# Luonic/semi-supervised_semantic_segmentation

Hardware: AMD Instinct MI355X
Metric: images/sec (UNet-R50 512x512 bs=16/GPU, mean-teacher + CowMix semi-supervised training step) (higher is better)
Workload: dtype bf16; 1 GPU; C2: UNet(ResNet-50 encoder, max_width=128, ConvT up) 512x512, semi-supervised mean-teacher + CowMix step (BCE sup loss w=0.5, consistency w=10, SGD m=0.9); global_batch=16, per_gpu_batch=16, image_size=512, parallelism=dp1

## Files before the change

### include/ssseg.h

```cpp
#ifndef SSSEG_H
#define SSSEG_H
#include <stdint.h>
#include <stddef.h>

#ifdef __cplusplus
extern "C" {
#endif

typedef struct ihipStream_t* ssseg_stream_t;

enum { SSSEG_F32 = 0, SSSEG_BF16 = 1, SSSEG_F16 = 2, SSSEG_F64 = 3  };
enum { SSSEG_OK = 0, SSSEG_EINVAL = -1, SSSEG_EUNSUPPORTED = -2, SSSEG_EWORKSPACE = -3, SSSEG_ECOMM = -4 };

const char* ssseg_version(void);


size_t ssseg_cowmix_workspace_bytes(int64_t B, int64_t H, int64_t W);

int ssseg_cowmix_mask(const float* noise, const float* sigma, const float* p, int64_t B, int64_t H,
                      int64_t W, float* mask_out, float* field_out, float* thr_out, void* workspace,
                      size_t workspace_bytes, ssseg_stream_t stream);

int ssseg_normal_f32(float* out, int64_t n, uint64_t seed, uint64_t offset, ssseg_stream_t stream);

// ... 184 lines not shown
                        const float* gout, float* gx, const void* ws, size_t ws_bytes, ssseg_stream_t stream);

int ssseg_ohem_labels_fwd(const float* x, const void* labels, int label_kind, int64_t B, int64_t C, int64_t HW,
                          int64_t ignore_label, float thresh, int64_t min_kept, float* out, void* ws, size_t ws_bytes,
                          ssseg_stream_t stream);
int ssseg_ohem_labels_bwd(const float* x, const void* labels, int label_kind, int64_t B, int64_t C, int64_t HW,
                          const float* gout, float* gx, const void* ws, size_t ws_bytes, ssseg_stream_t stream);

int ssseg_focal_fwd(const float* x, const float* t, int64_t n, double alpha, double gamma, float* out, void* ws,
                    size_t ws_bytes, ssseg_stream_t stream);
int ssseg_focal_bwd(const float* x, const float* t, int64_t n, double alpha, double gamma, const float* gout,
                    float* gx, ssseg_stream_t stream);

typedef struct ssseg_nfl_params {
  double alpha, gamma, eps, scale, weight, ignore_label;
  int32_t from_logits, size_average;
} ssseg_nfl_params;
int ssseg_nfl_fwd(const float* x, const float* label, int64_t B, int64_t C, int64_t HW,
                  const ssseg_nfl_params* params_host, float* out, float* k_sum, void* ws, size_t ws_bytes,
                  ssseg_stream_t stream);
int ssseg_nfl_bwd(const float* x, const float* label, int64_t B, int64_t C, int64_t HW,
                  const ssseg_nfl_params* params_host, const float* gout, float* gx, const void* ws, size_t ws_bytes,
                  ssseg_stream_t stream);

int ssseg_dice_logits_fwd(const float* x, const float* t, int64_t B, int64_t C, int64_t HW, float* out, void* ws,
                          size_t ws_bytes, ssseg_stream_t stream);
int ssseg_dice_logits_bwd(const float* x, const float* t, int64_t B, int64_t C, int64_t HW, const float* gout,
                          float* gx, const void* ws, size_t ws_bytes, ssseg_stream_t stream);

int ssseg_dice_prob_fwd(const float* p, const float* t, int64_t B, int64_t n, int log_mode, float gamma, float* out,
                        void* ws, size_t ws_bytes, ssseg_stream_t stream);
int ssseg_dice_prob_bwd(const float* t, int64_t B, int64_t n, int log_mode, float gamma, const float* gout,
                        float* gx, const void* ws, size_t ws_bytes, ssseg_stream_t stream);

int ssseg_binary_entropy_fwd(const float* x, int64_t n, float* out, void* ws, size_t ws_bytes,
                             ssseg_stream_t stream);
int ssseg_binary_entropy_bwd(const float* x, int64_t n, const float* gout, float* gx, ssseg_stream_t stream);
int ssseg_entropy_fwd(const float* x, int64_t B, int64_t C, int64_t HW, float* out, void* ws, size_t ws_bytes,
                      ssseg_stream_t stream);
int ssseg_entropy_bwd(const float* x, int64_t B, int64_t C, int64_t HW, const float* gout, float* gx,
                      ssseg_stream_t stream);

int ssseg_bce_logits_red_fwd(const float* x, const float* t, int64_t n, int reduction, float* out, void* ws,
                             size_t ws_bytes, ssseg_stream_t stream);
int ssseg_bce_logits_red_bwd(const float* x, const float* t, int64_t n, int reduction, const float* gout, float* gx,
                             ssseg_stream_t stream);

int ssseg_smooth_labels(const float* t, float* out, int64_t n, float a, float b, ssseg_stream_t stream);


int ssseg_ema_update(float* ema, const float* param, int64_t n, double alpha, ssseg_stream_t stream);

int ssseg_sigmoid_fwd(const float* x, float* y, int64_t n, ssseg_stream_t stream);
int ssseg_sigmoid_bwd(const float* y, const float* gy, float* gx, int64_t n, ssseg_stream_t stream);

int ssseg_axpby(const float* x, float a, const float* y, float b, float* out, int64_t n, ssseg_stream_t stream);
int ssseg_scale_f32(float* x, int64_t n, float a, ssseg_stream_t stream);

int ssseg_sqnorm_accum(const float* x, int64_t n, float* out, void* ws, size_t ws_bytes, ssseg_stream_t stream);

int ssseg_sgd_step(float* param, float* grad, float* momentum_buf, uint16_t* bf16_shadow, int64_t n,
                   float lr, float momentum, float weight_decay, float max_norm, const float* sqnorm,
                   int first_step, const float* amp_state, ssseg_stream_t stream);
int ssseg_amp_update(float* state, const float* sqnorm, float growth, float backoff, int interval,
                     ssseg_stream_t stream);
enum { SSSEG_OPT_ADAM = 0, SSSEG_OPT_ADAMOD = 1, SSSEG_OPT_DIFFGRAD = 2, SSSEG_OPT_DIFFMOD = 3, SSSEG_OPT_RANGER = 4 };
#define SSSEG_OPT_STATE_DOUBLES 8
int ssseg_optim_prepare(double* state, int mode, double lr, double beta1, double beta2, double weight_decay,
                        double max_norm, int64_t k, double nsma_threshold, const float* sqnorm,
                        const float* amp_state, ssseg_stream_t stream);
int ssseg_optim_step(float* param, const float* grad, float* exp_avg, float* exp_avg_sq, float* exp_avg_lr,
                     float* previous_grad, float* slow_buffer, int64_t n, int mode, int version, double beta1,
                     double beta2, double beta3, double eps, double weight_decay, double alpha, const double* state,
                     ssseg_stream_t stream);
int ssseg_scale_by(const float* x, const float* s, float* y, int64_t n, ssseg_stream_t stream);

typedef struct {
  int64_t N, H, W, C, ldx;
  int64_t OH, OW;
  int64_t K;
  int64_t R, S;
  int64_t sy, sx, dy, dx, py, px;
  int64_t outH, outW;
  int64_t osy, osx, ooy, oox;
  int64_t ldy;
  int64_t ldw;
} ssseg_conv_desc;

int ssseg_conv_igemm(const void* x, const void* w, void* y, const ssseg_conv_desc* desc_host, int dt, int dt_out,
                     const float* bias, int relu, void* ws, size_t ws_bytes, ssseg_stream_t stream);
#define SSSEG_ACT_NONE 0
#define SSSEG_ACT_RELU 1
#define SSSEG_ACT_RELU6 2
#define SSSEG_ACT_LEAKY 3

typedef struct ssseg_conv_epilogue {
  const float* scale;
  const float* shift;
  const void* residual;
  int64_t ldr;
  void* aux;
  int32_t relu;
  float slope;
  double* stats;
  int64_t stats_ld;
  int64_t* stats_rows_host;
} ssseg_conv_epilogue;
int ssseg_conv_igemm_epi(const void* x, const void* w, void* y, const ssseg_conv_desc* desc_host, int dt, int dt_out,
                         const ssseg_conv_epilogue* epi, void* ws, size_t ws_bytes, ssseg_stream_t stream);
int ssseg_conv_igemm_epi_actmask(const void* x, const void* w, void* y, const ssseg_conv_desc* desc_host, int dt,
                                 int dt_out, const ssseg_conv_epilogue* epi, int act, float slope, void* ws,
                                 size_t ws_bytes, ssseg_stream_t stream);
int ssseg_conv_igemm_epi_join(const void* x, const void* w, void* y, const ssseg_conv_desc* desc_host, int dt,
                              int dt_out, const ssseg_conv_epilogue* epi, const void* mask, int64_t ldm, void* ws,
                              size_t ws_bytes, ssseg_stream_t stream);
typedef struct {
  const void* x2;
  int64_t c1;
  int64_t ldx2;
} ssseg_vcat;

int ssseg_conv_igemm_epi_vcat(const void* x, const ssseg_vcat* vc, const void* w, void* y,
                              const ssseg_conv_desc* desc_host, int dt, int dt_out, const ssseg_conv_epilogue* epi,
                              void* ws, size_t ws_bytes, ssseg_stream_t stream);
int ssseg_conv_igemm_epi_vsplit(const void* x, const void* w, void* y, const ssseg_vcat* ysplit,
                                const ssseg_conv_desc* desc_host, int dt, int dt_out, const ssseg_conv_epilogue* epi,
                                void* ws, size_t ws_bytes, ssseg_stream_t stream);
int ssseg_conv_igemm_phases(const void* x, void* y, const ssseg_conv_desc* desc_host, int dt, int dt_out,
                            const ssseg_conv_epilogue* epi, int64_t nphase, const int64_t* phase_geom,
                            const void* const* w, ssseg_stream_t stream);
size_t ssseg_conv_igemm_phases_workspace_bytes(const ssseg_conv_desc* desc_host, int64_t nphase, int dt);
int ssseg_conv_igemm_phases_ws(const void* x, void* y, const ssseg_conv_desc* desc_host, int dt, int dt_out,
                               const ssseg_conv_epilogue* epi, int64_t nphase, const int64_t* phase_geom,
                               const void* const* w, void* ws, size_t ws_bytes, ssseg_stream_t stream);

int ssseg_conv_stem_epi(const void* x, const void* w4, void* y, const ssseg_conv_desc* desc_host, int dt,
                        const ssseg_conv_epilogue* epi, ssseg_stream_t stream);
size_t ssseg_conv_igemm_workspace_bytes(const ssseg_conv_desc* desc_host, int dt);

int ssseg_set_knob(int id, int value);

int64_t ssseg_tune_table_export(unsigned long long* keys_host, int32_t* variants_host, int64_t cap);
int ssseg_tune_table_import(const unsigned long long* keys_host, const int32_t* variants_host, int64_t n,
                            int overwrite);

size_t ssseg_conv_wgrad_workspace_bytes(const ssseg_conv_desc* desc_host, int dt);
int ssseg_conv_wgrad(const void* x, const void* dy, float* dw, const ssseg_conv_desc* desc_host, int dt, int64_t c_real,
                     int64_t k_real, int layout, int accumulate, void* ws, size_t ws_bytes, ssseg_stream_t stream);

size_t ssseg_conv_wgrad2_workspace_bytes(const ssseg_conv_desc* desc_host, int64_t n2, int dt);
int ssseg_conv_wgrad2(const void* x, const void* dy, const void* x2, const void* dy2, int64_t n2, float* dw,
                      const ssseg_conv_desc* desc_host, int dt, int64_t c_real, int64_t k_real, int layout,
                      int accumulate, void* ws, size_t ws_bytes, ssseg_stream_t stream);

int ssseg_conv_wgrad_vcat(const void* x, const ssseg_vcat* vc, const void* dy, float* dw,
                          const ssseg_conv_desc* desc_host, int dt, int64_t c_real, int64_t k_real, int layout,
                          int accumulate, void* ws, size_t ws_bytes, ssseg_stream_t stream);
int ssseg_conv_wgrad2_vcat(const void* x, const ssseg_vcat* vc, const void* dy, const void* x2, const ssseg_vcat* vc2,
                           const void* dy2, int64_t n2, float* dw, const ssseg_conv_desc* desc_host, int dt,
                           int64_t c_real, int64_t k_real, int layout, int accumulate, void* ws, size_t ws_bytes,
                           ssseg_stream_t stream);

int ssseg_weight_pack(const float* src, void* dst, int64_t Kd, int64_t Kr, int64_t Cd, int64_t Rs, int64_t Ss,
                      int64_t Cp, int layout, int64_t r0, int64_t rstep, int64_t Rn, int64_t s0, int64_t sstep,
                      int64_t Sn, int dt, ssseg_stream_t stream);

typedef struct ssseg_pack_desc {
  const float* src;
  void* dst;
  int64_t Kd, Kr, Cd, Rs, Ss, Cp;
  int64_t layout, r0, rstep, Rn, s0, sstep, Sn;
} ssseg_pack_desc;
int ssseg_weight_pack_batch(const ssseg_pack_desc* descs, int64_t n, int dt, ssseg_stream_t stream);

#define SSSEG_PSTEP_SGD 1
#define SSSEG_PSTEP_EMA 2
#define SSSEG_PSTEP_CLEAR 4
typedef struct ssseg_pstep_desc {
  int64_t off, n;
  int64_t A, B, Rs, Ss, Ap, Bp;
  int64_t pack0, npacks;
} ssseg_pstep_desc;
typedef struct ssseg_pstep_pack {
  void* dst;
  int64_t teacher, layout;
  int64_t Kd, Cp, r0, rstep, Rn, s0, sstep, Sn;
} ssseg_pstep_pack;
int ssseg_param_step(float* param, float* grad, float* momentum_buf, float* ema, const ssseg_pstep_desc* descs,
                     int64_t n_descs, const ssseg_pstep_pack* packs, float lr, float momentum, float weight_decay,
                     float max_norm, const float* sqnorm, int first_step, const float* amp_state, double alpha,
                     int flags, ssseg_stream_t stream);

int ssseg_dwconv_fwd(const void* x, const void* w, void* y, const ssseg_conv_desc* desc_host, int dt,
                     const ssseg_conv_epilogue* epi, ssseg_stream_t stream);
int ssseg_dwconv_dgrad(const void* dy, const void* w, void* dx, const ssseg_conv_desc* desc_host, int dt,
                       ssseg_stream_t stream);
size_t ssseg_dwconv_wgrad_workspace_bytes(const ssseg_conv_desc* desc_host, int dt);
int ssseg_dwconv_wgrad(const void* x, const void* dy, float* dw, const ssseg_conv_desc* desc_host, int dt,
                       int64_t c_real, int accumulate, void* ws, size_t ws_bytes, ssseg_stream_t stream);

size_t ssseg_bn_workspace_bytes(int64_t C);
int ssseg_bn_stats(const void* x, int64_t P, int64_t C, int64_t ldx, int dt, double* sums, void* ws, size_t ws_bytes,
                   ssseg_stream_t stream);
int ssseg_bn_finalize(const double* sums, int64_t C, double count, float eps, float momentum, float* mean_out,
                      float* invstd_out, float* running_mean, float* running_var, int64_t* num_batches_tracked,
                      ssseg_stream_t stream);
int ssseg_bn_stats_finalize(const void* x, int64_t P, int64_t C, int64_t ldx, int dt, double* sums, void* ws,
                            size_t ws_bytes, double count, float eps, float momentum, float* mean_out, float* invstd_out,
                            float* running_mean, float* running_var, int64_t* num_batches_tracked,
                            ssseg_stream_t stream);
int ssseg_bn_partials_finalize(double* part, int64_t nparts, int64_t C, double* sums, double count, float eps,
                               float momentum, float* mean_out, float* invstd_out, float* running_mean,
                               float* running_var, int64_t* num_batches_tracked, ssseg_stream_t stream);
int ssseg_channel_sum_grad(const void* x, int64_t P, int64_t C, int64_t ldx, int dt, float* dsum, double* sums,
                           void* ws, size_t ws_bytes, ssseg_stream_t stream);
int ssseg_bn_gstat_finalize(double* part, int64_t nparts, int64_t C, double* sums, const float* gamma,
                            const float* beta, const float* mean_eff, const float* invstd, float* dgamma, float* dbeta,
                            float* dconv_bias, ssseg_stream_t stream);
int ssseg_bn_gstat_finalize_x(double* part, int64_t nparts, int64_t C, double* sums, const float* gamma,
                              const float* beta, const void* dy, const void* x, int64_t P, int64_t ld, int dt,
                              const float* mean, const float* invstd, float* dgamma, float* dbeta,
                              ssseg_stream_t stream);
int ssseg_bn_eval_params(const float* running_mean, const float* running_var, float eps, int64_t C, float* mean_out,
                         float* invstd_out, ssseg_stream_t stream);
int ssseg_bn_fold(const float* running_mean, const float* running_var, const float* gamma, const float* beta,
                  const float* conv_bias, float eps, int64_t C, int64_t Cp, float* scale, float* shift,
                  float* mean_eff, float* invstd_out, ssseg_stream_t stream);
typedef struct ssseg_fold_desc {
  const float* running_mean;
  const float* running_var;
  const float* gamma;
  const float* beta;
  const float* conv_bias;
  float* out;
  int64_t C, Cp;
  double eps;
} ssseg_fold_desc;
int ssseg_bn_fold_batch(const ssseg_fold_desc* descs, int64_t n, ssseg_stream_t stream);
int ssseg_bn_eval_bwd(const void* dy, const void* y, const void* aux, void* dconv, void* dres, int64_t P, int64_t C,
                      int64_t ld, const float* scale, const float* mean_eff, const float* invstd, int relu, int dt,
                      double* sums, void* ws, size_t ws_bytes, ssseg_stream_t stream);
int ssseg_bn_eval_param_grad(const double* sums, int64_t C, const float* scale, float* dgamma, float* dbeta,
                             float* dconv_bias, ssseg_stream_t stream);
int ssseg_bn_eval_bwd_grad(const void* dy, const void* y, const void* aux, void* dconv, void* dres, int64_t P, int64_t C,
                           int64_t ld, const float* scale, const float* mean_eff, const float* invstd, int relu, int dt,
                           double* sums, void* ws, size_t ws_bytes, float* dgamma, float* dbeta, float* dconv_bias,
                           ssseg_stream_t stream);
int ssseg_bn_eval_bwd_grad_y(const void* dy, const void* y, void* dconv, void* dres, int64_t P, int64_t C, int64_t ld,
                             const float* scale, const float* shift, const float* mean_eff, const float* invstd,
                             int relu, int dt, double* sums, void* ws, size_t ws_bytes, float* dgamma, float* dbeta,
                             float* dconv_bias, ssseg_stream_t stream);
int ssseg_bn_eval_bwd_part(const void* dy, const void* y, const void* aux, void* dconv, void* dres, int64_t P, int64_t C,
                           int64_t ld, const float* scale, const float* shift, const float* mean_eff,
                           const float* invstd, int relu, int dt, double* part, size_t part_bytes, int64_t* nparts_host,
                           ssseg_stream_t stream);
typedef struct ssseg_pgrad_desc {
  const double* part;
  int64_t nparts, C;
  const float* scale;
  float* dgamma;
  float* dbeta;
  float* dconv_bias;
  const float* shift;
  const float* mean_eff;
  const float* invstd;
} ssseg_pgrad_desc;
int ssseg_bn_param_grad_batch(const ssseg_pgrad_desc* descs, int64_t n, int64_t max_c, ssseg_stream_t stream);
int ssseg_bn_apply(const void* x, const void* residual, void* y, int64_t P, int64_t C, int64_t ldx, int64_t ldr,
                   int64_t ldy, const float* mean, const float* invstd, const float* gamma, const float* beta, int relu,
                   int dt, ssseg_stream_t stream);
int ssseg_bn_bwd_reduce(const void* dy, const void* x, const void* residual, int64_t P, int64_t C, int64_t ldx,
                        int64_t ldr, int64_t lddy, const float* mean, const float* invstd, const float* gamma,
                        const float* beta, int relu, int dt, double* sums, void* ws, size_t ws_bytes,
                        ssseg_stream_t stream);
int ssseg_bn_param_grad(const double* sums, int64_t C, float* dgamma, float* dbeta, ssseg_stream_t stream);
int ssseg_bn_bwd_reduce_grad(const void* dy, const void* x, const void* residual, int64_t P, int64_t C, int64_t ldx,
                             int64_t ldr, int64_t lddy, const float* mean, const float* invstd, const float* gamma,
                             const float* beta, int relu, int dt, double* sums, void* ws, size_t ws_bytes,
                             float* dgamma, float* dbeta, ssseg_stream_t stream);
int ssseg_bn_bwd_apply(const void* dy, const void* x, const void* residual, void* dx, void* dres, int64_t P, int64_t C,
                       int64_t ldx, int64_t ldr, int64_t lddy, int64_t lddx, const float* mean, const float* invstd,
                       const float* gamma, const float* beta, int relu, int train, const double* sums, double count,
                       int dt, ssseg_stream_t stream);

int ssseg_maxpool_fwd(const void* x, void* y, uint8_t* idx, int64_t N, int64_t H, int64_t W, int64_t C, int64_t OH,
                      int64_t OW, int64_t k, int64_t s, int64_t p, int dt, ssseg_stream_t stream);
int ssseg_maxpool_bwd(const void* gy, const uint8_t* idx, void* gx, int64_t N, int64_t H, int64_t W, int64_t C,
                      int64_t OH, int64_t OW, int64_t k, int64_t s, int64_t p, int dt, ssseg_stream_t stream);
int ssseg_maxpool_bwd_res(const void* gy, const uint8_t* idx, const void* res, void* gx, int64_t N, int64_t H,
                          int64_t W, int64_t C, int64_t OH, int64_t OW, int64_t k, int64_t s, int64_t p, int dt,
                          ssseg_stream_t stream);
int ssseg_nhwc_copy(const void* src, void* dst, int64_t N, int64_t H, int64_t W, int64_t C, int64_t sH, int64_t sW,
                    int64_t sld, int64_t soy, int64_t sox, int64_t dH, int64_t dW, int64_t dld, int64_t doy, int64_t dox,
                    int dt, ssseg_stream_t stream);
int ssseg_zero(void* p, size_t bytes, ssseg_stream_t stream);

typedef struct {
  const void* src;
  void* dst;
  const void* add;
  int64_t ld;
  int64_t c;
} ssseg_cat_part;
int ssseg_nhwc_cat_n(const ssseg_cat_part* parts_host, int64_t nparts, void* y, int64_t npix, int64_t ldy, int dt,
                     ssseg_stream_t stream);
int ssseg_nhwc_split_n(const void* gy, int64_t ldg, const ssseg_cat_part* parts_host, int64_t nparts, int64_t npix,
// ... 100 lines not shown
```

### semi-supervised_semantic_segmentation_amd/csrc/conv_kernels.h

```cpp
#pragma once
#include <algorithm>
#include <type_traits>

#include "common.h"

typedef __bf16 bf16x8 __attribute__((ext_vector_type(8)));
typedef _Float16 f16x8 __attribute__((ext_vector_type(8)));

typedef short s16x4 __attribute__((ext_vector_type(4)));
typedef float f32x4 __attribute__((ext_vector_type(4)));

template <typename T16> struct M16;
template <> struct M16<bf16_t> {
  __device__ __forceinline__ static f32x4 mma(const bf16x8& a, const bf16x8& b, const f32x4& c) {
    return __builtin_amdgcn_mfma_f32_16x16x32_bf16(a, b, c, 0, 0, 0);
  }
};
template <> struct M16<f16_t> {
  __device__ __forceinline__ static f32x4 mma(const bf16x8& a, const bf16x8& b, const f32x4& c) {
    return __builtin_amdgcn_mfma_f32_16x16x32_f16(__builtin_bit_cast(f16x8, a), __builtin_bit_cast(f16x8, b), c, 0, 0,
                                                  0);
  }
};
typedef __attribute__((address_space(3))) s16x4 lds_s16x4;
// ... 1222 lines not shown
      const float z[8] = {0.f, 0.f, 0.f, 0.f, 0.f, 0.f, 0.f, 0.f};
      Out8<TO>::st(ep.aux + op * g.ldy + n, z);
    }
    Out8<TO>::st(out_at(ep, y, g.ldy, op, n), v);
  }
}

template <typename TO>
__global__ void phase_zero_kernel(TO* y, ConvGeom g, Epi<TO> ep) {
  const long long total = g.M * g.K;
  for (long long i = (long long)blockIdx.x * blockDim.x + threadIdx.x; i < total; i += (long long)gridDim.x * blockDim.x) {
    const int n = (int)(i % g.K);
    const long long m = i / g.K;
    const long long op = out_pixel(g, (int)m);
    float v = ep.shift ? ep.shift[n] : 0.f;
    if (ep.aux) io<TO>::st(ep.aux, op * g.ldy + n, 0.f);
    if (ep.res && !ep.rmask) v += io<TO>::ld(ep.res, op * ep.ldr + n);
    v = act_fwd(v, ep.relu, ep.slope);
    io<TO>::st(out_at(ep, y, g.ldy, op, n), 0, v);
  }
}

template <typename T, int BM, int BN>
inline int plan_splits(const ConvGeom& g);

template <typename TO>
__global__ void splitk_finalize_kernel(const float* __restrict__ ws, TO* __restrict__ y, ConvGeom g, Epi<TO> ep);

extern thread_local int t_dsplit;

unsigned* ticket_slots(long long n);

template <typename TO, int BM, int BN, int WM, int WN, int NW, int NS, int VC>
int launch_glds_vc(const void* x, const void* w, void* y, const ConvGeom& g, const Epi<TO>& ep, unsigned xb,
                   unsigned wb, hipStream_t s, float* ws, const PhaseTab* ph, const void* x2, unsigned x2b) {
  static_assert(sizeof(TO) == 2, "LDS-DMA configs: 16-bit activations in and out (fp32-output heads have K <= 16)");
  constexpr int FRAGS = (BM / WM / 16) * (BN / WN / 16);
  const long long tiles = ((g.M + BM - 1) / BM) * ((g.K + BN - 1) / BN);
  const int epi = (int)(g_knobs[7] == 0);
  const TO* xa = (const TO*)x2;
  const PhaseTab one{1, {0}, {0}, {0}, {0}, {nullptr}};
  const bool phased = ph && ph->n > 1;
  const PhaseTab& pt = phased ? *ph : one;
  const unsigned nph = phased ? (unsigned)ph->n : 1u;
  const int sp = ws ? t_dsplit : 1;
  if (sp > 1 && (FRAGS > DSPLIT_MAX_FRAGS || tiles * sp > 0x7fffffffLL)) return -1;
  unsigned* tix = sp > 1 ? ticket_slots(tiles * nph) : nullptr;
  if (sp > 1 && !tix) return -1;
  const dim3 grid((unsigned)(tiles * sp), nph);
  if (ep.zmask) {
    if constexpr (VC != 1 && BM * BN < 256 * 256) {
      if (ep.stats) return -1;
      hipLaunchKernelGGL((igemm_glds_kernel<TO, BM, BN, WM, WN, NW, NS, false, VC, true>), grid, dim3(NW * 64), 0, s,
                         (const TO*)x, (const TO*)w, (TO*)y, g, ep, xb, wb, epi, sp, ws, tix, pt, xa, x2b);
      return BM;
    }
    return -1;
  }
  if (ep.stats)
    hipLaunchKernelGGL((igemm_glds_kernel<TO, BM, BN, WM, WN, NW, NS, true, VC>), grid, dim3(NW * 64), 0, s,
                       (const TO*)x, (const TO*)w, (TO*)y, g, ep, xb, wb, epi, sp, ws, tix, pt, xa, x2b);
  else
    hipLaunchKernelGGL((igemm_glds_kernel<TO, BM, BN, WM, WN, NW, NS, false, VC>), grid, dim3(NW * 64), 0, s,
                       (const TO*)x, (const TO*)w, (TO*)y, g, ep, xb, wb, epi, sp, ws, tix, pt, xa, x2b);
  return BM;
}

static inline size_t dsplit_ws_bytes(const ConvGeom& g, int nph, int S) {
  if (S <= 1) return 0;
  const long long t64 = (long long)nph * ((g.M + 63) / 64) * ((g.K + 63) / 64);
  return (size_t)(dsplit_ticket_bytes(t64) + (long long)S * nph * (g.M + 255) * (g.K + 127) * 4);
}

template <typename TO, int BM, int BN, int WM, int WN, int NW, int NS>
int launch_glds(const void* x, const void* w, void* y, const ConvGeom& g, const Epi<TO>& ep, unsigned xb, unsigned wb,
                hipStream_t s, float* ws, const PhaseTab* ph, const void* x2 = nullptr, unsigned x2b = 0) {
  if (x2) return launch_glds_vc<TO, BM, BN, WM, WN, NW, NS, 1>(x, w, y, g, ep, xb, wb, s, ws, ph, x2, x2b);
  if (g.C & 63) {
    if constexpr (BN == 64) return launch_glds_vc<TO, BM, BN, WM, WN, NW, NS, 2>(x, w, y, g, ep, xb, wb, s, ws, ph, nullptr, 0);
    return -1;
  }
  return launch_glds_vc<TO, BM, BN, WM, WN, NW, NS, 0>(x, w, y, g, ep, xb, wb, s, ws, ph, nullptr, 0);
}


template <typename TO>
int launch_glds_grp_a(int cfg, const void* x, const void* w, void* y, const ConvGeom& g, const Epi<TO>& ep, unsigned xb,
                      unsigned wb, hipStream_t s, float* ws, const PhaseTab* ph, const void* x2 = nullptr,
                      unsigned x2b = 0);
template <typename TO>
int launch_glds_grp_b(int cfg, const void* x, const void* w, void* y, const ConvGeom& g, const Epi<TO>& ep, unsigned xb,
                      unsigned wb, hipStream_t s, float* ws, const PhaseTab* ph, const void* x2 = nullptr,
                      unsigned x2b = 0);
template <typename TO>
int launch_glds_grp_d(int cfg, const void* x, const void* w, void* y, const ConvGeom& g, const Epi<TO>& ep, unsigned xb,
                      unsigned wb, hipStream_t s, float* ws, const PhaseTab* ph, const void* x2 = nullptr,
                      unsigned x2b = 0);
template <typename TO>
int launch_glds_grp_e(int cfg, const void* x, const void* w, void* y, const ConvGeom& g, const Epi<TO>& ep, unsigned xb,
                      unsigned wb, hipStream_t s, float* ws, const PhaseTab* ph, const void* x2 = nullptr,
                      unsigned x2b = 0);
template <typename TO>
int launch_glds_grp_c(int cfg, const void* x, const void* w, void* y, const ConvGeom& g, const Epi<TO>& ep, unsigned xb,
                      unsigned wb, hipStream_t s, float* ws, const PhaseTab* ph, const void* x2 = nullptr,
                      unsigned x2b = 0);


template <typename T, int BM, int BN>
inline int plan_splits(const ConvGeom& g) {
  const long long tiles = ((g.M + BM - 1) / BM) * ((g.K + BN - 1) / BN);
  const int nk = (g.KK + 64 / (int)sizeof(T) - 1) / (64 / (int)sizeof(T));
  if (g_knobs[1] < 0 || tiles >= 512 || nk < 32) return 1;
  long long sp = (1024 + tiles - 1) / tiles;
  sp = std::min<long long>(sp, nk / 16);
  if (g_knobs[1] > 0) sp = std::min<long long>(sp, g_knobs[1]);
  return (int)std::max<long long>(1, std::min<long long>(sp, 64));
}


template <typename TO>
int launch_hconv3(const void* x, const void* w, void* y, const ConvGeom& g, const Epi<TO>& ep, unsigned xb,
                  unsigned wb, hipStream_t s, float* ws, const PhaseTab* ph, const void* x2, unsigned x2b,
                  int mode = 0);

template <typename TO>
int launch_hconv3s(const void* x, const void* w, void* y, const ConvGeom& g, const Epi<TO>& ep, unsigned xb,
                   hipStream_t s, float* ws, const PhaseTab* ph, const void* x2);

template <typename TO>
int launch_pw(int fj, const void* x, const void* w, void* y, const ConvGeom& g, const Epi<TO>& ep, hipStream_t s,
              float* ws, const PhaseTab* ph, const void* x2);
extern thread_local long long t_pw_rows;

struct HaloSeg {
  const void* x;
  const void* x2;
  const void* dy;
  unsigned xbytes, x2bytes, dbytes;
};
struct HaloArgs {
  HaloSeg seg[2];
  int H, W, C, K, ldx, ldx2, ldy, c1;
  int ncb, nkb, nstrips;
  long long steps[2], sps[2];
  int splits, s1;
  float* slab;
  float* dw;
  int c_real, k_real, layout, accumulate;
};
struct HaloPlan {
  int ncb, nkb, nstrips, splits, s1;
  long long steps[2], sps[2];
};
bool halo3_eligible(const ConvGeom& g, int dt);
HaloPlan halo3_plan(const ConvGeom& g, long long n1, long long n2);
size_t halo3_ws_bytes(const ConvGeom& g, long long n1, long long n2);
void launch_wgrad_halo3(int dt, const HaloArgs& a, hipStream_t s);

template <typename T, typename TO>
int dispatch_regstaged(const void* x, const void* w, void* y, const ConvGeom& g, const Epi<TO>& ep, float* ws,
                       hipStream_t s);
```

### semi-supervised_semantic_segmentation_amd/csrc/conv_wgrad.hip

```cpp
#include <algorithm>

#include "conv_kernels.h"

template <typename T> struct WG;
template <> struct WG<bf16_t> {
  static constexpr int BKP = 64;
  static constexpr int PADB = 32;
};
template <> struct WG<f16_t> : WG<bf16_t> {};
template <> struct WG<float> {
  static constexpr int BKP = 16;
  static constexpr int PADB = 64;
};

__device__ __forceinline__ int kperm(int g, int j) { return 16 * (g >> 1) + 8 * (j >> 2) + 4 * (g & 1) + (j & 3); }

struct WDirect {
  float* dw;
  int c_real, k_real, layout, accumulate;
};

template <typename T, int BMW, int BNW>
__global__ void __launch_bounds__(256) wgrad_kernel(const T* __restrict__ x, const T* __restrict__ dy,
                                                    float* __restrict__ slab, ConvGeom g, long long pix_per_split,
// ... 90 lines not shown
    const int buf = kt & 1;
    if (kt + 1 < nk) load();
    const char* Xs = smem + buf * BKP * (ROWX + ROWD);
    const char* Ds = Xs + BKP * ROWX;
    if constexpr (sizeof(T) == 2) {
#pragma unroll
      for (int ks = 0; ks < BKP / 32; ++ks) {
      bf16x8 af[FM], bfr[FN];
      const int r0 = ks * 32 + kperm(gq, q4), r1 = ks * 32 + kperm(gq, 4 + q4);
#pragma unroll
      for (int i = 0; i < FM; ++i) {
        const int col = wm * WTM + i * 16 + 4 * p4;
        s16x4 lo = __builtin_amdgcn_ds_read_tr16_b64_v4i16((lds_s16x4*)(Xs + r0 * ROWX + col * 2));
        s16x4 hi = __builtin_amdgcn_ds_read_tr16_b64_v4i16((lds_s16x4*)(Xs + r1 * ROWX + col * 2));
        af[i] = __builtin_bit_cast(bf16x8, __builtin_shufflevector(lo, hi, 0, 1, 2, 3, 4, 5, 6, 7));
      }
#pragma unroll
      for (int j = 0; j < FN; ++j) {
        const int col = wn * WTN + j * 16 + 4 * p4;
        s16x4 lo = __builtin_amdgcn_ds_read_tr16_b64_v4i16((lds_s16x4*)(Ds + r0 * ROWD + col * 2));
        s16x4 hi = __builtin_amdgcn_ds_read_tr16_b64_v4i16((lds_s16x4*)(Ds + r1 * ROWD + col * 2));
        bfr[j] = __builtin_bit_cast(bf16x8, __builtin_shufflevector(lo, hi, 0, 1, 2, 3, 4, 5, 6, 7));
      }
#pragma unroll
      for (int i = 0; i < FM; ++i)
#pragma unroll
        for (int j = 0; j < FN; ++j) acc[i][j] = M16<T>::mma(af[i], bfr[j], acc[i][j]);
      }
    } else {
#pragma unroll
      for (int ks = 0; ks < BKP / 4; ++ks) {
        const int row = ks * 4 + gq;
        float af[FM], bfr[FN];
#pragma unroll
        for (int i = 0; i < FM; ++i) af[i] = *(const float*)(Xs + row * ROWX + (wm * WTM + i * 16 + li) * 4);
#pragma unroll
        for (int j = 0; j < FN; ++j) bfr[j] = *(const float*)(Ds + row * ROWD + (wn * WTN + j * 16 + li) * 4);
#pragma unroll
        for (int i = 0; i < FM; ++i)
#pragma unroll
          for (int j = 0; j < FN; ++j) acc[i][j] = __builtin_amdgcn_mfma_f32_16x16x4f32(af[i], bfr[j], acc[i][j], 0, 0, 0);
      }
    }
    if (kt + 1 < nk) store(buf ^ 1);
    __syncthreads();
  }

  if (dd.dw) {
#pragma unroll
    for (int i = 0; i < FM; ++i) {
      const int kkb = kk0 + wm * WTM + i * 16 + 4 * gq;
#pragma unroll
      for (int j = 0; j < FN; ++j) {
        const int co = co0 + wn * WTN + j * 16 + li;
        if (co >= dd.k_real) continue;
#pragma unroll
        for (int e = 0; e < 4; ++e) {
          const int kk = kkb + e;
          if (kk >= g.KK) continue;
          const int c = kk % g.C, tap = kk / g.C;
          if (c >= dd.c_real) continue;
          long long o;
          if (dd.layout == 0) o = ((long long)co * g.R * g.S + tap) * g.C + c;
          else o = (((long long)co * dd.c_real + c) * g.R + tap / g.S) * g.S + tap % g.S;
          dd.dw[o] = dd.accumulate ? dd.dw[o] + acc[i][j][e] : acc[i][j][e];
        }
      }
    }
    return;
  }
  float* sl = slab + (long long)blockIdx.z * g.K * g.KK;
#pragma unroll
  for (int i = 0; i < FM; ++i) {
    const int kk = kk0 + wm * WTM + i * 16 + 4 * gq;
#pragma unroll
    for (int j = 0; j < FN; ++j) {
      const int co = co0 + wn * WTN + j * 16 + li;
      if (co >= g.K || kk >= g.KK) continue;
      float* p = sl + (long long)co * g.KK + kk;
      if (kk + 3 < g.KK) {
        *(float4*)p = make_float4(acc[i][j][0], acc[i][j][1], acc[i][j][2], acc[i][j][3]);
      } else {
        for (int e = 0; e < 4 && kk + e < g.KK; ++e) p[e] = acc[i][j][e];
      }
    }
  }
}

template <int FM, int FN>
__device__ __forceinline__ void wgrad_store(const f32x4 (&acc)[FM][FN], int kkb0, int cob0, int lane,
                                            const ConvGeom& g, float* __restrict__ slab, const WDirect& dd,
                                            int split) {
  const int gq = lane >> 4, li = lane & 15;
  if (dd.dw) {
#pragma unroll
    for (int i = 0; i < FM; ++i) {
      const int kkb = kkb0 + i * 16 + 4 * gq;
#pragma unroll
      for (int j = 0; j < FN; ++j) {
        const int co = cob0 + j * 16 + li;
        if (co >= dd.k_real) continue;
#pragma unroll
        for (int e = 0; e < 4; ++e) {
          const int kk = kkb + e;
          if (kk >= g.KK) continue;
          const int c = kk % g.C, tap = kk / g.C;
          if (c >= dd.c_real) continue;
          long long o;
          if (dd.layout == 0) o = ((long long)co * g.R * g.S + tap) * g.C + c;
          else o = (((long long)co * dd.c_real + c) * g.R + tap / g.S) * g.S + tap % g.S;
          dd.dw[o] = dd.accumulate ? dd.dw[o] + acc[i][j][e] : acc[i][j][e];
        }
      }
    }
    return;
  }
  float* sl = slab + (long long)split * g.K * g.KK;
#pragma unroll
  for (int i = 0; i < FM; ++i) {
    const int kk = kkb0 + i * 16 + 4 * gq;
#pragma unroll
    for (int j = 0; j < FN; ++j) {
      const int co = cob0 + j * 16 + li;
      if (co >= g.K || kk >= g.KK) continue;
      float* p = sl + (long long)co * g.KK + kk;
      if (kk + 3 < g.KK) {
        *(float4*)p = make_float4(acc[i][j][0], acc[i][j][1], acc[i][j][2], acc[i][j][3]);
      } else {
        for (int e = 0; e < 4 && kk + e < g.KK; ++e) p[e] = acc[i][j][e];
      }
    }
  }
}

template <int ROWB>
__device__ __forceinline__ int wswz(int r) {
  if constexpr (ROWB == 256) return ((r & 3) << 2) | ((r >> 2) & 3);
  else return (((r >> 1) & 1) << 2) | (((r >> 3) & 1) << 1);
}
__device__ __forceinline__ int wkp(int g, int j) { return 16 * (g >> 1) + 8 * (g & 1) + 4 * (j >> 2) + (j & 3); }

struct WSeg2 {
  const void* x;
  const void* dy;
  long long M;
  unsigned xbytes, dbytes;
  int s1;
  int c1, ldx2;
  const void* xa;
  const void* xb;
  unsigned xabytes, xbbytes;
};

template <typename T16, int BMW, int BNW, int NS, int WM = 2, int WN = 2, int BKP = 64, bool ST = false, bool GK = false>
__global__ void __launch_bounds__(WM * WN * 64) wgrad_glds_kernel(const T16* __restrict__ x, const T16* __restrict__ dy,
                                                                   float* __restrict__ slab, ConvGeom g,
                                                                   long long pix_per_split, WDirect dd, unsigned xbytes,
                                                                   unsigned dbytes, WSeg2 sg) {
  constexpr int NW = WM * WN, NT = NW * 64;
  constexpr int ROWX = BMW * 2, ROWD = BNW * 2;
  constexpr int XCPR = ROWX / 16, DCPR = ROWD / 16;
  constexpr int XI = BKP * XCPR / NT, DI = BKP * DCPR / NT;
  constexpr int NL = (ST ? 2 : 1) * XI + DI;
  constexpr int STAGE = BKP * (ROWX + ROWD);
  constexpr int WTM = BMW / WM, WTN = BNW / WN, FM = WTM / 16, FN = WTN / 16;
  static_assert(XI >= 1 && DI >= 1 && NS >= 2 && NS <= 4 && FM >= 1 && FN >= 1 && BKP % 32 == 0, "wgrad glds tile");
  __shared__ __attribute__((aligned(1024))) char smem[NS * STAGE];

  const int t = threadIdx.x, lane = t & 63, wave = __builtin_amdgcn_readfirstlane(t >> 6);
  const int wm = wave / WN, wn = wave % WN;
  const int mt = (g.KK + BMW - 1) / BMW, nt = (g.K + BNW - 1) / BNW;
  const int tile = xcd_tile(blockIdx.x, gridDim.x);
  const int split = tile / (mt * nt), rem = tile - split * (mt * nt);
  const int kk0 = (rem % mt) * BMW, co0 = (rem / mt) * BNW;
  const bool seg2 = sg.s1 > 0 && split >= sg.s1;
  const long long p_begin = (long long)(seg2 ? split - sg.s1 : split) * pix_per_split;
  const long long p_end = min(p_begin + pix_per_split, seg2 ? sg.M : g.M);
  const int tap = kk0 / g.C, c0 = kk0 - tap * g.C;
  const int tr = tap / g.S, ts = tap - tr * g.S;
  const int offy = tr * g.dy + g.py, offx = ts * g.dx + g.px;
  const bool src2 = sg.c1 > 0 && c0 >= sg.c1;
  const void* xbase = src2 ? (seg2 ? sg.xb : sg.xa) : (seg2 ? sg.x : (const void*)x);
  const unsigned xbyt = src2 ? (seg2 ? sg.xbbytes : sg.xabytes) : (seg2 ? sg.xbytes : xbytes);
  const int ldx = src2 ? sg.ldx2 : g.ldx, cb0 = src2 ? c0 - sg.c1 : c0;
  const __amdgpu_buffer_rsrc_t xr = __builtin_amdgcn_make_buffer_rsrc((void*)xbase, (short)0, (int)xbyt, 0x00020000);
  const bool strad = ST && sg.c1 > c0 && sg.c1 < c0 + BMW;
  __amdgpu_buffer_rsrc_t xr2 = xr;
  if constexpr (ST)
    xr2 = __builtin_amdgcn_make_buffer_rsrc(seg2 ? (void*)sg.xb : (void*)sg.xa, (short)0,
                                            (int)(seg2 ? sg.xbbytes : sg.xabytes), 0x00020000);
  const __amdgpu_buffer_rsrc_t dr = __builtin_amdgcn_make_buffer_rsrc(seg2 ? (void*)sg.dy : (void*)dy, (short)0,
                                                                      (int)(seg2 ? sg.dbytes : dbytes), 0x00020000);

  long long xp[XI];
  int xoy[XI], xox[XI], ximg[XI], xcb[XI];
  int gofy[GK ? XI : 1], gofx[GK ? XI : 1];
  bool xin2[ST ? XI : 1];
#pragma unroll
  for (int ii = 0; ii < XI; ++ii) {
    const int row = (wave * XI + ii) * (64 / XCPR) + lane / XCPR;
    xcb[ii] = (cb0 + ((lane % XCPR) ^ wswz<ROWX>(row)) * 8) * 2;
    if constexpr (GK) {
      const int kk = kk0 + ((lane % XCPR) ^ wswz<ROWX>(row)) * 8;
      const int tp = fdiv(kk, g.mC, g.sC), c = kk - tp * g.C;
      const int r = fdiv(tp, g.mS, g.sS), s_ = tp - r * g.S;
      xcb[ii] = c * 2;
      gofy[ii] = tp < g.R * g.S ? r * g.dy + g.py : -0x40000000;
      gofx[ii] = s_ * g.dx + g.px;
    }
    if constexpr (ST) {
      xin2[ii] = strad && c0 + ((lane % XCPR) ^ wswz<ROWX>(row)) * 8 >= sg.c1;
      if (xin2[ii]) xcb[ii] -= sg.c1 * 2;
    }
    xp[ii] = p_begin + row;
    const long long pp = xp[ii] < p_end ? xp[ii] : 0;
    decode_m(g, (int)pp, ximg[ii], xoy[ii], xox[ii]);
  }
  long long dp[DI];
  int dcb[DI];
#pragma unroll
  for (int jj = 0; jj < DI; ++jj) {
    const int row = (wave * DI + jj) * (64 / DCPR) + lane / DCPR;
    const int co = co0 + ((lane % DCPR) ^ wswz<ROWD>(row)) * 8;
    dcb[jj] = co < g.K ? co * 2 : -1;
    dp[jj] = p_begin + row;
  }
  auto issue = [&](int buf) {
    char* Xs = smem + buf * STAGE;
    char* Ds = Xs + BKP * ROWX;
#pragma unroll
    for (int ii = 0; ii < XI; ++ii) {
      unsigned off = OOB;
      if constexpr (ST) {
        if (strad) {
          unsigned o1 = OOB, o2 = OOB;
          if (xp[ii] < p_end) {
            const int iy = xoy[ii] * g.sy + offy, ix = xox[ii] * g.sx + offx;
            if ((unsigned)iy < (unsigned)g.H && (unsigned)ix < (unsigned)g.W) {
              const unsigned pix = (unsigned)((ximg[ii] * g.H + iy) * g.W + ix);
              o1 = pix * (unsigned)g.ldx * 2u + (unsigned)xcb[ii];
              o2 = pix * (unsigned)sg.ldx2 * 2u + (unsigned)xcb[ii];
            }
          }
          if (!xin2[ii]) bldslds16_nt(xr, Xs + (wave * XI + ii) * 1024, o1, 0);
          if (xin2[ii]) bldslds16_nt(xr2, Xs + (wave * XI + ii) * 1024, o2, 0);
        }
      }
      if (xp[ii] < p_end) {
        const int iy = xoy[ii] * g.sy + (GK ? gofy[ii] : offy), ix = xox[ii] * g.sx + (GK ? gofx[ii] : offx);
        if ((unsigned)iy < (unsigned)g.H && (unsigned)ix < (unsigned)g.W)
          off = (unsigned)(((ximg[ii] * g.H + iy) * g.W + ix) * ldx) * 2u + (unsigned)xcb[ii];
      }
      if (!strad) bldslds16_nt(xr, Xs + (wave * XI + ii) * 1024, off, 0);
      xp[ii] += BKP;
      if (BKP < g.OW) {
        xox[ii] += BKP;
        if (xox[ii] >= g.OW) {
          xox[ii] -= g.OW;
          if (++xoy[ii] == g.OH) {
            xoy[ii] = 0;
            ++ximg[ii];
          }
        }
      } else if (xp[ii] < p_end) {
        decode_m(g, (int)xp[ii], ximg[ii], xoy[ii], xox[ii]);
      }
    }
#pragma unroll
    for (int jj = 0; jj < DI; ++jj) {
      const unsigned off = (dp[jj] < p_end && dcb[jj] >= 0) ? (unsigned)(dp[jj] * g.ldy * 2 + dcb[jj]) : OOB;
      bldslds16_nt(dr, Ds + (wave * DI + jj) * 1024, off, 0);
      dp[jj] += BKP;
    }
  };

  f32x4 acc[FM][FN];
#pragma unroll
  for (int i = 0; i < FM; ++i)
#pragma unroll
    for (int j = 0; j < FN; ++j) acc[i][j] = f32x4{0.f, 0.f, 0.f, 0.f};

  const int gq = lane >> 4, li = lane & 15, q4 = li >> 2, p4 = li & 3;
  auto compute = [&](int buf) {
    const char* Xs = smem + buf * STAGE;
    const char* Ds = Xs + BKP * ROWX;
#pragma unroll
    for (int ks = 0; ks < BKP / 32; ++ks) {
      const int r0 = ks * 32 + wkp(gq, q4), r1 = ks * 32 + wkp(gq, 4 + q4);
      const int sx0 = 16 * wswz<ROWX>(r0), sx1 = 16 * wswz<ROWX>(r1);
      const int sd0 = 16 * wswz<ROWD>(r0), sd1 = 16 * wswz<ROWD>(r1);
      bf16x8 af[FM], bfr[FN];
#pragma unroll
      for (int i = 0; i < FM; ++i) {
        const int col = wm * WTM + i * 16 + 4 * p4;
        const int cb = 16 * (col >> 3), e8 = 2 * (col & 7);
        s16x4 lo = __builtin_amdgcn_ds_read_tr16_b64_v4i16((lds_s16x4*)(Xs + r0 * ROWX + (cb ^ sx0) + e8));
        s16x4 hi = __builtin_amdgcn_ds_read_tr16_b64_v4i16((lds_s16x4*)(Xs + r1 * ROWX + (cb ^ sx1) + e8));
        af[i] = __builtin_bit_cast(bf16x8, __builtin_shufflevector(lo, hi, 0, 1, 2, 3, 4, 5, 6, 7));
      }
#pragma unroll
      for (int j = 0; j < FN; ++j) {
        const int col = wn * WTN + j * 16 + 4 * p4;
        const int cb = 16 * (col >> 3), e8 = 2 * (col & 7);
        s16x4 lo = __builtin_amdgcn_ds_read_tr16_b64_v4i16((lds_s16x4*)(Ds + r0 * ROWD + (cb ^ sd0) + e8));
        s16x4 hi = __builtin_amdgcn_ds_read_tr16_b64_v4i16((lds_s16x4*)(Ds + r1 * ROWD + (cb ^ sd1) + e8));
        bfr[j] = __builtin_bit_cast(bf16x8, __builtin_shufflevector(lo, hi, 0, 1, 2, 3, 4, 5, 6, 7));
      }
#pragma unroll
      for (int i = 0; i < FM; ++i)
#pragma unroll
        for (int j = 0; j < FN; ++j) acc[i][j] = M16<T16>::mma(af[i], bfr[j], acc[i][j]);
    }
  };

  const long long npix = p_end > p_begin ? p_end - p_begin : 0;
  const int nk = (int)((npix + BKP - 1) / BKP);
  constexpr int D = NS - 1;
#pragma unroll
  for (int p = 0; p < D; ++p)
    if (p < nk) issue(p);
  for (int kt = 0; kt < nk; ++kt) {
    const int ahead = min(nk - 1, kt + D - 1) - kt;
    if (ST && !strad) ring_wait<XI + DI, D>(ahead);
    else ring_wait<NL, D>(ahead);
    __builtin_amdgcn_s_barrier();
    if (kt + D < nk) issue((kt + D) % NS);
    compute(kt % NS);
  }
  wgrad_store<FM, FN>(acc, kk0 + wm * WTM, co0 + wn * WTN, lane, g, slab, dd, split);
}

template <int V>
__global__ void __launch_bounds__(1024) wgrad_reduce_wide_kernel(const float* __restrict__ slab, int splits, int K, int R,
                                                            int S, int C, int c_real, int k_real,
                                                            float* __restrict__ dst, int layout, int accumulate) {
  typedef float vec_t __attribute__((ext_vector_type(V)));
  __shared__ vec_t red[16][64];
  const long long KK = (long long)R * S * C;
  const long long total = (long long)K * KK;
  const int lane = threadIdx.x & 63, w = threadIdx.x >> 6;
  const long long i = ((long long)blockIdx.x * 64 + lane) * V;
  vec_t a0 = 0.f, a1 = 0.f;
  if (i < total) {
    int z = w;
#pragma unroll 8
    for (; z + 16 < splits; z += 32) {
      a0 += *(const vec_t*)(slab + (long long)z * total + i);
      a1 += *(const vec_t*)(slab + (long long)(z + 16) * total + i);
    }
    if (z < splits) a0 += *(const vec_t*)(slab + (long long)z * total + i);
  }
  red[w][lane] = a0 + a1;
  __syncthreads();
  if (w != 0 || i >= total) return;
  vec_t sum = 0.f;
#pragma unroll
  for (int k = 0; k < 16; ++k) sum += red[k][lane];
  const int kk = (int)(i % KK), k = (int)(i / KK);
  const int c = kk % C, tap = kk / C, r = tap / S, s = tap % S;
  if (k >= k_real) return;
#pragma unroll
  for (int e = 0; e < V; ++e) {
    if (c + e >= c_real) break;
    long long o;
    if (layout == 0) o = ((long long)k * R * S + tap) * C + c + e;
    else o = (((long long)k * c_real + c + e) * R + r) * S + s;
    const float v = sum[e];
    dst[o] = accumulate ? dst[o] + v : v;
  }
}

__global__ void wgrad_reduce_kernel(const float* __restrict__ slab, int splits, int K, int R, int S, int C, int c_real,
                                    int k_real, float* __restrict__ dst, int layout, int accumulate) {
  const long long KK = (long long)R * S * C;
  const long long total = (long long)K * KK;
  for (long long i = (long long)blockIdx.x * blockDim.x + threadIdx.x; i < total; i += (long long)gridDim.x * blockDim.x) {
    const int kk = (int)(i % KK), k = (int)(i / KK);
    const int c = kk % C, tap = kk / C, r = tap / S, s = tap % S;
    if (c >= c_real || k >= k_real) continue;
    float s0 = 0.f, s1 = 0.f, s2 = 0.f, s3 = 0.f;
    int z = 0;
    for (; z + 4 <= splits; z += 4) {
      s0 += slab[(long long)z * total + i];
      s1 += slab[(long long)(z + 1) * total + i];
      s2 += slab[(long long)(z + 2) * total + i];
      s3 += slab[(long long)(z + 3) * total + i];
    }
    for (; z < splits; ++z) s0 += slab[(long long)z * total + i];
    const float sum = (s0 + s1) + (s2 + s3);
    long long o;
    if (layout == 0) o = ((long long)k * R * S + tap) * C + c;
    else o = (((long long)k * c_real + c) * R + r) * S + s;
    dst[o] = accumulate ? dst[o] + sum : sum;
  }
}

namespace {

struct WgradPlan {
  int bmw, bnw, mt, nt, splits;
  long long pps;
  bool glds;
  int cfg;
  bool st = false;
};

struct WgradCfg {
  int bmw, bnw, ns, wm, wn, bkp;
  int pct = 100;
};
constexpr WgradCfg WGRAD_CFGS[] = {
    {0, 0, 0, 0, 0, 0},
    {64, 64, 3, 2, 2, 64},
    {128, 64, 3, 2, 2, 64},
    {64, 128, 3, 2, 2, 64},
    {128, 128, 2, 2, 2, 64},
    {128, 64, 3, 4, 2, 64},
    {128, 128, 2, 2, 4, 64},
    {128, 64, 2, 2, 2, 128},
    {64, 64, 3, 2, 2, 128},
    {256, 64, 2, 4, 2, 64},
    {128, 128, 3, 2, 4, 64},
    {64, 64, 4, 2, 2, 64},
    {128, 64, 4, 2, 2, 64},
    {64, 128, 4, 2, 2, 64},
    {64, 64, 3, 2, 4, 64},
    {64, 128, 3, 2, 4, 64},
    {64, 128, 3, 4, 2, 64},
    {128, 128, 2, 4, 2, 64},
    {128, 64, 2, 4, 2, 64},
    {128, 128, 2, 2, 4, 64, 50},
    {64, 128, 3, 4, 2, 64, 50},
};
constexpr int N_WGRAD_CFGS = (int)(sizeof(WGRAD_CFGS) / sizeof(WGRAD_CFGS[0]));

template <typename T>
WgradPlan plan_wgrad(const ConvGeom& g, int bmw = 0, long long slots = 0, int bnw = 0, int bkp_ = 0, int pct = 100) {
  WgradPlan p;
  p.glds = false;
  p.cfg = 0;
  p.bnw = bnw ? bnw : (g.K <= 64 ? 64 : 128);
  p.bmw = bmw ? bmw : (g.KK <= 64 ? 64 : 128);
  p.mt = (g.KK + p.bmw - 1) / p.bmw;
  p.nt = (g.K + p.bnw - 1) / p.bnw;
  const long long tiles = (long long)p.mt * p.nt;
  const int bkp = bkp_ ? bkp_ : WG<T>::BKP;
  const long long max_splits_by_work = std::max<long long>(1, g.M / (bkp * 8));
  long long want = std::max<long long>(1, (1024 + tiles - 1) / tiles);
  if (slots > 0 && tiles < 1024) {
    const long long rounds = std::max<long long>(1, (1024 + slots / 2) / slots);
    want = std::max<long long>(1, rounds * slots / tiles);
  }
  if (pct != 100) want = std::max<long long>(1, want * pct / 100);
  if (g_knobs[10] != 100 && g_knobs[10] > 0) want = std::max<long long>(1, want * g_knobs[10] / 100);
  const long long slab_cap = std::max<long long>(1, (64ll << 20) / (4ll * g.K * g.KK + 1));
  long long sp = std::min(std::min(want, max_splits_by_work), slab_cap);
  sp = std::max<long long>(1, std::min<long long>(sp, 65535));
  p.pps = (g.M + sp - 1) / sp;
  p.pps = (p.pps + bkp - 1) / bkp * bkp;
  p.splits = (int)((g.M + p.pps - 1) / p.pps);
  if (p.splits < 1) p.splits = 1;
  return p;
}

template <typename T>
void launch_wgrad(const void* x, const void* dy, float* slab, const ConvGeom& g, const WgradPlan& p, WDirect dd,
                  hipStream_t s) {
  const dim3 grid(p.mt, p.nt, p.splits);
  if (p.bmw == 64 && p.bnw == 64)
    hipLaunchKernelGGL((wgrad_kernel<T, 64, 64>), grid, dim3(256), 0, s, (const T*)x, (const T*)dy, slab, g, p.pps, dd);
  else if (p.bmw == 64)
    hipLaunchKernelGGL((wgrad_kernel<T, 64, 128>), grid, dim3(256), 0, s, (const T*)x, (const T*)dy, slab, g, p.pps, dd);
  else if (p.bnw == 64)
    hipLaunchKernelGGL((wgrad_kernel<T, 128, 64>), grid, dim3(256), 0, s, (const T*)x, (const T*)dy, slab, g, p.pps, dd);
  else
    hipLaunchKernelGGL((wgrad_kernel<T, 128, 128>), grid, dim3(256), 0, s, (const T*)x, (const T*)dy, slab, g, p.pps, dd);
}

static bool wgrad_glds_ok(const ConvGeom& g, int dt) {
  if ((dt != SSSEG_BF16 && dt != SSSEG_F16) || g_knobs[8] != 0) return false;
  if (g.C % 8 || g.ldx % 8 || g.ldy % 8 || g.K % 8) return false;
  const long long xb = (long long)g.N * g.H * g.W * g.ldx * 2, db = g.M * g.ldy * 2;
  return xb < 0x7fffffffLL && db < 0x7fffffffLL;
}

long long wgrad_slots(int cfg);

static int static_wgrad_cfg(const ConvGeom& g) {
  const int bmw = (g.C % 128 == 0 && g.KK > 64) ? 128 : 64;
  const int bnw = g.K <= 64 ? 64 : 128;
  return bmw == 64 ? (bnw == 64 ? 1 : 20) : (bnw == 64 ? 18 : 19);
}

static int wgrad_cfg_for(const ConvGeom& g, int c1 = 0, bool* st = nullptr) {
  int c = g_knobs[9];
  if (!(c > 0 && c < N_WGRAD_CFGS && (g.C % 64 ? WGRAD_CFGS[c].bmw == 64 : g.C % WGRAD_CFGS[c].bmw == 0)))
    c = static_wgrad_cfg(g);
  if (st) *st = false;
  if (c1 > 0 && c1 % WGRAD_CFGS[c].bmw) {
    if (WGRAD_CFGS[c].bmw == 128 && c1 % 64 == 0 && st) *st = true;
    else c = WGRAD_CFGS[c].bnw == 64 ? 1 : 20;
  }
  return c;
}

static WgradPlan plan_for_cfg(const ConvGeom& g, int c) {
  const WgradCfg& wc = WGRAD_CFGS[c];
  WgradPlan p = plan_wgrad<bf16_t>(g, wc.bmw, wgrad_slots(c), wc.bnw, wc.bkp, wc.pct);
  p.glds = true;
  p.cfg = c;
  return p;
}

static WgradPlan choose_wgrad(const ConvGeom& g, int dt) {
  if (wgrad_glds_ok(g, dt)) return plan_for_cfg(g, wgrad_cfg_for(g));
  return dt != SSSEG_F32 ? plan_wgrad<bf16_t>(g) : plan_wgrad<float>(g);
}

template <typename T16, int C, bool ST = false, bool GK = false>
constexpr auto wgrad_kernel_of() {
  return &wgrad_glds_kernel<T16, WGRAD_CFGS[C].bmw, WGRAD_CFGS[C].bnw, WGRAD_CFGS[C].ns, WGRAD_CFGS[C].wm,
                            WGRAD_CFGS[C].wn, WGRAD_CFGS[C].bkp, ST, GK>;
}

template <int C>
long long wgrad_slots_t() {
  static long long slots = -1;
  if (slots < 0) {
    int per_cu = 0, dev = 0, cus = 0;
    if (hipGetDevice(&dev) != hipSuccess ||
        hipDeviceGetAttribute(&cus, hipDeviceAttributeMultiprocessorCount, dev) != hipSuccess ||
        hipOccupancyMaxActiveBlocksPerMultiprocessor(&per_cu, wgrad_kernel_of<bf16_t, C>(),
                                                     WGRAD_CFGS[C].wm * WGRAD_CFGS[C].wn * 64, 0) != hipSuccess)
      return 0;
    slots = (long long)per_cu * cus;
  }
  return slots;
}

template <int C = 1>
long long wgrad_slots_dispatch(int c) {
  if constexpr (C < N_WGRAD_CFGS) {
    if (c == C) return wgrad_slots_t<C>();
    return wgrad_slots_dispatch<C + 1>(c);
  } else {
    return 0;
  }
}

long long wgrad_slots(int cfg) { return wgrad_slots_dispatch<1>(cfg); }

template <typename T16, int C>
void launch_wgrad_glds_t(const void* x, const void* dy, float* slab, const ConvGeom& g, const WgradPlan& p, WDirect dd,
                         hipStream_t s, const WSeg2& sg) {
  const unsigned xb = (unsigned)((long long)g.N * g.H * g.W * g.ldx * 2), db = (unsigned)(g.M * g.ldy * 2);
  if constexpr (WGRAD_CFGS[C].bmw == 64) {
    if (g.C % 64) {
      hipLaunchKernelGGL((wgrad_kernel_of<T16, C, false, true>()), dim3(p.mt * p.nt * p.splits),
                         dim3(WGRAD_CFGS[C].wm * WGRAD_CFGS[C].wn * 64), 0, s, (const T16*)x, (const T16*)dy, slab, g,
                         p.pps, dd, xb, db, sg);
      return;
    }
  }
  if constexpr (WGRAD_CFGS[C].bmw == 128) {
    if (p.st) {
      hipLaunchKernelGGL((wgrad_kernel_of<T16, C, true>()), dim3(p.mt * p.nt * p.splits),
                         dim3(WGRAD_CFGS[C].wm * WGRAD_CFGS[C].wn * 64), 0, s, (const T16*)x, (const T16*)dy, slab, g,
                         p.pps, dd, xb, db, sg);
      return;
    }
  }
  hipLaunchKernelGGL((wgrad_kernel_of<T16, C>()), dim3(p.mt * p.nt * p.splits),
                     dim3(WGRAD_CFGS[C].wm * WGRAD_CFGS[C].wn * 64), 0, s, (const T16*)x, (const T16*)dy, slab, g,
                     p.pps, dd, xb, db, sg);
}

template <typename T16, int C = 1>
void launch_wgrad_glds_dispatch(const void* x, const void* dy, float* slab, const ConvGeom& g, const WgradPlan& p,
                                WDirect dd, hipStream_t s, const WSeg2& sg) {
  if constexpr (C < N_WGRAD_CFGS) {
    if (p.cfg == C) return launch_wgrad_glds_t<T16, C>(x, dy, slab, g, p, dd, s, sg);
    return launch_wgrad_glds_dispatch<T16, C + 1>(x, dy, slab, g, p, dd, s, sg);
  }
}

template <typename T16>
void launch_wgrad_glds(const void* x, const void* dy, float* slab, const ConvGeom& g, const WgradPlan& p, WDirect dd,
                       hipStream_t s, const WSeg2& sg = WSeg2{nullptr, nullptr, 0, 0, 0, 0, 0, 0, nullptr, nullptr, 0,
                                                               0}) {
  launch_wgrad_glds_dispatch<T16, 1>(x, dy, slab, g, p, dd, s, sg);
}


bool wg_geom_ok(const ConvGeom& g, int dt) {
  const int vec = dt == SSSEG_F32 ? 4 : 8;
  if (g.C % vec || g.ldx % vec || g.ldw % vec) return false;
  if (g.N < 1 || g.OH < 1 || g.OW < 1 || g.K < 1 || g.C < 1) return false;
  if (g.M >= 0x7fffffffLL) return false;
  if (g.R < 0 || g.S < 0) return false;
  return true;
}

}

static size_t wgrad_ws_bytes(const ConvGeom& g, int dt) {
  const WgradPlan p = choose_wgrad(g, dt);
  size_t b = (size_t)p.splits * g.K * g.KK * sizeof(float);
  if (halo3_eligible(g, dt)) b = std::max(b, halo3_ws_bytes(g, g.N, 0));
  if (p.glds) {
    const WgradPlan q = plan_for_cfg(g, wgrad_cfg_for(g, 64));
    b = std::max(b, (size_t)q.splits * g.K * g.KK * sizeof(float));
  }
  return b + 256;
}

extern "C" size_t ssseg_conv_wgrad_workspace_bytes(const ssseg_conv_desc* d, int dt) {
  ConvGeom g;
  if (!make_geom(d, g)) return 0;
  return wgrad_ws_bytes(g, dt);
}

namespace {

void launch_reduce(const float* slab, const ConvGeom& g, int splits, int64_t c_real, int64_t k_real, float* dw,
                   int layout, int accumulate, hipStream_t s) {
  const long long total = (long long)g.K * g.KK;
  if (splits >= 64 && total >= 32768 && g.C % 4 == 0 && ((uintptr_t)slab & 15) == 0)
    hipLaunchKernelGGL(wgrad_reduce_wide_kernel<4>, dim3((unsigned)((total + 255) / 256)), dim3(1024), 0, s, slab,
                       splits, g.K, g.R, g.S, g.C, (int)c_real, (int)k_real, dw, layout, accumulate);
  else if (splits >= 64)
    hipLaunchKernelGGL(wgrad_reduce_wide_kernel<1>, dim3((unsigned)((total + 63) / 64)), dim3(1024), 0, s, slab, splits,
                       g.K, g.R, g.S, g.C, (int)c_real, (int)k_real, dw, layout, accumulate);
  else
    hipLaunchKernelGGL(wgrad_reduce_kernel, dim3(ssseg_grid(total, 256)), dim3(256), 0, s, slab, splits, g.K, g.R, g.S,
                       g.C, (int)c_real, (int)k_real, dw, layout, accumulate);
}

bool vcat_ok(const ssseg_vcat* vc, const ConvGeom& g, int dt) {
  if (!vc) return true;
  return vc->x2 && vc->c1 > 0 && vc->c1 < g.C && vc->c1 % 64 == 0 && (g.C - vc->c1) % 64 == 0 && g.ldx >= vc->c1 &&
         vc->ldx2 >= g.C - vc->c1 && vc->ldx2 % 8 == 0 && vc->ldx2 <= 0x7fffffff && (dt == SSSEG_BF16 || dt == SSSEG_F16) &&
         (long long)g.N * g.H * g.W * vc->ldx2 * 2 < 0x7fffffffLL;
}

void run_halo3(const ConvGeom& g, int dt, const void* x, const ssseg_vcat* vc, const void* dy, const void* x2,
               const ssseg_vcat* vc2, const void* dy2, long long n2, float* dw, int64_t c_real, int64_t k_real,
               int layout, int accumulate, float* slab, hipStream_t s) {
  const HaloPlan p = halo3_plan(g, g.N, n2);
  HaloArgs a{};
  const long long pix1 = (long long)g.N * g.H * g.W, pix2 = n2 * g.H * g.W;
  a.seg[0] = HaloSeg{x, vc ? vc->x2 : nullptr, dy, (unsigned)(pix1 * g.ldx * 2),
                     vc ? (unsigned)(pix1 * vc->ldx2 * 2) : 0u, (unsigned)(pix1 * g.ldy * 2)};
  if (n2 > 0)
    a.seg[1] = HaloSeg{x2, vc2 ? vc2->x2 : nullptr, dy2, (unsigned)(pix2 * g.ldx * 2),
                       vc2 ? (unsigned)(pix2 * vc2->ldx2 * 2) : 0u, (unsigned)(pix2 * g.ldy * 2)};
  a.H = g.H;
  a.W = g.W;
  a.C = g.C;
  a.K = g.K;
  a.ldx = g.ldx;
  a.ldx2 = vc ? (int)vc->ldx2 : 0;
  a.ldy = g.ldy;
  a.c1 = vc ? (int)vc->c1 : 0;
  a.ncb = p.ncb;
  a.nkb = p.nkb;
  a.nstrips = p.nstrips;
  a.steps[0] = p.steps[0];
  a.steps[1] = p.steps[1];
  a.sps[0] = p.sps[0];
  a.sps[1] = p.sps[1];
  a.splits = p.splits;
  a.s1 = p.s1;
  a.slab = slab;
  a.dw = p.splits == 1 ? dw : nullptr;
  a.c_real = (int)c_real;
  a.k_real = (int)k_real;
  a.layout = layout;
  a.accumulate = accumulate;
  launch_wgrad_halo3(dt, a, s);
  if (p.splits > 1) launch_reduce(slab, g, p.splits, c_real, k_real, dw, layout, accumulate, s);
}

bool halo3_fits(const ConvGeom& g, long long n, const ssseg_vcat* vc) {
  if (!vc && g.ldx < g.C) return false;
  const long long pix = n * g.H * g.W;
  return pix * g.ldx * 2 < 0x7fffffffLL && pix * g.ldy * 2 < 0x7fffffffLL && (!vc || pix * vc->ldx2 * 2 < 0x7fffffffLL);
}

int wgrad_one(const void* x, const ssseg_vcat* vc, const void* dy, float* dw, const ssseg_conv_desc* d, int dt,
              int64_t c_real, int64_t k_real, int layout, int accumulate, void* ws, size_t ws_bytes,
              ssseg_stream_t stream) {
  ConvGeom g;
  if (!make_geom(d, g) || !x || !dy || !dw) return SSSEG_EINVAL;
  const int vec = dt == SSSEG_F32 ? 4 : 8;
  if (!wg_geom_ok(g, dt) || g.ldy % vec || g.K % vec) return SSSEG_EINVAL;
  if (c_real < 1 || c_real > g.C || k_real < 1 || k_real > g.K || (layout != 0 && layout != 1)) return SSSEG_EINVAL;
  if (!vcat_ok(vc, g, dt)) return SSSEG_EINVAL;
  if (!ws || ws_bytes < wgrad_ws_bytes(g, dt)) return SSSEG_EWORKSPACE;
  if (dt != SSSEG_BF16 && dt != SSSEG_F16 && dt != SSSEG_F32) return SSSEG_EUNSUPPORTED;
  hipStream_t s = (hipStream_t)stream;
  float* slab = (float*)ws;
  if (halo3_eligible(g, dt) && halo3_fits(g, g.N, vc)) {
    run_halo3(g, dt, x, vc, dy, nullptr, nullptr, nullptr, 0, dw, c_real, k_real, layout, accumulate, slab, s);
    SSSEG_LAUNCH_CHECK();
    return 0;
  }
  WgradPlan p = choose_wgrad(g, dt);
  if (!p.glds && g.C > g.ldx) return SSSEG_EUNSUPPORTED;
  if (vc) {
    if (!p.glds) return SSSEG_EUNSUPPORTED;
    bool st = false;
    p = plan_for_cfg(g, wgrad_cfg_for(g, (int)vc->c1, &st));
    p.st = st;
  }
  const WDirect dd{p.splits == 1 ? dw : nullptr, (int)c_real, (int)k_real, layout, accumulate};
  WSeg2 sg{nullptr, nullptr, 0, 0, 0, 0, 0, 0, nullptr, nullptr, 0, 0};
  if (vc) {
    sg.c1 = (int)vc->c1;
    sg.ldx2 = (int)vc->ldx2;
    sg.xa = vc->x2;
    sg.xabytes = (unsigned)((long long)g.N * g.H * g.W * vc->ldx2 * 2);
  }
  if (p.glds && dt == SSSEG_F16)
    launch_wgrad_glds<f16_t>(x, dy, slab, g, p, dd, s, sg);
  else if (p.glds)
    launch_wgrad_glds<bf16_t>(x, dy, slab, g, p, dd, s, sg);
  else if (dt == SSSEG_BF16)
    launch_wgrad<bf16_t>(x, dy, slab, g, p, dd, s);
  else if (dt == SSSEG_F16)
    launch_wgrad<f16_t>(x, dy, slab, g, p, dd, s);
  else
    launch_wgrad<float>(x, dy, slab, g, p, dd, s);
  if (p.splits > 1) launch_reduce(slab, g, p.splits, c_real, k_real, dw, layout, accumulate, s);
  SSSEG_LAUNCH_CHECK();
  return 0;
}

bool merged_plan(const ConvGeom& g1, int64_t n2, int dt, WgradPlan& p, int& s1, ConvGeom& g2, int c1 = 0,
                 bool allow_st = true) {
  if (n2 < 1 || n2 > 0x7fffffff || !wgrad_glds_ok(g1, dt)) return false;
  g2 = g1;
  g2.N = (int)n2;
  g2.M = n2 * (long long)g1.OH * g1.OW;
  if (g2.M >= 0x7fffffffLL || !wgrad_glds_ok(g2, dt)) return false;
  ConvGeom gm = g1;
  gm.M = g1.M + g2.M;
  bool st = false;
  p = plan_for_cfg(gm, wgrad_cfg_for(g1, c1, allow_st ? &st : nullptr));
  p.st = st;
  const int bkp = WGRAD_CFGS[p.cfg].bkp;
  const long long sp = std::max(2, p.splits);
  long long a = std::min(sp - 1, std::max(1LL, (long long)((double)sp * g1.M / gm.M + 0.5)));
  long long pps = std::max((g1.M + a - 1) / a, (g2.M + (sp - a) - 1) / (sp - a));
  pps = (pps + bkp - 1) / bkp * bkp;
  p.pps = pps;
  s1 = (int)((g1.M + pps - 1) / pps);
  p.splits = s1 + (int)((g2.M + pps - 1) / pps);
  return true;
}

size_t wgrad2_ws_bytes(const ConvGeom& g, int64_t n2, int dt) {
  ConvGeom g2;
  WgradPlan p;
  int s1;
  size_t b = 0;
  for (int c1 : {0, 64})
    if (merged_plan(g, n2, dt, p, s1, g2, c1)) b = std::max(b, (size_t)p.splits * g.K * g.KK * sizeof(float) + 256);
  if (halo3_eligible(g, dt)) b = std::max(b, halo3_ws_bytes(g, g.N, n2));
  if (b) return b;
  ConvGeom gb = g;
  gb.N = (int)n2;
  gb.M = n2 * (long long)g.OH * g.OW;
  return std::max(wgrad_ws_bytes(g, dt), wgrad_ws_bytes(gb, dt));
}

int wgrad_two(const void* x, const ssseg_vcat* vc, const void* dy, const void* x2, const ssseg_vcat* vc2,
              const void* dy2, int64_t n2, float* dw, const ssseg_conv_desc* d, int dt, int64_t c_real, int64_t k_real,
              int layout, int accumulate, void* ws, size_t ws_bytes, ssseg_stream_t stream) {
  ConvGeom g, g2;
  if (!make_geom(d, g) || !x || !dy || !x2 || !dy2 || !dw || n2 < 1 || n2 > 0x7fffffff) return SSSEG_EINVAL;
  const int vec = dt == SSSEG_F32 ? 4 : 8;
  if (!wg_geom_ok(g, dt) || g.ldy % vec || g.K % vec) return SSSEG_EINVAL;
  if (c_real < 1 || c_real > g.C || k_real < 1 || k_real > g.K || (layout != 0 && layout != 1)) return SSSEG_EINVAL;
  if ((vc == nullptr) != (vc2 == nullptr) || (vc && (vc->c1 != vc2->c1 || vc->ldx2 != vc2->ldx2))) return SSSEG_EINVAL;
  ConvGeom gb = g;
  gb.N = (int)n2;
  gb.M = n2 * (long long)g.OH * g.OW;
  if (!vcat_ok(vc, g, dt) || !vcat_ok(vc2, gb, dt)) return SSSEG_EINVAL;
  if (!ws || ws_bytes < wgrad2_ws_bytes(g, n2, dt)) return SSSEG_EWORKSPACE;
  if (halo3_eligible(g, dt) && halo3_fits(g, g.N, vc) && halo3_fits(g, n2, vc2)) {
    run_halo3(g, dt, x, vc, dy, x2, vc2, dy2, n2, dw, c_real, k_real, layout, accumulate, (float*)ws,
              (hipStream_t)stream);
    SSSEG_LAUNCH_CHECK();
    return 0;
  }
  WgradPlan p;
  int s1;
  if (!merged_plan(g, n2, dt, p, s1, g2, vc ? (int)vc->c1 : 0)) {
    if (vc) return SSSEG_EUNSUPPORTED;
    ssseg_conv_desc d2 = *d;
    d2.N = n2;
    const int rc = wgrad_one(x, nullptr, dy, dw, d, dt, c_real, k_real, layout, accumulate, ws, ws_bytes, stream);
    if (rc) return rc;
    return wgrad_one(x2, nullptr, dy2, dw, &d2, dt, c_real, k_real, layout, 1, ws, ws_bytes, stream);
  }
  hipStream_t s = (hipStream_t)stream;
  float* slab = (float*)ws;
  WSeg2 sg{x2, dy2, g2.M, (unsigned)((long long)g2.N * g2.H * g2.W * g2.ldx * 2), (unsigned)(g2.M * g2.ldy * 2), s1,
           0, 0, nullptr, nullptr, 0, 0};
  if (vc) {
    sg.c1 = (int)vc->c1;
    sg.ldx2 = (int)vc->ldx2;
    sg.xa = vc->x2;
    sg.xb = vc2->x2;
    sg.xabytes = (unsigned)((long long)g.N * g.H * g.W * vc->ldx2 * 2);
    sg.xbbytes = (unsigned)((long long)g2.N * g2.H * g2.W * vc->ldx2 * 2);
  }
  const WDirect dd{nullptr, (int)c_real, (int)k_real, layout, accumulate};
  if (dt == SSSEG_F16)
    launch_wgrad_glds<f16_t>(x, dy, slab, g, p, dd, s, sg);
  else
    launch_wgrad_glds<bf16_t>(x, dy, slab, g, p, dd, s, sg);
  launch_reduce(slab, g, p.splits, c_real, k_real, dw, layout, accumulate, s);
  SSSEG_LAUNCH_CHECK();
  return 0;
}

}

extern "C" int ssseg_conv_wgrad(const void* x, const void* dy, float* dw, const ssseg_conv_desc* d, int dt,
                                int64_t c_real, int64_t k_real, int layout, int accumulate, void* ws, size_t ws_bytes,
                                ssseg_stream_t stream) {
  return wgrad_one(x, nullptr, dy, dw, d, dt, c_real, k_real, layout, accumulate, ws, ws_bytes, stream);
}

extern "C" int ssseg_conv_wgrad_vcat(const void* x, const ssseg_vcat* vc, const void* dy, float* dw,
                                     const ssseg_conv_desc* d, int dt, int64_t c_real, int64_t k_real, int layout,
                                     int accumulate, void* ws, size_t ws_bytes, ssseg_stream_t stream) {
  if (!vc) return SSSEG_EINVAL;
  return wgrad_one(x, vc, dy, dw, d, dt, c_real, k_real, layout, accumulate, ws, ws_bytes, stream);
}

extern "C" size_t ssseg_conv_wgrad2_workspace_bytes(const ssseg_conv_desc* d, int64_t n2, int dt) {
  ConvGeom g;
  if (!make_geom(d, g) || n2 < 1 || n2 > 0x7fffffff) return 0;
  return wgrad2_ws_bytes(g, n2, dt);
}

extern "C" int ssseg_conv_wgrad2(const void* x, const void* dy, const void* x2, const void* dy2, int64_t n2, float* dw,
                                 const ssseg_conv_desc* d, int dt, int64_t c_real, int64_t k_real, int layout,
                                 int accumulate, void* ws, size_t ws_bytes, ssseg_stream_t stream) {
  return wgrad_two(x, nullptr, dy, x2, nullptr, dy2, n2, dw, d, dt, c_real, k_real, layout, accumulate, ws, ws_bytes,
                   stream);
}

extern "C" int ssseg_conv_wgrad2_vcat(const void* x, const ssseg_vcat* vc, const void* dy, const void* x2,
                                      const ssseg_vcat* vc2, const void* dy2, int64_t n2, float* dw,
                                      const ssseg_conv_desc* d, int dt, int64_t c_real, int64_t k_real, int layout,
                                      int accumulate, void* ws, size_t ws_bytes, ssseg_stream_t stream) {
  if (!vc || !vc2) return SSSEG_EINVAL;
  return wgrad_two(x, vc, dy, x2, vc2, dy2, n2, dw, d, dt, c_real, k_real, layout, accumulate, ws, ws_bytes, stream);
}
```

### semi-supervised_semantic_segmentation_amd/csrc/conv_wgrad_halo.hip

```cpp
#include "conv_kernels.h"

namespace {

constexpr int HX_ROWS = 66;
constexpr int HX_SLOT = 72 * 128;
constexpr int HD_SLOT = 64 * 128;
constexpr int HD = 2;
constexpr int HXS = HD + 3;
constexpr int HDS = HD + 1;
constexpr int H_SMEM = HXS * HX_SLOT + HDS * HD_SLOT;
constexpr int H_NL = 5;

__device__ __forceinline__ int hswz(int r) { return (((r >> 1) & 1) << 2) | (((r >> 3) & 1) << 1); }
__device__ __forceinline__ int hkp(int g, int j) { return 16 * (g >> 1) + 8 * (g & 1) + 4 * (j >> 2) + (j & 3); }

template <typename T16>
__global__ void __launch_bounds__(256, 2) wgrad_halo3_kernel(HaloArgs a) {
  __shared__ __attribute__((aligned(1024))) char smem[H_SMEM];
  const int lane = threadIdx.x & 63, wave = __builtin_amdgcn_readfirstlane(threadIdx.x >> 6);
  const int tiles = a.ncb * a.nkb;
  const int tile = xcd_tile(blockIdx.x, gridDim.x);
  const int split = tile / tiles, rem = tile - split * tiles;
  const int cb = rem % a.ncb, kb = rem / a.ncb;
  const int sg = split >= a.s1 ? 1 : 0;
  const long long t0 = (long long)(sg ? split - a.s1 : split) * a.sps[sg];
  const long long t1 = min(t0 + a.sps[sg], a.steps[sg]);
  const HaloSeg& S = a.seg[sg];
  const bool part2 = a.c1 > 0 && cb * 64 >= a.c1;
  const char* xsrc = (const char*)(part2 ? S.x2 : S.x);
  const unsigned xbytes = part2 ? S.x2bytes : S.xbytes;
  const int ldx = part2 ? a.ldx2 : a.ldx, c0 = part2 ? cb * 64 - a.c1 : cb * 64;
  const __amdgpu_buffer_rsrc_t xr = __builtin_amdgcn_make_buffer_rsrc((void*)xsrc, (short)0, (int)xbytes, 0x00020000);
  const __amdgpu_buffer_rsrc_t dr = __builtin_amdgcn_make_buffer_rsrc((void*)S.dy, (short)0, (int)S.dbytes, 0x00020000);
  const int H = a.H, W = a.W;

  const int lrow = lane >> 3;
  auto chunk_of = [&](int row) { return ((lane & 7) ^ hswz(row)) * 16; };
  auto x_off = [&](int n, int yy, int row, int strip) {
    const int xx = strip * 64 - 1 + row;
    if ((unsigned)yy >= (unsigned)H || row >= HX_ROWS || (unsigned)xx >= (unsigned)W) return OOB;
    return (unsigned)(((n * H + yy) * W + xx) * ldx + c0) * 2u + (unsigned)chunk_of(row);
  };
  auto issue_x = [&](int slot, int n, int yy, int strip) {
    char* base = smem + slot * HX_SLOT;
#pragma unroll
    for (int h = 0; h < 2; ++h) {
      const int i = 2 * wave + h;
      bldslds16_nt(xr, base + i * 1024, x_off(n, yy, 8 * i + lrow, strip), 0);
    }
    if (lane < 16) bldslds16_nt(xr, base + 8 * 1024 + wave * 256, x_off(n, yy, 64 + 2 * wave + lrow, strip), 0);
  };
  auto issue_dy = [&](int slot, int n, int y, int strip) {
    char* base = smem + HXS * HX_SLOT + slot * HD_SLOT;
#pragma unroll
    for (int h = 0; h < 2; ++h) {
      const int i = 2 * wave + h;
      const int row = 8 * i + lrow;
      const unsigned off =
          (unsigned)(((n * H + y) * W + strip * 64 + row) * a.ldy + kb * 64) * 2u + (unsigned)chunk_of(row);
      bldslds16_nt(dr, base + i * 1024, off, 0);
    }
  };
  auto decode = [&](long long t, int& n, int& strip, int& y) {
    const long long q = t / H;
    y = (int)(t - q * H);
    n = (int)(q / a.nstrips);
    strip = (int)(q - (long long)n * a.nstrips);
  };
  auto xslot = [&](int yy) { return (yy + 1) % HXS; };

  f32x4 acc[9][4];
#pragma unroll
  for (int i = 0; i < 9; ++i)
#pragma unroll
    for (int j = 0; j < 4; ++j) acc[i][j] = f32x4{0.f, 0.f, 0.f, 0.f};

  const int gq = lane >> 4, li = lane & 15, q4 = li >> 2, p4 = li & 3;
  const int xcol = 2 * wave + (p4 >> 1), dsub = 8 * (p4 & 1);

  auto compute = [&](int y) {
    const char* D = smem + HXS * HX_SLOT + (y % HDS) * HD_SLOT;
#pragma unroll
    for (int ks = 0; ks < 2; ++ks) {
      const int r0 = ks * 32 + hkp(gq, q4), r1 = ks * 32 + hkp(gq, 4 + q4);
      bf16x8 bfr[4];
#pragma unroll
      for (int j = 0; j < 4; ++j) {
        const int ch = 2 * j + (p4 >> 1);
        s16x4 lo = __builtin_amdgcn_ds_read_tr16_b64_v4i16((lds_s16x4*)(D + r0 * 128 + ((ch ^ hswz(r0)) * 16) + dsub));
        s16x4 hi = __builtin_amdgcn_ds_read_tr16_b64_v4i16((lds_s16x4*)(D + r1 * 128 + ((ch ^ hswz(r1)) * 16) + dsub));
        bfr[j] = __builtin_bit_cast(bf16x8, __builtin_shufflevector(lo, hi, 0, 1, 2, 3, 4, 5, 6, 7));
      }
#pragma unroll
      for (int r = 0; r < 3; ++r) {
        const char* X = smem + xslot(y + r - 1) * HX_SLOT;
#pragma unroll
        for (int s = 0; s < 3; ++s) {
          const int x0 = r0 + s, x1 = r1 + s;
          s16x4 lo = __builtin_amdgcn_ds_read_tr16_b64_v4i16(
              (lds_s16x4*)(X + x0 * 128 + ((xcol ^ hswz(x0)) * 16) + dsub));
          s16x4 hi = __builtin_amdgcn_ds_read_tr16_b64_v4i16(
              (lds_s16x4*)(X + x1 * 128 + ((xcol ^ hswz(x1)) * 16) + dsub));
          const bf16x8 af = __builtin_bit_cast(bf16x8, __builtin_shufflevector(lo, hi, 0, 1, 2, 3, 4, 5, 6, 7));
#pragma unroll
          for (int j = 0; j < 4; ++j) acc[r * 3 + s][j] = M16<T16>::mma(af, bfr[j], acc[r * 3 + s][j]);
        }
      }
    }
  };

  if (t0 < t1) {
    int n, strip, y;
    decode(t0, n, strip, y);
    long long t = t0;
    while (true) {
      const int last = (int)min((long long)(H - 1), y + (t1 - 1 - t));
      issue_x(xslot(y - 1), n, y - 1, strip);
      issue_x(xslot(y), n, y, strip);
      issue_x(xslot(y + 1), n, y + 1, strip);
      issue_dy(y % HDS, n, y, strip);
#pragma unroll
      for (int d = 1; d < HD; ++d)
        if (y + d <= last) {
          issue_x(xslot(y + d + 1), n, y + d + 1, strip);
          issue_dy((y + d) % HDS, n, y + d, strip);
        }
      for (;; ++y, ++t) {
        ring_wait<H_NL, HD + 1>(min(HD - 1, last - y));
        __builtin_amdgcn_s_barrier();
        if (y + HD <= last) {
          issue_x(xslot(y + HD + 1), n, y + HD + 1, strip);
          issue_dy((y + HD) % HDS, n, y + HD, strip);
        }
        compute(y);
        if (y == last) break;
      }
      ++t;
      if (t >= t1) break;
      lds_barrier();
      decode(t, n, strip, y);
    }
  }

  const int cbase = cb * 64 + 16 * wave + 4 * gq;
#pragma unroll
  for (int tap = 0; tap < 9; ++tap)
#pragma unroll
    for (int j = 0; j < 4; ++j) {
      const int k = kb * 64 + 16 * j + li;
      const int kk = tap * a.C + cbase;
      if (a.dw) {
        if (k >= a.k_real) continue;
#pragma unroll
        for (int e = 0; e < 4; ++e) {
          const int c = cbase + e;
          if (c >= a.c_real) continue;
          const long long o = a.layout == 0 ? ((long long)k * 9 + tap) * a.C + c
                                            : (((long long)k * a.c_real + c) * 3 + tap / 3) * 3 + tap % 3;
          a.dw[o] = a.accumulate ? a.dw[o] + acc[tap][j][e] : acc[tap][j][e];
        }
      } else {
        float* p = a.slab + ((long long)split * a.K + k) * (9LL * a.C) + kk;
        *(float4*)p = make_float4(acc[tap][j][0], acc[tap][j][1], acc[tap][j][2], acc[tap][j][3]);
      }
    }
}

}

bool halo3_eligible(const ConvGeom& g, int dt) {
  if (g_knobs[11] < 0 || (dt != SSSEG_BF16 && dt != SSSEG_F16)) return false;
  return g.R == 3 && g.S == 3 && g.sy == 1 && g.sx == 1 && g.dy == 1 && g.dx == 1 && g.py == -1 && g.px == -1 &&
         g.OH == g.H && g.OW == g.W && g.W % 64 == 0 && g.C % 64 == 0 && g.K % 64 == 0 && g.ldx % 8 == 0 &&
         g.ldy % 8 == 0 && g.ldy >= g.K;
}

HaloPlan halo3_plan(const ConvGeom& g, long long n1, long long n2) {
  HaloPlan p;
  p.ncb = g.C / 64;
  p.nkb = g.K / 64;
  p.nstrips = g.W / 64;
  const long long tiles = (long long)p.ncb * p.nkb;
  const long long st1 = n1 * p.nstrips * g.H, st2 = n2 * p.nstrips * g.H;
  const long long slab1 = 4LL * g.K * 9 * g.C;
  long long want = std::max<long long>(1, (512 + tiles - 1) / tiles);
  const long long cap = std::max<long long>((256 + tiles - 1) / tiles, (64LL << 20) / slab1);
  want = std::min(want, cap);
  if (g_knobs[10] != 100 && g_knobs[10] > 0) want = std::max<long long>(1, want * g_knobs[10] / 100);
  want = std::min<long long>(want, st1 + st2);
  long long a1 = n2 > 0 ? std::max<long long>(1, std::min(want - 1, (long long)((double)want * st1 / (st1 + st2) + 0.5)))
                        : want;
  if (n2 > 0 && want < 2) a1 = 1;
  const long long a2 = n2 > 0 ? std::max<long long>(1, want - a1) : 0;
  p.steps[0] = st1;
  p.steps[1] = st2;
  p.sps[0] = (st1 + a1 - 1) / a1;
  p.sps[1] = a2 ? (st2 + a2 - 1) / a2 : 1;
  p.s1 = (int)((st1 + p.sps[0] - 1) / p.sps[0]);
  p.splits = p.s1 + (a2 ? (int)((st2 + p.sps[1] - 1) / p.sps[1]) : 0);
  return p;
}

size_t halo3_ws_bytes(const ConvGeom& g, long long n1, long long n2) {
  const HaloPlan p = halo3_plan(g, n1, n2);
  return (size_t)p.splits * g.K * 9 * g.C * sizeof(float) + 256;
}

void launch_wgrad_halo3(int dt, const HaloArgs& a, hipStream_t s) {
  const unsigned blocks = (unsigned)(a.splits * a.ncb * a.nkb);
  if (dt == SSSEG_F16)
    hipLaunchKernelGGL(wgrad_halo3_kernel<f16_t>, dim3(blocks), dim3(256), 0, s, a);
  else
    hipLaunchKernelGGL(wgrad_halo3_kernel<bf16_t>, dim3(blocks), dim3(256), 0, s, a);
}
```

### semi-supervised_semantic_segmentation_amd/ssseg/native.py

```python
import ctypes
import os
import re

import torch

_HERE = os.path.dirname(os.path.abspath(__file__))
LIB_PATH = os.environ.get('SSSEG_LIB_PATH') or os.path.join(_HERE, 'libssseg.so')
HEADER = os.path.join(_HERE, '..', '..', 'include', 'ssseg.h')

F32, BF16, F16, F64 = 0, 1, 2, 3
SSSEG_SUM, SSSEG_AVG = 0, 1
_ERRS = {-1: 'SSSEG_EINVAL', -2: 'SSSEG_EUNSUPPORTED', -3: 'SSSEG_EWORKSPACE', -4: 'SSSEG_ECOMM'}

vp, i64, i32, f32, f64, sz, u64 = (ctypes.c_void_p, ctypes.c_int64, ctypes.c_int, ctypes.c_float, ctypes.c_double,
                                   ctypes.c_size_t, ctypes.c_uint64)
I64P = ctypes.POINTER(ctypes.c_int64)

class CatPart(ctypes.Structure):
    _fields_ = [('src', vp), ('dst', vp), ('add', vp), ('ld', i64), ('c', i64)]


def cat_parts(rows):
    return (CatPart * len(rows))(*[CatPart(*r) for r in rows])


SIGS = {
    'ssseg_version': (ctypes.c_char_p, []),
    'ssseg_cowmix_workspace_bytes': (sz, [i64, i64, i64]),
    'ssseg_cowmix_mask': (i32, [vp, vp, vp, i64, i64, i64, vp, vp, vp, vp, sz, vp]),
    'ssseg_normal_f32': (i32, [vp, i64, u64, u64, vp]),
    'ssseg_mix': (i32, [vp, vp, vp, vp, i64, i64, i64, i32, vp]),
    'ssseg_cowmix_draw': (i32, [vp, vp, vp, i64, i64, f64, f64, f64, f64, u64, u64, vp]),
    'ssseg_cowmix_draw_dev': (i32, [vp, vp, vp, i64, i64, f64, f64, f64, f64, u64, vp, vp]),
    'ssseg_classmix_workspace_bytes': (sz, [i64, i64, i64]),
    'ssseg_classmix_mask': (i32, [vp, I64P, i32, vp, i64, i64, i64, i64, vp, vp, vp, vp, sz, vp]),
    'ssseg_cutmix_mask': (i32, [vp, i64, i64, i64, f64, f64, vp, vp, vp]),
    'ssseg_mixmask_draw_dev': (i32, [vp, vp, i64, i64, u64, vp, vp]),
    'ssseg_nchw_to_nhwc': (i32, [vp, vp, i64, i64, i64, i64, i64, i32, i32, vp]),
    'ssseg_nhwc_to_nchw': (i32, [vp, vp, i64, i64, i64, i64, i64, i32, i32, vp]),
    'ssseg_cast': (i32, [vp, vp, i64, i32, i32, vp]),
    'ssseg_bilinear_fwd': (i32, [vp, vp, i64, i64, i64, i64, i64, i64, I64P, I64P, i32, i32, vp]),
    'ssseg_bilinear_bwd': (i32, [vp, vp, i64, i64, i64, i64, i64, i64, I64P, I64P, i32, i32, vp]),
    'ssseg_bilinear_bwd_workspace_bytes': (sz, [i64, i64, i64, i64]),
    'ssseg_bilinear_bwd_ws': (i32, [vp, vp, i64, i64, i64, i64, i64, i64, I64P, I64P, i32, i32, vp, sz, vp]),
    'ssseg_aug_warp': (i32, [vp, vp, i64, i64, i64, i64, vp, vp, i64, i64, vp, vp, vp, i32, vp]),
    'ssseg_aug_color': (i32, [vp, i64, i64, i64, vp, vp]),
    'ssseg_aug_blur': (i32, [vp, vp, i64, i64, i64, i64, vp, vp, i64, i32, i32, vp]),
    'ssseg_aug_iso_finish': (i32, [vp, vp, i64, i64, i64, vp, vp, u64, vp]),
    'ssseg_aug_uniform_field': (i32, [vp, i64, u64, vp]),
    'ssseg_rotate_fwd': (i32, [vp, vp, i64, i64, i64, i64, f64, vp]),
    'ssseg_rotate_bwd': (i32, [vp, vp, i64, i64, i64, i64, f64, vp]),
    'ssseg_affine_warp_fwd': (i32, [vp, vp, vp, i64, i64, i64, i64, I64P, I64P, i32, vp, vp]),
    'ssseg_affine_warp_bwd': (i32, [vp, vp, vp, vp, i64, i64, i64, i64, I64P, I64P, i32, vp]),
    'ssseg_affine_draw_dev': (i32, [vp, vp, i64, i64, i64, f64, f64, f64, u64, vp, vp]),
    'ssseg_reduce_workspace_bytes': (sz, [i64]),
    'ssseg_bce_logits_fwd': (i32, [vp, vp, i64, vp, vp, sz, vp]),
    'ssseg_bce_logits_bwd': (i32, [vp, vp, i64, vp, vp, vp]),
    'ssseg_consistency_fwd': (i32, [vp, vp, i64, i64, i64, f32, vp, vp, sz, vp]),
    'ssseg_consistency_bwd': (i32, [vp, vp, i64, i64, i64, f32, vp, vp, vp, vp]),
    'ssseg_consistency_w_fwd': (i32, [vp, vp, vp, i64, i64, i64, f32, vp, vp, sz, vp]),
    'ssseg_consistency_w_bwd': (i32, [vp, vp, vp, i64, i64, i64, f32, vp, vp, vp, vp]),
    'ssseg_consistency_sm_fwd': (i32, [vp, vp, vp, i64, i64, i64, f32, vp, vp, sz, vp]),
    'ssseg_consistency_sm_bwd': (i32, [vp, vp, vp, i64, i64, i64, f32, vp, vp, vp, vp]),
    'ssseg_consistency_ce_workspace_bytes': (sz, [i64]),
    'ssseg_consistency_ce_fwd': (i32, [vp, vp, vp, i64, i64, i64, f32, i32, vp, vp, sz, vp]),
    'ssseg_consistency_ce_bwd': (i32, [vp, vp, vp, i64, i64, i64, f32, i32, vp, vp, vp, vp]),
    'ssseg_consistency_ce_cls_fwd': (i32, [vp, vp, vp, i64, i64, i64, vp, i32, vp, vp, sz, vp]),
    'ssseg_consistency_ce_cls_bwd': (i32, [vp, vp, vp, i64, i64, i64, vp, i32, vp, vp, vp, vp]),
    'ssseg_adaptive_thr_workspace_bytes': (sz, [i64]),
    'ssseg_adaptive_thr_update': (i32, [vp, i64, i64, i64, f64, vp, vp, vp, sz, vp]),
    'ssseg_lovasz_workspace_bytes': (sz, [i64, i64]),
    'ssseg_lovasz_fwd': (i32, [vp, vp, i64, i64, i64, vp, vp, sz, vp]),
    'ssseg_lovasz_bwd': (i32, [vp, vp, i64, i64, i64, vp, vp, vp, sz, vp]),
    'ssseg_lovasz_bwd_from_fwd': (i32, [vp, vp, i64, i64, i64, vp, vp, vp, sz, vp]),
    'ssseg_lovasz_sort_workspace_bytes': (sz, [i64, i64]),
    'ssseg_lovasz_sort': (i32, [vp, vp, vp, vp, i64, i64, vp, sz, vp]),
    'ssseg_lovasz_gen_workspace_bytes': (sz, [i64, i64, i64, i32, i64]),
    'ssseg_lovasz_gen_fwd': (i32, [vp, vp, i32, i64, i64, i64, i32, i32, i32, I64P, i64, i32, i64, vp, vp, sz, vp]),
    'ssseg_lovasz_gen_bwd': (i32, [vp, vp, i32, i64, i64, i64, i32, i32, i32, I64P, i64, i32, i64, vp, vp, vp, sz,
                                   vp]),
    'ssseg_lovasz_gen_bwd_from_fwd': (i32, [vp, vp, i32, i64, i64, i64, i32, i32, i32, I64P, i64, i32, i64, vp, vp,
                                            vp, sz, vp]),
    'ssseg_rmi_workspace_bytes': (sz, [i64] * 9),
    'ssseg_rmi_fwd': (i32, [vp, vp] + [i64] * 9 + [i32, vp, vp, sz, vp]),
    'ssseg_rmi_bwd': (i32, [vp] + [i64] * 9 + [vp, vp, vp, sz, vp]),
    'ssseg_segloss_workspace_bytes': (sz, [i32, i64, i64, i64]),
    'ssseg_ce_fwd': (i32, [vp, vp, i64, i64, i64, i32, vp, vp, sz, vp]),
    'ssseg_ce_bwd': (i32, [vp, vp, i64, i64, i64, i32, vp, vp, vp]),
    'ssseg_ohem_fwd': (i32, [vp, vp, i64, i64, i64, f32, i64, vp, vp, sz, vp]),
    'ssseg_ohem_bwd': (i32, [vp, vp, i64, i64, i64, vp, vp, vp, sz, vp]),
    'ssseg_ce_labels_fwd': (i32, [vp, vp, i32, i64, i64, i64, vp, i64, f32, i32, i32, vp, vp, sz, vp]),
    'ssseg_ce_labels_bwd': (i32, [vp, vp, i32, i64, i64, i64, vp, i64, f32, i32, vp, vp, vp, sz, vp]),
    'ssseg_ohem_labels_fwd': (i32, [vp, vp, i32, i64, i64, i64, i64, f32, i64, vp, vp, sz, vp]),
    'ssseg_ohem_labels_bwd': (i32, [vp, vp, i32, i64, i64, i64, vp, vp, vp, sz, vp]),
    'ssseg_focal_fwd': (i32, [vp, vp, i64, f64, f64, vp, vp, sz, vp]),
    'ssseg_focal_bwd': (i32, [vp, vp, i64, f64, f64, vp, vp, vp]),
    'ssseg_nfl_fwd': (i32, [vp, vp, i64, i64, i64, vp, vp, vp, vp, sz, vp]),
    'ssseg_nfl_bwd': (i32, [vp, vp, i64, i64, i64, vp, vp, vp, vp, sz, vp]),
    'ssseg_dice_logits_fwd': (i32, [vp, vp, i64, i64, i64, vp, vp, sz, vp]),
    'ssseg_dice_logits_bwd': (i32, [vp, vp, i64, i64, i64, vp, vp, vp, sz, vp]),
    'ssseg_dice_prob_fwd': (i32, [vp, vp, i64, i64, i32, f32, vp, vp, sz, vp]),
    'ssseg_dice_prob_bwd': (i32, [vp, i64, i64, i32, f32, vp, vp, vp, sz, vp]),
    'ssseg_binary_entropy_fwd': (i32, [vp, i64, vp, vp, sz, vp]),
    'ssseg_binary_entropy_bwd': (i32, [vp, i64, vp, vp, vp]),
    'ssseg_entropy_fwd': (i32, [vp, i64, i64, i64, vp, vp, sz, vp]),
    'ssseg_entropy_bwd': (i32, [vp, i64, i64, i64, vp, vp, vp]),
    'ssseg_bce_logits_red_fwd': (i32, [vp, vp, i64, i32, vp, vp, sz, vp]),
    'ssseg_bce_logits_red_bwd': (i32, [vp, vp, i64, i32, vp, vp, vp]),
    'ssseg_smooth_labels': (i32, [vp, vp, i64, f32, f32, vp]),
    'ssseg_uncertainty_workspace_bytes': (sz, [i64, i64, i64]),
    'ssseg_uncertainty_scores': (i32, [vp, i64, i64, i64, vp, vp, sz, vp]),
    'ssseg_kmeans_workspace_bytes': (sz, [i64, i64, i64]),
    'ssseg_kmeans_seed': (i32, [vp, i64, i64, i64, vp, vp, vp, vp, sz, vp]),
    'ssseg_kmeans_fit': (i32, [vp, i64, i64, i64, f64, i64, vp, vp, vp, vp, vp, sz, vp]),
    'ssseg_prob_onehot': (i32, [vp, i64, i64, vp, vp, vp]),
    'ssseg_seg_metrics': (i32, [vp, I64P, i64, i64, vp, I64P, i64, i64, i64, vp, vp, vp, vp]),
    'ssseg_seg_metrics_mc': (i32, [vp, I64P, i64, i64, vp, I64P, i32, i32, i64, i64, i64, i64, i64, vp, vp, vp, vp,
                                   vp]),
    'ssseg_prob_onehot_mc': (i32, [vp, i64, i64, i64, i32, vp, vp, vp]),
    'ssseg_ema_update': (i32, [vp, vp, i64, f64, vp]),
    'ssseg_scale_f32': (i32, [vp, i64, f32, vp]),
    'ssseg_axpby': (i32, [vp, f32, vp, f32, vp, i64, vp]),
    'ssseg_sigmoid_fwd': (i32, [vp, vp, i64, vp]),
    'ssseg_sigmoid_bwd': (i32, [vp, vp, vp, i64, vp]),
    'ssseg_sqnorm_accum': (i32, [vp, i64, vp, vp, sz, vp]),
    'ssseg_sgd_step': (i32, [vp, vp, vp, vp, i64, f32, f32, f32, f32, vp, i32, vp, vp]),
    'ssseg_optim_prepare': (i32, [vp, i32, f64, f64, f64, f64, f64, i64, f64, vp, vp, vp]),
    'ssseg_optim_step': (i32, [vp, vp, vp, vp, vp, vp, vp, i64, i32, i32, f64, f64, f64, f64, f64, f64, vp, vp]),
    'ssseg_amp_update': (i32, [vp, vp, f32, f32, i32, vp]),
    'ssseg_scale_by': (i32, [vp, vp, vp, i64, vp]),
    'ssseg_conv_igemm': (i32, [vp, vp, vp, vp, i32, i32, vp, i32, vp, sz, vp]),
    'ssseg_conv_igemm_phases': (i32, [vp, vp, vp, i32, i32, vp, i64, vp, vp, vp]),
    'ssseg_conv_igemm_phases_ws': (i32, [vp, vp, vp, i32, i32, vp, i64, vp, vp, vp, sz, vp]),
    'ssseg_conv_igemm_phases_workspace_bytes': (sz, [vp, i64, i32]),
    'ssseg_conv_stem_epi': (i32, [vp, vp, vp, vp, i32, vp, vp]),
    'ssseg_conv_igemm_epi': (i32, [vp, vp, vp, vp, i32, i32, vp, vp, sz, vp]),
    'ssseg_conv_igemm_epi_actmask': (i32, [vp, vp, vp, vp, i32, i32, vp, i32, f32, vp, sz, vp]),
    'ssseg_conv_igemm_epi_join': (i32, [vp, vp, vp, vp, i32, i32, vp, vp, i64, vp, sz, vp]),
    'ssseg_weight_pack_batch': (i32, [vp, i64, i32, vp]),
    'ssseg_param_step': (i32, [vp, vp, vp, vp, vp, i64, vp, f32, f32, f32, f32, vp, i32, vp, f64, i32, vp]),
    'ssseg_dwconv_fwd': (i32, [vp, vp, vp, vp, i32, vp, vp]),
    'ssseg_dwconv_dgrad': (i32, [vp, vp, vp, vp, i32, vp]),
    'ssseg_dwconv_wgrad_workspace_bytes': (sz, [vp, i32]),
    'ssseg_dwconv_wgrad': (i32, [vp, vp, vp, vp, i32, i64, i32, vp, sz, vp]),
    'ssseg_conv_igemm_workspace_bytes': (sz, [vp, i32]),
    'ssseg_set_knob': (i32, [i32, i32]),
    'ssseg_tune_table_export': (i64, [vp, vp, i64]),
    'ssseg_tune_table_import': (i32, [vp, vp, i64, i32]),
    'ssseg_conv_wgrad_workspace_bytes': (sz, [vp, i32]),
    'ssseg_conv_wgrad': (i32, [vp, vp, vp, vp, i32, i64, i64, i32, i32, vp, sz, vp]),
    'ssseg_conv_wgrad2_workspace_bytes': (sz, [vp, i64, i32]),
    'ssseg_conv_wgrad2': (i32, [vp, vp, vp, vp, i64, vp, vp, i32, i64, i64, i32, i32, vp, sz, vp]),
    'ssseg_conv_igemm_epi_vcat': (i32, [vp, vp, vp, vp, vp, i32, i32, vp, vp, sz, vp]),
    'ssseg_conv_igemm_epi_vsplit': (i32, [vp, vp, vp, vp, vp, i32, i32, vp, vp, sz, vp]),
    'ssseg_conv_wgrad_vcat': (i32, [vp, vp, vp, vp, vp, i32, i64, i64, i32, i32, vp, sz, vp]),
    'ssseg_conv_wgrad2_vcat': (i32, [vp, vp, vp, vp, vp, vp, i64, vp, vp, i32, i64, i64, i32, i32, vp, sz, vp]),
    'ssseg_weight_pack': (i32, [vp, vp, i64, i64, i64, i64, i64, i64, i32, i64, i64, i64, i64, i64, i64, i32, vp]),
    'ssseg_bn_workspace_bytes': (sz, [i64]),
    'ssseg_bn_stats': (i32, [vp, i64, i64, i64, i32, vp, vp, sz, vp]),
    'ssseg_bn_partials_finalize': (i32, [vp, i64, i64, vp, f64, f32, f32, vp, vp, vp, vp, vp, vp]),
    'ssseg_bn_gstat_finalize': (i32, [vp, i64, i64, vp, vp, vp, vp, vp, vp, vp, vp, vp]),
    'ssseg_bn_gstat_finalize_x': (i32, [vp, i64, i64, vp, vp, vp, vp, vp, i64, i64, i32, vp, vp, vp, vp, vp]),
    'ssseg_channel_sum_grad': (i32, [vp, i64, i64, i64, i32, vp, vp, vp, sz, vp]),
    'ssseg_bn_finalize': (i32, [vp, i64, f64, f32, f32, vp, vp, vp, vp, vp, vp]),
    'ssseg_bn_eval_params': (i32, [vp, vp, f32, i64, vp, vp, vp]),
    'ssseg_bn_fold': (i32, [vp, vp, vp, vp, vp, f32, i64, i64, vp, vp, vp, vp, vp]),
    'ssseg_bn_fold_batch': (i32, [vp, i64, vp]),
    'ssseg_bn_eval_bwd': (i32, [vp, vp, vp, vp, vp, i64, i64, i64, vp, vp, vp, i32, i32, vp, vp, sz, vp]),
    'ssseg_bn_eval_bwd_grad_y': (i32, [vp, vp, vp, vp, i64, i64, i64, vp, vp, vp, vp, i32, i32, vp, vp, sz, vp, vp, vp,
                                      vp]),
    'ssseg_bn_eval_bwd_grad': (i32, [vp, vp, vp, vp, vp, i64, i64, i64, vp, vp, vp, i32, i32, vp, vp, sz, vp, vp,
                                      vp, vp]),
    'ssseg_bn_eval_param_grad': (i32, [vp, i64, vp, vp, vp, vp, vp]),
    'ssseg_bn_eval_bwd_part': (i32, [vp, vp, vp, vp, vp, i64, i64, i64, vp, vp, vp, vp, i32, i32, vp, sz, I64P, vp]),
    'ssseg_bn_param_grad_batch': (i32, [vp, i64, i64, vp]),
    'ssseg_bn_apply': (i32, [vp, vp, vp, i64, i64, i64, i64, i64, vp, vp, vp, vp, i32, i32, vp]),
    'ssseg_bn_bwd_reduce': (i32, [vp, vp, vp, i64, i64, i64, i64, i64, vp, vp, vp, vp, i32, i32, vp, vp, sz, vp]),
    'ssseg_bn_param_grad': (i32, [vp, i64, vp, vp, vp]),
    'ssseg_bn_bwd_reduce_grad': (i32, [vp, vp, vp, i64, i64, i64, i64, i64, vp, vp, vp, vp, i32, i32, vp, vp, sz, vp,
                                        vp, vp]),
    'ssseg_bn_stats_finalize': (i32, [vp, i64, i64, i64, i32, vp, vp, sz, f64, f32, f32, vp, vp, vp, vp, vp, vp]),
    'ssseg_bn_bwd_apply': (i32, [vp, vp, vp, vp, vp, i64, i64, i64, i64, i64, i64, vp, vp, vp, vp, i32, i32, vp, f64,
                                 i32, vp]),
    'ssseg_maxpool_fwd': (i32, [vp, vp, vp, i64, i64, i64, i64, i64, i64, i64, i64, i64, i32, vp]),
    'ssseg_maxpool_bwd': (i32, [vp, vp, vp, i64, i64, i64, i64, i64, i64, i64, i64, i64, i32, vp]),
    'ssseg_maxpool_bwd_res': (i32, [vp, vp, vp, vp, i64, i64, i64, i64, i64, i64, i64, i64, i64, i32, vp]),
    'ssseg_nhwc_copy': (i32, [vp, vp, i64, i64, i64, i64, i64, i64, i64, i64, i64, i64, i64, i64, i64, i64, i32, vp]),
    'ssseg_zero': (i32, [vp, sz, vp]),
    'ssseg_nhwc_cat_n': (i32, [vp, i64, vp, i64, i64, i32, vp]),
    'ssseg_nhwc_split_n': (i32, [vp, i64, vp, i64, i64, i32, vp]),
    'ssseg_act_bwd': (i32, [vp, vp, vp, i64, i32, f32, i32, vp]),
    'ssseg_relu_bwd': (i32, [vp, vp, vp, i64, i32, vp]),
    'ssseg_avgpool_fwd': (i32, [vp, vp, i64, i64, i64, i64, i64, i64, i64, i64, i64, i32, vp]),
    'ssseg_avgpool_bwd': (i32, [vp, vp, i64, i64, i64, i64, i64, i64, i64, i64, i64, i32, vp]),
    'ssseg_global_avgpool_workspace_bytes': (sz, [i64, i64, i64]),
    'ssseg_global_avgpool_fwd': (i32, [vp, vp, i64, i64, i64, i64, i32, vp, sz, vp]),
    'ssseg_global_avgpool_bwd': (i32, [vp, vp, i64, i64, i64, i64, i32, vp]),
    'ssseg_add_n': (i32, [ctypes.POINTER(ctypes.c_void_p), i32, vp, i64, i32, f32, i32, vp]),
    'ssseg_dropout': (i32, [vp, vp, i64, f32, u64, u64, i32, vp]),
    'ssseg_dropout_dev': (i32, [vp, vp, i64, f32, u64, vp, i32, vp]),
    'ssseg_rng_take': (i32, [vp, vp, u64, vp]),
    'ssseg_att_blend_fwd': (i32, [vp, I64P, vp, I64P, vp, I64P, vp, i64, i64, i64, i64, vp]),
    'ssseg_att_blend_bwd': (i32, [vp, I64P, vp, I64P, vp, I64P, vp, I64P, vp, vp, vp, i64, i64, i64, i64, vp]),
    'ssseg_window_gather': (i32, [vp, I64P, i64, i64, i64, i64, vp, i64, vp, I64P, i64, i64, i32, vp]),
    'ssseg_window_accumulate': (i32, [vp, I64P, i64, i64, i64, i64, vp, vp, i64, i64, i32, i32, vp, vp, i64, i64, i64,
                                      vp]),
    'ssseg_window_merge': (i32, [vp, vp, i64, i64, i64, i64, i64, i64, vp, i64, i64, f32, i32, vp]),
    'ssseg_window_argmax': (i32, [vp, i64, i64, i64, vp, vp]),
    'ssseg_absmax_update': (i32, [vp, i64, i64, i64, i32, vp, vp]),
    'ssseg_quantize_i8': (i32, [vp, i64, i64, i64, i32, vp, vp, i64, vp]),
    'ssseg_weight_quant_i8': (i32, [vp, i64, i64, i64, i64, i64, i64, vp, vp, vp]),
    'ssseg_conv_i8_fwd': (i32, [vp, vp, vp, vp, i32, vp, vp, vp, vp]),
    'ssseg_comm_unique_id_bytes': (sz, []),
    'ssseg_comm_get_unique_id': (i32, [vp]),
    'ssseg_comm_init': (i32, [ctypes.POINTER(ctypes.c_void_p), vp, i32, i32, i32]),
    'ssseg_comm_destroy': (i32, [vp]),
    'ssseg_comm_async_error': (i32, [vp]),
    'ssseg_comm_last_error': (ctypes.c_char_p, []),
    'ssseg_allreduce_buckets': (i32, [vp, ctypes.POINTER(ctypes.c_void_p), I64P, i64, i32, i32, vp]),
    'ssseg_probe_event_create': (i32, [ctypes.POINTER(ctypes.c_void_p)]),
    'ssseg_probe_event_record': (i32, [vp, vp]),
    'ssseg_probe_event_elapsed': (i32, [vp, vp, ctypes.POINTER(ctypes.c_float)]),
    'ssseg_probe_event_destroy': (i32, [vp]),
}


class ConvDesc(ctypes.Structure):
    _fields_ = [(n, ctypes.c_int64) for n in (
        'N', 'H', 'W', 'C', 'ldx', 'OH', 'OW', 'K', 'R', 'S', 'sy', 'sx', 'dy', 'dx', 'py', 'px',
        'outH', 'outW', 'osy', 'osx', 'ooy', 'oox', 'ldy', 'ldw')]


class ConvEpilogue(ctypes.Structure):
    _fields_ = [('scale', ctypes.c_void_p), ('shift', ctypes.c_void_p), ('residual', ctypes.c_void_p),
                ('ldr', ctypes.c_int64), ('aux', ctypes.c_void_p), ('relu', ctypes.c_int32), ('slope', ctypes.c_float),
                ('stats', ctypes.c_void_p), ('stats_ld', ctypes.c_int64), ('stats_rows', ctypes.c_void_p)]


class NflParams(ctypes.Structure):
    _fields_ = [(n, ctypes.c_double) for n in ('alpha', 'gamma', 'eps', 'scale', 'weight', 'ignore_label')] + \
               [('from_logits', ctypes.c_int32), ('size_average', ctypes.c_int32)]


OPT_ADAM, OPT_ADAMOD, OPT_DIFFGRAD, OPT_DIFFMOD, OPT_RANGER = range(5)
OPT_STATE_DOUBLES = 8
RED_NONE, RED_MEAN, RED_SUM = 0, 1, 2
LOSS_REDUCE, LOSS_OHEM, LOSS_NFL, LOSS_DICE_LOGITS, LOSS_DICE_PROB = 0, 1, 2, 3, 4
LOSS_CE_LABELS, LOSS_OHEM_LABELS = 5, 6
LOVASZ_PROBAS, LOVASZ_SOFTMAX, LOVASZ_HINGE = 0, 1, 2
LOVASZ_LABEL_I64, LOVASZ_LABEL_U8, LOVASZ_LABEL_F32, LOVASZ_LABEL_DENSE = 0, 1, 2, 3


class VCat(ctypes.Structure):
    _fields_ = [('x2', ctypes.c_void_p), ('c1', ctypes.c_int64), ('ldx2', ctypes.c_int64)]


_lib = None


def header_symbols():
    with open(HEADER) as f:
        text = f.read()
    text = re.sub(r'/\*.*?\*/', '', text, flags=re.S)
    return sorted(set(re.findall(r'\b(ssseg_[a-z0-9_]+)\s*\(', text)))


def lib():
    global _lib
    if _lib is None:
        if not os.path.exists(LIB_PATH):
            raise RuntimeError(f'ssseg: native library not built ({LIB_PATH}); run __graft_entry__.build() '
                               'or make -C semi-supervised_semantic_segmentation_amd/csrc. There is no CPU fallback.')
        L = ctypes.CDLL(LIB_PATH)
        for name, (res, args) in SIGS.items():
            fn = getattr(L, name)
            fn.restype = res
            fn.argtypes = args
        _lib = L
        for kv in filter(None, os.environ.get('SSSEG_KNOBS', '').split(',')):
            k, v = kv.split('=')
            if L.ssseg_set_knob(int(k), int(v)) != 0:
                raise ValueError(f'SSSEG_KNOBS: bad knob {kv!r}')
    return _lib


def call(name, *args):
    rc = getattr(lib(), name)(*args)
    if rc != 0:
        raise RuntimeError(f'ssseg: {name} failed with {_ERRS.get(rc, "hipError " + str(rc))}')


EUNSUPPORTED = -2


def call_or_unsupported(name, *args):
    rc = getattr(lib(), name)(*args)
    if rc == EUNSUPPORTED:
        return False
    if rc != 0:
        raise RuntimeError(f'ssseg: {name} failed with {_ERRS.get(rc, "hipError " + str(rc))}')
    return True


def stream():
    return torch.cuda.current_stream().cuda_stream


def dev_ptr(t, name='tensor'):
    if t is None:
        return None
    if not t.is_cuda:
        raise RuntimeError(f'ssseg: {name} must be a HIP device tensor (no CPU fallback), got {t.device}')
    return t.data_ptr()


def dt_code(t):
    if t.dtype == torch.float32:
        return F32
    if t.dtype == torch.bfloat16:
        return BF16
    if t.dtype == torch.float16:
        return F16
    raise RuntimeError(f'ssseg: unsupported dtype {t.dtype}')


def workspace(nbytes, device):
    return torch.empty(max(int(nbytes), 16), dtype=torch.uint8, device=device)


def strides4(t):
    arr = (ctypes.c_int64 * 4)(*t.stride())
    return arr
```

### semi-supervised_semantic_segmentation_amd/ssseg/nn.py

```python
import contextlib
import ctypes
import os

import torch
import torch.distributed as dist
import torch.nn as nn

from . import comm as _comm
from . import native as N

_CFG = {'act_mask': os.environ.get('SSSEG_ACT_MASK', '1') != '0',
        'grad_join': True, 'stem': os.environ.get('SSSEG_STEM', '1') != '0', 'phases': True, 'eval_bwd_y': True, 'dtype': torch.bfloat16, 'sync_bn': True,
        'fuse_stats': True, 'vcat': os.environ.get('SSSEG_VCAT', '1') != '0',
        'vpad': os.environ.get('SSSEG_VPAD', '1') != '0',
        'bn_gstat': os.environ.get('SSSEG_BN_GSTAT', '1') != '0',
        'bn_join': os.environ.get('SSSEG_BN_JOIN', '1') != '0'}


_QUANT = [None]


def set_bn_grad_stats(on):
    _CFG['bn_gstat'] = bool(on)


def set_bn_join(on):
    _CFG['bn_join'] = bool(on)


def _bn_join_on():
    return _CFG['bn_join'] and _CFG['bn_gstat'] and _CFG['act_mask']


def set_virtual_concat(on):
    _CFG['vcat'] = bool(on)


def set_eval_bwd_from_y(on):
    _CFG['eval_bwd_y'] = bool(on)


def set_phase_launch(on):
    _CFG['phases'] = bool(on)


def set_stem_kernel(on):
    _CFG['stem'] = bool(on)


def set_grad_join(on):
    _CFG['grad_join'] = bool(on)


def set_compute_dtype(dtype):
    assert dtype in (torch.bfloat16, torch.float16, torch.float32)
    _CFG['dtype'] = dtype


def compute_dtype():
    return _CFG['dtype']


def set_sync_bn(flag):
    _CFG['sync_bn'] = bool(flag)


_WGRAD = {'merge': os.environ.get('SSSEG_WGRAD_MERGE', '1') != '0', 'defer': False, 'pending': []}


def set_wgrad_merge(on):
    _WGRAD['merge'] = bool(on)


@contextlib.contextmanager
def defer_wgrad():
    if not _WGRAD['merge']:
        yield
        return
    prev = _WGRAD['defer']
    _WGRAD['defer'] = True
    try:
        yield
    finally:
        _WGRAD['defer'] = prev


def flush_wgrad():
    pending, _WGRAD['pending'] = _WGRAD['pending'], []
    for mod in pending:
        pair = mod.__dict__.pop('_ssseg_wg_pending', None)
        if pair is not None:
            mod._ssseg_wgrad(*pair, bias_grad=False, want=(True, False))


_HOLD = {'on': False, 'tag': None, 'calls': [], 'params': False, 'adds': []}


@contextlib.contextmanager
def hold_wgrad(tag, params=False):
    prev = _HOLD['on'], _HOLD['tag'], _HOLD['params']
    _HOLD['on'], _HOLD['tag'], _HOLD['params'] = True, tag, params
    try:
        yield
    finally:
        _HOLD['on'], _HOLD['tag'], _HOLD['params'] = prev


def _grad_ptrs(*params):
    if not (_HOLD['on'] and _HOLD['params']):
        return tuple(N.dev_ptr(_grad_of(p)) if p is not None else None for p in params)
    out = []
    for p in params:
        if p is None:
            out.append(None)
            continue
        tmp = torch.zeros_like(_grad_of(p))
        _HOLD['adds'].append((p, tmp))
        out.append(N.dev_ptr(tmp))
    return tuple(out)


def clear_held():
    _HOLD['calls'] = []
    _HOLD['adds'] = []


def _held(mod, x, gy, bias_grad, want):
    if not _HOLD['on']:
        return False
    _HOLD['calls'].append((_HOLD['tag'], mod, (x, gy), {'bias_grad': bias_grad, 'want': want}))
    return True


def replay_held(order):
    calls, _HOLD['calls'] = _HOLD['calls'], []
    adds, _HOLD['adds'] = _HOLD['adds'], []
    cur = torch.cuda.current_stream()
    for _, tmp in adds:
        tmp.record_stream(cur)
    for _, _, args, kw in calls:
        for t in list(args) + list(kw.values()):
            if isinstance(t, torch.Tensor) and t.is_cuda:
                t.record_stream(cur)
    for p, tmp in adds:
        g = _grad_of(p)
        N.call('ssseg_axpby', N.dev_ptr(g), 1.0, N.dev_ptr(tmp), 1.0, N.dev_ptr(g), g.numel(), N.stream())
    with defer_wgrad():
        for tag, mod, args, kw in calls:
            if tag == order[0]:
                mod._ssseg_wgrad(*args, **kw)
    for tag, mod, args, kw in calls:
        if tag == order[1]:
            mod._ssseg_wgrad(*args, **kw)
    flush_wgrad()


_PGRAD = {'on': os.environ.get('SSSEG_DEFER_BN_PGRAD', '1') != '0', 'live': False, 'pending': [], 'table': None}


@contextlib.contextmanager
def defer_param_grads():
    if not _PGRAD['on'] or _PGRAD['live'] or not torch.cuda.is_available():
        yield
        return
    _PGRAD['live'] = True
    try:
        yield
    finally:
        _PGRAD['live'] = False
        flush_param_grads()


_GRAPH_REFS = {'live': None}


def _graph_ref(t):
    if _GRAPH_REFS['live'] is not None and torch.cuda.is_current_stream_capturing():
        _GRAPH_REFS['live'].append(t)
    return t


@contextlib.contextmanager
def graph_refs():
    prev, _GRAPH_REFS['live'] = _GRAPH_REFS['live'], []
    try:
        yield _GRAPH_REFS['live']
    finally:
        _GRAPH_REFS['live'] = prev


def flush_param_grads():
    import struct
    pend, _PGRAD['pending'] = _PGRAD['pending'], []
    if not pend:
        return
    rows = tuple((e['part'].data_ptr(), e['nparts'], e['C'], e['scale'].data_ptr(), e['dg'], e['db'], e['dbias'])
                 + (e.get('gs') or (0, 0, 0)) for e in pend)
    ent = _PGRAD['table']
    if ent is None or ent[0] != rows:
        if torch.cuda.is_current_stream_capturing():
            for e in pend:
                sums = torch.empty(2 * e['C'], dtype=torch.float64, device=e['part'].device)
                if e.get('gs'):
                    N.call('ssseg_bn_gstat_finalize', N.dev_ptr(e['part']), e['nparts'], e['C'], N.dev_ptr(sums),
                           N.dev_ptr(e['scale']), *e['gs'], e['dg'] or None, e['db'] or None, e['dbias'] or None,
                           N.stream())
                    continue
                N.call('ssseg_bn_partials_finalize', N.dev_ptr(e['part']), e['nparts'], e['C'], N.dev_ptr(sums), 0.0,
                       0.0, 0.0, None, None, None, None, None, N.stream())
                N.call('ssseg_bn_eval_param_grad', N.dev_ptr(sums), e['C'], N.dev_ptr(e['scale']), e['dg'] or None,
                       e['db'] or None, e['dbias'] or None, N.stream())
            return
        blob = b''.join(struct.pack('<10q', *r) for r in rows)
        ent = (rows, torch.frombuffer(bytearray(blob), dtype=torch.uint8).to(pend[0]['part'].device))
        _PGRAD['table'] = ent
    N.call('ssseg_bn_param_grad_batch', N.dev_ptr(_graph_ref(ent[1])), len(rows), max(e['C'] for e in pend),
           N.stream())


def wgrad_pending():
    return sum(1 for m in _WGRAD['pending'] if '_ssseg_wg_pending' in m.__dict__)


def set_fused_bn_stats(flag):
    _CFG['fuse_stats'] = bool(flag)


def vec(dtype=None):
    return 4 if (dtype or _CFG['dtype']) == torch.float32 else 8


def rup(c, v):
    return (c + v - 1) // v * v


def set_virtual_pad(on):
    _CFG['vpad'] = bool(on)


def vpad(c):
    if not _CFG['vpad'] or _CFG['dtype'] == torch.float32 or c % 64 == 0:
        return c
    p = rup(c, 64)
    return p if (p - c) * 8 <= c else c


def _zero_(t):
    N.call('ssseg_zero', N.dev_ptr(t), t.numel() * t.element_size(), N.stream())
    return t


def new_act(n, c, h, w, dtype, device, zero=False):
    t = torch.empty((n, c, h, w), dtype=dtype, device=device, memory_format=torch.channels_last)
    return _zero_(t) if zero else t


def _is_act(x, c_phys=None):
    return (x.is_cuda and x.dim() == 4 and (c_phys is None or x.shape[1] == c_phys)
            and x.dtype == _CFG['dtype'] and x.is_contiguous(memory_format=torch.channels_last))


def _need_act(x, c_phys, what):
    if not _is_act(x, c_phys):
        raise RuntimeError(f'ssseg: {what} expects a {_CFG["dtype"]} channels_last HIP activation with {c_phys} '
                           f'channels, got {tuple(x.shape)} {x.dtype} {x.device} strides {x.stride()}')


_PROBE = {'on': False, 'rows': [], 'fenced': os.environ.get('SSSEG_PROBE_FENCED', '0') == '1'}


class ProbeEvent:
    __slots__ = ('ev',)

    def __init__(self):
        h = ctypes.c_void_p()
        N.call('ssseg_probe_event_create', ctypes.byref(h))
        self.ev = h.value

    def record(self):
        N.call('ssseg_probe_event_record', self.ev, N.stream())

    def elapsed_time(self, end):
        ms = ctypes.c_float()
        N.call('ssseg_probe_event_elapsed', self.ev, end.ev, ctypes.byref(ms))
        return ms.value

    def __del__(self):
        if self.ev and N._lib is not None:
            N._lib.ssseg_probe_event_destroy(self.ev)
            self.ev = None


def _probe_event():
    return torch.cuda.Event(enable_timing=True) if _PROBE['fenced'] else ProbeEvent()


def probe(enable):
    _PROBE['on'] = bool(enable)
    if enable:
        _PROBE['rows'] = []
    return _PROBE['rows']


class _Timed:
    def __init__(self, flops, kind, tag=''):
        self.flops, self.kind, self.tag = flops, kind, tag
# ... 449 lines not shown
        return not (self._ssseg_dw or self._ssseg_head)

    def _fwd_desc(self, n, H, W):
        cin, cout = self._dims()
        (R, S), (sh, sw), (ph, pw), (dh, dw) = self.kernel_size, self.stride, self.padding, self.dilation
        OH, OW = self._out_hw(H, W)
        ce = vpad(cin) if self._vpad_ok() else cin
        return _desc(N=n, H=H, W=W, C=ce, ldx=cin, OH=OH, OW=OW, K=cout, R=R, S=S, sy=sh, sx=sw, dy=dh, dx=dw,
                     py=-ph, px=-pw, outH=OH, outW=OW, osy=1, osx=1, ooy=0, oox=0, ldy=cout, ldw=R * S * ce)

    def _ssseg_res_dgrad(self):
        return not self._ssseg_dw

    def forward(self, x, handoff=None, stats=None):
        if not _is_act(x):
            x = to_act(x)
        return _ConvFn.apply(x, self.weight, self.bias, self, False, handoff, stats, _join_fwd(x))

    def stat_rows_cap(self, n, H, W):
        if self._ssseg_dw or self._ssseg_head:
            return None
        OH, OW = self._out_hw(H, W)
        return (n * OH * OW + 63) // 64

    def forward_relu(self, x):
        return self.forward_act(x, True)

    def forward_act(self, x, act, single_use=False):
        if not _is_act(x):
            x = to_act(x)
        y = _ConvFn.apply(x, self.weight, self.bias, self, act, None, None, _join_fwd(x))
        code, slope = _act(act)
        if single_use and code in (ACT_RELU, ACT_LEAKY) and torch.is_grad_enabled() and y.requires_grad:
            y.__dict__['_ssseg_act_out'] = (code, slope)
        return y

    def _dw_desc(self, n, H, W):
        d = self._fwd_desc(n, H, W)
        d.ldw = d.C
        return d

    def _dw_pack(self):
        cin = self._dims()[0]
        R, S = self.kernel_size
        return self._pack('dw', 1, 1, self.in_channels, cin, 1, 0, 1, R, 0, 1, S)

    def _dw_forward(self, x, relu, bn, residual, keep_pre, aux_copy=True):
        cin, cout = self._dims()
        n, _, H, W = x.shape
        d = self._dw_desc(n, H, W)
        y = new_act(n, cout, d.OH, d.OW, _CFG['dtype'], x.device)
        aux = bwd = None
        if bn is not None:
            _need_res(residual, y)
            aux = torch.empty_like(y) if keep_pre and aux_copy else None
            fold, bwd = self._fold(bn, residual, cout, aux)
        else:
            fold = (None, self.bias, None, None)
        scale, shift, res, aux_t = fold
        code, slope = _act(relu)
        ep = N.ConvEpilogue(N.dev_ptr(scale) if scale is not None else None,
                            N.dev_ptr(shift.detach() if shift is not None else None) if shift is not None else None,
                            N.dev_ptr(res) if res is not None else None, res.shape[1] if res is not None else 0,
                            N.dev_ptr(aux_t) if aux_t is not None else None, code, slope)
        R, S = self.kernel_size
        with _Timed(2.0 * n * d.OH * d.OW * self.in_channels * R * S, 'fwd', _tag(self, n, H, W)):
            N.call('ssseg_dwconv_fwd', N.dev_ptr(x), N.dev_ptr(self._dw_pack()), N.dev_ptr(y), ctypes_ref(d),
                   N.dt_code(x), ctypes_ref(ep), N.stream())
        return (y, aux, bwd) if keep_pre else y

    def _ssseg_forward(self, x, relu, bn=None, residual=None, keep_pre=False, stats=None, aux_copy=True):
        cin, cout = self._dims()
        _need_act(x, cin, 'Conv2d')
        if _QUANT[0] is not None and not keep_pre and stats is None and not torch.is_grad_enabled():
            y = _QUANT[0](self, x, relu, bn, residual)
            if y is not None:
                return y
        if self._ssseg_dw:
            if stats is not None:
                raise NotImplementedError('ssseg: fused BN statistics on a depthwise conv')
            return self._dw_forward(x, relu, bn, residual, keep_pre, aux_copy)
        n, _, H, W = x.shape
        d = self._fwd_desc(n, H, W)
        R, S = self.kernel_size
        stem = self._stem_ok(cout, d.OW)
        if stem:
            w = self._pack('stem', cout, self.out_channels, self.in_channels, 4, 0, 0, 1, R, 0, 1, S)
        else:
            w = self._pack('fwd', cout, self.out_channels, self.in_channels, d.C, 0, 0, 1, R, 0, 1, S)
        fl = _conv_flops(n, d.OH, d.OW, self.out_channels, self.in_channels, R, S)
        tg = _tag(self, n, H, W)
        if bn is not None:
            y = new_act(n, cout, d.OH, d.OW, _CFG['dtype'], x.device)
            _need_res(residual, y)
            aux = torch.empty_like(y) if keep_pre and aux_copy else None
            fold, bwd = self._fold(bn, residual, cout, aux)
            with _Timed(fl, 'fwd', tg):
                self._igemm(x, w, y, d, N.dt_code(y), relu=relu, fold=fold, stem=stem)
            return (y, aux, bwd) if keep_pre else y
        if self._ssseg_head:
            y = torch.empty((n, cout, d.OH, d.OW), dtype=torch.float32, device=x.device,
                            memory_format=torch.channels_last)
            with _Timed(fl, 'fwd', tg):
                self._igemm(x, w, y, d, N.F32, self.bias, relu)
            return y[:, :self.out_channels]
        y = new_act(n, cout, d.OH, d.OW, _CFG['dtype'], x.device)
        with _Timed(fl, 'fwd', tg):
            self._igemm(x, w, y, d, N.dt_code(y), self.bias, relu, stats=stats, stem=stem)
        return y

    def _stem_ok(self, cout, ow=None):
        R, S = self.kernel_size
        return (_CFG['stem'] and not self._ssseg_head and not self._ssseg_dw and self.in_channels <= 4
                and R in (3, 7) and S <= 8 and self.dilation == (1, 1) and self.stride[1] <= 2 and cout % 16 == 0
                and _CFG['dtype'] in (torch.bfloat16, torch.float16) and ow is not None and ow % 128 == 0)

    def _grad_in(self, gy):
        cin, cout = self._dims()
        if self._ssseg_head:
            n, c, h, w = gy.shape
            g = new_act(n, cout, h, w, _CFG['dtype'], gy.device)
            gc = gy if gy.is_contiguous() else gy.contiguous()
            N.call('ssseg_nchw_to_nhwc', N.dev_ptr(gc), N.dev_ptr(g), n, c, h, w, cout, N.dt_code(gc), N.dt_code(g),
                   N.stream())
            return g
        _need_act(gy, cout, 'Conv2d backward')
        return gy

    def _ssseg_wgrad(self, x, gy, bias_grad=True, want=None):
        if _held(self, x, gy, bias_grad, want):
            return
        ww = self.weight.requires_grad if want is None else want[0]
        if bias_grad:
            _bias_grad(self, gy, None if want is None else want[1])
        if not ww:
            if self.bias is not None and (self.bias.requires_grad if want is None else want[1]):
                _ready(self.bias)
            return
        n, _, H, W = x.shape
        if self._ssseg_dw:
            d = self._dw_desc(n, H, W)
            nb = N.lib().ssseg_dwconv_wgrad_workspace_bytes(ctypes_ref(d), N.dt_code(x))
            ws = N.workspace(nb, x.device)
            R, S = self.kernel_size
            with _Timed(2.0 * n * d.OH * d.OW * self.in_channels * R * S, 'wgrad', _tag(self, n, H, W)):
                N.call('ssseg_dwconv_wgrad', N.dev_ptr(x), N.dev_ptr(gy), N.dev_ptr(_grad_of(self.weight)),
                       ctypes_ref(d), N.dt_code(x), self.in_channels, 1, N.dev_ptr(ws), nb, N.stream())
            _ready(*[p for p in (self.weight, self.bias) if p is not None])
            return
        if self._wg_defer(x, gy):
            return
        self._wgrad_launch(x, gy, self._wg_take(x, gy))

    def _wgrad_launch(self, x, gy, pend):
        n, _, H, W = x.shape
        R, S = self.kernel_size
        if pend is None:
            d = self._fwd_desc(n, H, W)
            nb = N.lib().ssseg_conv_wgrad_workspace_bytes(ctypes_ref(d), N.dt_code(x))
            ws = N.workspace(nb, x.device)
            vc = _vcat_of(x)
            with _Timed(_conv_flops(n, d.OH, d.OW, self.out_channels, self.in_channels, R, S), 'wgrad',
                        _tag(self, n, H, W)):
                if not (vc is not None and vc.ready(d) and N.call_or_unsupported(
                        'ssseg_conv_wgrad_vcat', N.dev_ptr(vc.a), ctypes_ref(vc.desc2()), N.dev_ptr(gy),
                        N.dev_ptr(_grad_of(self.weight)), ctypes_ref(vc.desc_for(d)), N.dt_code(x), self.in_channels,
                        self.out_channels, 1, 1, N.dev_ptr(ws), nb, N.stream())):
                    if vc is not None:
                        materialize(x)
                    N.call('ssseg_conv_wgrad', N.dev_ptr(x), N.dev_ptr(gy), N.dev_ptr(_grad_of(self.weight)),
                           ctypes_ref(d), N.dt_code(x), self.in_channels, self.out_channels, 1, 1, N.dev_ptr(ws), nb,
                           N.stream())
        else:
            x1, gy1 = pend
            n1 = x1.shape[0]
            d = self._fwd_desc(n1, H, W)
            nb = N.lib().ssseg_conv_wgrad2_workspace_bytes(ctypes_ref(d), n, N.dt_code(x))
            ws = N.workspace(nb, x.device)
            v1, v2 = _vcat_of(x1), _vcat_of(x)
            with _Timed(_conv_flops(n1 + n, d.OH, d.OW, self.out_channels, self.in_channels, R, S), 'wgrad',
                        _tag(self, n1 + n, H, W)):
                both = v1 is not None and v2 is not None and v1.same_split(v2) and v1.ready(d)
                if not (both and N.call_or_unsupported(
                        'ssseg_conv_wgrad2_vcat', N.dev_ptr(v1.a), ctypes_ref(v1.desc2()), N.dev_ptr(gy1),
                        N.dev_ptr(v2.a), ctypes_ref(v2.desc2()), N.dev_ptr(gy), n, N.dev_ptr(_grad_of(self.weight)),
                        ctypes_ref(v1.desc_for(d)), N.dt_code(x), self.in_channels, self.out_channels, 1, 1,
                        N.dev_ptr(ws), nb, N.stream())):
                    for t in (x1, x):
                        if _vcat_of(t) is not None:
                            materialize(t)
                    N.call('ssseg_conv_wgrad2', N.dev_ptr(x1), N.dev_ptr(gy1), N.dev_ptr(x), N.dev_ptr(gy), n,
                           N.dev_ptr(_grad_of(self.weight)), ctypes_ref(d), N.dt_code(x), self.in_channels,
                           self.out_channels, 1, 1, N.dev_ptr(ws), nb, N.stream())
        if self.bias is not None:
            _ready(self.weight, self.bias)
        else:
            _ready(self.weight)

    def _ssseg_mask_dgrad_ok(self):
        return not self._ssseg_dw and _CFG['dtype'] in (torch.bfloat16, torch.float16, torch.float32)

    def _ssseg_gstat_ok(self):
        (R, S), (sh, sw) = self.kernel_size, self.stride
        return (sh == 1 and sw == 1) or (R >= sh and S >= sw and sh * sw <= 4 and self.dilation in (1, (1, 1)))

    def _ssseg_join_dgrad_ok(self):
        return self._ssseg_mask_dgrad_ok() and self.stride == (1, 1)

    def _ssseg_dgrad(self, gy, xshape, residual=None, mask=None, stats=None, scale=None, join=None):
        if join is not None and (residual is None or mask is not None or stats is not None or scale is not None
                                 or self.stride != (1, 1)):
            raise ValueError('ssseg.nn.Conv2d: the residual-join input gradient needs the pending gradient and stride 1')
        if (stats is not None or scale is not None) and (mask is None or residual is not None):
            raise ValueError('ssseg.nn.Conv2d: gradient statistics / scale need the masked input gradient')
        fold = (None, None, residual, None) if residual is not None else (
            (scale, None, None, None) if scale is not None else None)
        cin, cout = self._dims()
        n, _, H, W = xshape
        (R, S), (sh, sw), (ph, pw), (dh, dw) = self.kernel_size, self.stride, self.padding, self.dilation
        OH, OW = gy.shape[2], gy.shape[3]
        dx = new_act(n, cin, H, W, _CFG['dtype'], gy.device)
        if residual is not None:
            _need_res(residual, dx)
            if self._ssseg_dw:
                raise NotImplementedError('ssseg.nn.Conv2d: fused input-gradient accumulation needs a dense conv')
        if self._ssseg_dw:
            d = self._dw_desc(n, H, W)
            with _Timed(2.0 * n * OH * OW * self.in_channels * R * S, 'dgrad', _tag(self, n, H, W)):
                N.call('ssseg_dwconv_dgrad', N.dev_ptr(gy), N.dev_ptr(self._dw_pack()), N.dev_ptr(dx), ctypes_ref(d),
                       N.dt_code(gy), N.stream())
            return dx
        timer = _Timed(_conv_flops(n, OH, OW, self.out_channels, self.in_channels, R, S), 'dgrad', _tag(self, n, H, W))
        ce = vpad(cout) if self._vpad_ok() else cout
        if sh == 1 and sw == 1:
            w = self._pack('dgrad', cin, self.in_channels, self.out_channels, ce, 1, R - 1, -1, R, S - 1, -1, S)
            d = _desc(N=n, H=OH, W=OW, C=ce, ldx=cout, OH=H, OW=W, K=cin, R=R, S=S, sy=1, sx=1, dy=dh, dx=dw,
                      py=ph - (R - 1) * dh, px=pw - (S - 1) * dw, outH=H, outW=W, osy=1, osx=1, ooy=0, oox=0,
                      ldy=cin, ldw=R * S * ce)
            with timer:
                if join is not None:
                    if self._igemm(gy, w, dx, d, N.dt_code(dx), fold=fold, join=join):
                        dx.__dict__['_ssseg_premasked'] = True
                    else:
                        self._igemm(gy, w, dx, d, N.dt_code(dx), fold=fold)
                else:
                    self._igemm(gy, w, dx, d, N.dt_code(dx), fold=fold, mask=mask, stats=stats)
            return dx
        timer.__enter__()
        for (phy, ry0, rny, dly, qy) in _phases(sh, ph, R, H, dh):
            for (phx, rx0, rnx, dlx, qx) in _phases(sw, pw, S, W, dw):
                if qy == 0 or qx == 0:
                    continue
                rr, ss = (rny, rnx) if rny * rnx > 0 else (0, 0)
                w = self._pack(('dgrad', phy, phx), cin, self.in_channels, self.out_channels, ce, 1, ry0, sh,
                               rny, rx0, sw, rnx) if rr else None
                d = _desc(N=n, H=OH, W=OW, C=ce, ldx=cout, OH=qy, OW=qx, K=cin, R=rr, S=ss, sy=1, sx=1, dy=-1,
                          dx=-1, py=dly, px=dlx, outH=H, outW=W, osy=sh, osx=sw, ooy=phy, oox=phx, ldy=cin,
                          ldw=max(rr * ss * ce, ce))
                self._igemm(gy, w, dx, d, N.dt_code(dx), fold=fold, mask=mask, stats=stats)
        timer.__exit__()
        return dx


    def _ssseg_dgrad_vsplit(self, gy, xshape, vc):
        cin, cout = self._dims()
        n, cp, H, W = xshape
        if (self._ssseg_dw or self.stride != (1, 1) or cp != vc.ca + vc.cb or cin != cp
                or _CFG['dtype'] not in (torch.bfloat16, torch.float16)):
            return None
        (R, S), (ph, pw), (dh, dw) = self.kernel_size, self.padding, self.dilation
        OH, OW = gy.shape[2], gy.shape[3]
        da = new_act(n, vc.ca, H, W, _CFG['dtype'], gy.device)
        db = new_act(n, vc.cb, H, W, _CFG['dtype'], gy.device)
        w = self._pack('dgrad', cin, self.in_channels, self.out_channels, cout, 1, R - 1, -1, R, S - 1, -1, S)
        d = _desc(N=n, H=OH, W=OW, C=cout, ldx=cout, OH=H, OW=W, K=cin, R=R, S=S, sy=1, sx=1, dy=dh, dx=dw,
                  py=ph - (R - 1) * dh, px=pw - (S - 1) * dw, outH=H, outW=W, osy=1, osx=1, ooy=0, oox=0,
                  ldy=vc.ca, ldw=R * S * cout)
        dref = ctypes_ref(d)
        nb = N.lib().ssseg_conv_igemm_workspace_bytes(dref, N.dt_code(gy))
        ws = N.workspace(nb, gy.device) if nb else None
        mask = vc.a if vc.mask_a else None
        ep = N.ConvEpilogue(None, None, N.dev_ptr(mask) if mask is not None else None, vc.ca if mask is not None else 0,
                            None, 0, 0.0, None, 0, None)
        split = N.VCat(N.dev_ptr(db), vc.ca, vc.cb)
        with _Timed(_conv_flops(n, OH, OW, self.out_channels, self.in_channels, R, S), 'dgrad', _tag(self, n, H, W)):
            ok = N.call_or_unsupported('ssseg_conv_igemm_epi_vsplit', N.dev_ptr(gy), N.dev_ptr(w), N.dev_ptr(da),
                                       ctypes_ref(split), dref, N.dt_code(gy), N.dt_code(gy), ctypes_ref(ep),
                                       N.dev_ptr(ws) if ws is not None else None, nb, N.stream())
        if not ok:
            return None
        if mask is not None:
            da.__dict__['_ssseg_premasked'] = True
        return da, db


class ConvTranspose2d(nn.ConvTranspose2d, _ConvBase):

    def __init__(self, *args, **kw):
        super().__init__(*args, **kw)
        if self.groups != 1 or self.dilation != (1, 1) or self.output_padding != (0, 0):
            raise NotImplementedError('ssseg.nn.ConvTranspose2d: groups/dilation/output_padding not implemented')
        self._ssseg_init(False)
        self._fuse_relu = False

    def _dims(self):
        v = vec()
        return rup(self.in_channels, v), rup(self.out_channels, v)

    def forward(self, x, output_size=None, stats=None):
        if output_size is not None:
            raise NotImplementedError('ssseg.nn.ConvTranspose2d: output_size')
        if not _is_act(x):
            x = to_act(x)
        return _ConvFn.apply(x, self.weight, self.bias, self, self._fuse_relu, None, stats, _join_fwd(x))

    def stat_rows_cap(self, n, H, W):
        (R, S), (sh, sw), (ph, pw) = self.kernel_size, self.stride, self.padding
        OH, OW = self._out_hw(H, W)
        rows = 0
        for (_, _, rny, _, qy) in _phases(sh, ph, R, OH):
            for (_, _, rnx, _, qx) in _phases(sw, pw, S, OW):
                if qy == 0 or qx == 0:
                    continue
                if rny * rnx == 0:
                    return None
                rows += (n * qy * qx + 63) // 64
        return rows

    def forward_relu(self, x):
        return self.forward_act(x, True)

    def forward_act(self, x, act):
# ... 981 lines not shown
```

### semi-supervised_semantic_segmentation_amd/train.py

```python
import contextlib
import os
import time

import torch

import cowmix
import mean_teacher
import metrics
import mixmasks
import utils.utils as utils
from ssseg import nn as snn
from ssseg import ops
from ssseg import param_step
from ssseg import sliding
from ssseg.ddp import DistributedDataParallel as _DDP
from ssseg.optim import SGD as _SGD, FusedOptimizer as _Fused


def _inner(model):
    return model.module if hasattr(model, 'module') else model


def _batched_eval_ok(ema_model, a, b):
    m = _inner(ema_model)
# ... 120 lines not shown
        raise ValueError("consistency_loss 'ce' is defined over mutually exclusive classes: it needs "
                         "consistency_activation 'softmax'")
    return kind, weighting


def _confidence_threshold_mode(tc):
    mode = tc.get('confidence_threshold_mode', 'fixed')
    if mode == 'fixed':
        return mode, None
    if mode != 'adaptive':
        raise ValueError(f"confidence_threshold_mode must be 'fixed' or 'adaptive', got {mode!r}")
    if _consistency_loss_kind(tc)[0] != 'ce':
        raise ValueError("confidence_threshold_mode 'adaptive' is defined for consistency_loss 'ce' (the squared-"
                         "difference forms keep the scalar confidence_threshold)")
    momentum = tc.get('confidence_threshold_momentum', 0.999)
    if not isinstance(momentum, (int, float)) or not 0.0 <= momentum < 1.0:
        raise ValueError(f'confidence_threshold_momentum must be a number in [0, 1), got {momentum!r}')
    return mode, float(momentum)


def _adaptive_threshold(tc):
    mode, momentum = _confidence_threshold_mode(tc)
    if mode == 'fixed':
        return None
    sat = tc.get('confidence_threshold_state')
    if sat is None:
        sat = tc['confidence_threshold_state'] = ops.AdaptiveThreshold(momentum)
    sat.momentum = momentum
    return sat


def _threshold_key(tc):
    sat = _adaptive_threshold(tc)
    return _confidence_threshold_mode(tc) + (id(sat) if sat is not None else None,)


def _consistency_forward(model, targets, tc, epoch):
    mixed_ema_pred, mixed_images = targets
    aug = _consistency_augmentation(tc)
    view = aug.apply([mixed_images])[0] if aug is not None else mixed_images
    model.eval()
    with snn.folded(_inner(model)):
        student_pred = model(view)[-1][-1]
    model.train()
    student_pred = ops.interpolate_bilinear(student_pred, mixed_images.shape[2:4], align_corners=False)
    activation = _consistency_activation(tc)
    if aug is not None:
        student_pred = aug.reverse([student_pred])[0]
    loss_kind, weighting = _consistency_loss_kind(tc)
    if loss_kind == 'ce':
        sat = _adaptive_threshold(tc)
        thr = sat.update(mixed_ema_pred) if sat is not None else tc['confidence_threshold']
        consistency, cm_mean = ops.consistency_loss_ce(student_pred, mixed_ema_pred, thr,
                                                       aug.valid if aug is not None else None, weighting)
    elif activation == 'softmax':
        consistency, cm_mean = ops.consistency_loss_softmax(student_pred, mixed_ema_pred, tc['confidence_threshold'],
                                                            aug.valid if aug is not None else None)
    elif aug is not None:
        consistency, cm_mean = ops.consistency_loss_weighted(student_pred, mixed_ema_pred, aug.valid,
                                                             tc['confidence_threshold'])
    else:
        consistency, cm_mean = ops.consistency_loss(student_pred, mixed_ema_pred, tc['confidence_threshold'])
    return ops.scale(consistency, float(tc['consistency_loss_weight']) * float(epoch > 25)), cm_mean


def _side_stream(device):
    s = _OVERLAP['streams'].get(device)
    if s is None:
        s = _OVERLAP['streams'][device] = torch.cuda.Stream(device=device)
    return s


def train_step(model, ema_model, optimizer, image, mask, unsup_a, unsup_b, epoch, step, config):
    tc = config['train']
    ddp = model if isinstance(model, _DDP) else None
    semi = tc['use_semi_supervised']
    adv = tc.get('adversarial')
    if semi:
        mixmasks.mix_mask_kind(tc)
        _consistency_loss_kind(tc)
        _confidence_threshold_mode(tc)
    if mask.dim() == 3:
        if adv is not None:
            raise ValueError('train_step: the adversarial branch feeds the mask to the discriminator and needs a '
                             f'[B, C, H, W] mask, got a label map {tuple(mask.shape)}')
        if tc.get('device_augment') is not None:
            raise NotImplementedError('train_step: device augmentation resamples a float [B, C, H, W] mask; a label '
                                      f'map {tuple(mask.shape)} is not covered')
    features, pred_maps = model(image)
    classification_loss = tc['loss'](pred_maps, mask)
    sup_loss = classification_loss
    prob = None
    if adv is not None:
        adv_loss, prob = adversarial_terms(pred_maps, mask, adv)
        sup_loss = ops.add_scaled(sup_loss, adv_loss)
    key = _step_key(model, ema_model, image, unsup_a)
    seen = _OVERLAP['seen'].get(key, 0)
    overlap = (semi and _OVERLAP['teacher'] and image.is_cuda and unsup_a.is_cuda
               and seen >= _OVERLAP['serial_steps'])
    _OVERLAP['seen'][key] = seen + 1
    _OVERLAP['steps'] += 1
    targets = cons = None
    side_bwd = overlap and ddp is None and _OVERLAP['consistency'] and _OVERLAP['consistency_bwd']
    pgrad_ctx = contextlib.ExitStack()
    with pgrad_ctx:
        if overlap:
            main = torch.cuda.current_stream()
            side = _side_stream(image.device)
            side.wait_stream(main)
            for t in (unsup_a, unsup_b):
                t.record_stream(side)
            with torch.cuda.stream(side):
                targets = _teacher_targets(ema_model, unsup_a, unsup_b, tc)
                if _OVERLAP['consistency']:
                    cons = _consistency_forward(model, targets, tc, epoch)
                if side_bwd:
                    snn.clear_held()
                    pgrad_ctx.enter_context(snn.defer_param_grads())
                    with snn.hold_wgrad('cons', params=True):
                        ops.backward(_scaled(cons[0], optimizer))
            for t in targets:
                t.record_stream(main)
        if ddp is not None and not semi:
            ddp.arm()
        with snn.hold_wgrad('sup') if side_bwd else snn.defer_wgrad() if semi else contextlib.nullcontext():
            vbm = tc['virtual_batch_size_multiplier']
            ops.backward(_scaled(ops.scale(sup_loss, 1.0 / vbm) if vbm != 1 else sup_loss, optimizer))
        del pred_maps, features
        if adv is not None:
            _set_requires_grad(adv['discriminator'], True)
            adv['last_loss_d'] = discriminator_step(mask, prob, adv)
            adv['last_loss_adv'] = adv_loss.detach()
            del prob
        unsup_loss = cm_mean = None
        if side_bwd:
            torch.cuda.current_stream().wait_stream(_side_stream(image.device))
            unsup_loss, cm_mean = cons
            del targets, cons
            snn.replay_held(('sup', 'cons'))
            pgrad_ctx.close()
            semi_rest = False
        else:
            semi_rest = semi
    if semi_rest:
        if overlap:
            torch.cuda.current_stream().wait_stream(_side_stream(image.device))
        else:
            targets = _teacher_targets(ema_model, unsup_a, unsup_b, tc)
        side_fwd = cons is not None
        unsup_loss, cm_mean = cons if side_fwd else _consistency_forward(model, targets, tc, epoch)
        del targets, cons
        if ddp is not None:
            ddp.arm()
        with snn.defer_param_grads():
            if side_fwd:
                side = _side_stream(image.device)
                side.wait_stream(torch.cuda.current_stream())
            ops.backward(_scaled(unsup_loss, optimizer))
            if side_fwd:
                torch.cuda.current_stream().wait_stream(side)
    snn.flush_wgrad()
    if ddp is not None:
        ddp.finish()
    plan = param_step.plan_for(_inner(model), _inner(ema_model), optimizer) if semi else None
    if step % tc['virtual_batch_size_multiplier'] == 0 and step != 0:
        clip = tc['gradient_clip_value']
        if plan is not None:
            optimizer.step(max_norm=clip, fused=(plan, _inner(ema_model)._ssseg_arena, tc['ema_model_alpha']))
        elif isinstance(optimizer, (_SGD, _Fused)):
            optimizer.step(max_norm=clip)
        else:
            torch.nn.utils.clip_grad_norm_(_inner(model).parameters(), clip)
            optimizer.step()
        optimizer.zero_grad()
        if plan is None:
            snn.invalidate_packed(_inner(model))
    elif plan is not None:
        param_step.step(plan, optimizer, _inner(ema_model)._ssseg_arena, 0.0, tc['ema_model_alpha'], sgd=False)
    if semi:
        mean_teacher.update_ema_variables(model, ema_model, alpha=tc['ema_model_alpha'], averaged=plan is not None)
    return classification_loss.detach(), (unsup_loss.detach() if unsup_loss is not None else None), \
        (cm_mean.detach() if cm_mean is not None else None)


_GRAPH = {'on': os.environ.get('SSSEG_TRAIN_GRAPH', '1') != '0', 'cache': {}, 'eager_steps': 2, 'max_graphs': 2,
          'captures': 0, 'replays': 0}


_TUNE = {'steps': 0}


def _optimizers(optimizer, config):
    adv = config['train'].get('adversarial')
    return [optimizer] + ([adv['optimizer']] if adv is not None else [])


def _graph_key(model, ema_model, optimizer, image, mask, unsup_a, unsup_b, epoch, step, config):
    tc = config['train']
    if not (_GRAPH['on'] and image.is_cuda and torch.cuda.is_available()):
        return None
    if tc['use_semi_supervised'] and cowmix.NOISE_SOURCE != 'device':
        return None
    kind = mixmasks.mix_mask_kind(tc) if tc['use_semi_supervised'] else 'cowmix'
    if not mixmasks.capturable(kind):
        return None
    aug = _consistency_augmentation(tc) if tc['use_semi_supervised'] else None
    if aug is not None and (aug.source != 'device' or aug.fixed is not None):
        return None
    if torch.distributed.is_initialized() and (_world() > 1 or getattr(model, '_active', False)):
        from ssseg import comm as scomm
        if scomm.kind() != 'native':
            return None
    opts = _optimizers(optimizer, config)
    opt_step = step % tc['virtual_batch_size_multiplier'] == 0 and step != 0
    if (opt_step and getattr(optimizer, '_first', False)) or any(getattr(o, '_first', False) for o in opts[1:]):
        return None
    step_key = _step_key(model, ema_model, image, unsup_a)
    if _OVERLAP['seen'].get(step_key, 0) < _GRAPH['eager_steps']:
        return None
    lrs = tuple(float(g['lr']) for o in opts for g in o.param_groups)
    shapes = tuple((tuple(t.shape), t.dtype) if t is not None else None for t in (image, mask, unsup_a, unsup_b))
    sat = _adaptive_threshold(tc) if tc['use_semi_supervised'] else None
    if sat is not None and sat.state is None:
        return None
    thr_key = _threshold_key(tc) if tc['use_semi_supervised'] else ('fixed', None, None)
    return step_key + (id(optimizer), opt_step, float(epoch > 25), lrs, shapes, id(config),
                       _consistency_activation(tc), kind) + _consistency_loss_kind(tc) + thr_key


def _graph_step(key, model, ema_model, optimizer, image, mask, unsup_a, unsup_b, epoch, step, config):
    from ssseg.graph import StepGraph
    g = _GRAPH['cache'].pop(key, None)
    if g is None:
        while len(_GRAPH['cache']) >= _GRAPH['max_graphs']:
            _GRAPH['cache'].pop(next(iter(_GRAPH['cache'])))
        ins = (image, mask, unsup_a, unsup_b)
        live = [i for i, t in enumerate(ins) if t is not None]

        def fn(*xs):
            full = [None] * 4
            for i, t in zip(live, xs):
                full[i] = t
            out = train_step(model, ema_model, optimizer, *full, epoch, step, config)
            return tuple(t for t in out if t is not None)
        g = StepGraph(fn, *[ins[i] for i in live])
        g.live = live
        _GRAPH['captures'] += 1
    _GRAPH['cache'][key] = g
    ins = (image, mask, unsup_a, unsup_b)
    outs = iter(t.clone() for t in g(*[ins[i] for i in g.live]))
    _GRAPH['replays'] += 1
    semi = config['train']['use_semi_supervised']
    cls = next(outs)
    unsup = next(outs) if semi else None
    cm = next(outs) if semi else None
    return cls, unsup, cm


def run_step(model, ema_model, optimizer, image, mask, unsup_a, unsup_b, epoch, step, config):
    if _world() > 1 and image.is_cuda:
        from ssseg import tune
        _TUNE['steps'] += 1
        if not tune.synced() and _TUNE['steps'] > _GRAPH['eager_steps']:
            tune.sync()
    key = _graph_key(model, ema_model, optimizer, image, mask, unsup_a, unsup_b, epoch, step, config)
    if key is None:
        return train_step(model, ema_model, optimizer, image, mask, unsup_a, unsup_b, epoch, step, config)
    return _graph_step(key, model, ema_model, optimizer, image, mask, unsup_a, unsup_b, epoch, step, config)


def release_graphs():
    _GRAPH['cache'].clear()


def _reduce_meters(meters, keys, world):
    if world < 2:
        return
    live = [k for k in keys if meters[k].initialized]
    if not live:
        return
    dev = next((meters[k].sum.device for k in live if isinstance(meters[k].sum, torch.Tensor)), None)
    sums = torch.stack([torch.as_tensor(meters[k].sum, dtype=torch.float32, device=dev).reshape(()) for k in live])
    torch.distributed.all_reduce(sums)
    sums = sums / world
    for i, k in enumerate(live):
        meters[k].sum = sums[i]


def train(model, ema_model, optimizer, dataloader, unsupervised_dataloader, epoch, initial_step, summary_writer,
          config, device):
    model.train()
    meters = {k: utils.AverageMeter() for k in ('cls', 'sup', 'unsup', 'cm', 'time')}
    rank = torch.distributed.get_rank() if torch.distributed.is_initialized() else 0
    world = _world()
    optimizer.zero_grad()
    tc = config['train']
    aug = tc.get('device_augment')
    for step, sample in enumerate(dataloader):
        tic = time.time()
        global_step = initial_step + step
        if aug is not None:
            sample = aug.train_batch(sample)
        image = sample['image'].to(device, non_blocking=True)
        mask = sample['semantic_mask'].to(device, non_blocking=True)
        ua = ub = None
        if tc['use_semi_supervised']:
            us = [next(unsupervised_dataloader) for _ in range(2)]
# ... 89 lines not shown
```

Measured before the change: 533.6 images/sec.

## Batch same-shape conv weight-gradient kernels into grouped launches

Result: no change. 537.2 images/sec (median of 4 runs) (+0.7%).

```diff
diff --git a/include/ssseg.h b/include/ssseg.h
--- a/include/ssseg.h
+++ b/include/ssseg.h
@@ -360,6 +360,21 @@
 int ssseg_conv_wgrad2(const void* x, const void* dy, const void* x2, const void* dy2, int64_t n2, float* dw,
                       const ssseg_conv_desc* desc_host, int dt, int64_t c_real, int64_t k_real, int layout,
                       int accumulate, void* ws, size_t ws_bytes, ssseg_stream_t stream);
+
+#define SSSEG_WGRAD_GROUP_MAX 8
+typedef struct {
+  const void* x1;
+  const void* dy1;
+  const void* x2;
+  const void* dy2;
+  float* dw;
+} ssseg_wgrad_member;
+size_t ssseg_conv_wgrad_group_workspace_bytes(const ssseg_conv_desc* desc_host, int64_t n2, int dt, int count);
+int ssseg_conv_wgrad_group(const ssseg_wgrad_member* members, int count, int64_t n2, const ssseg_conv_desc* desc_host,
+                           int dt, int64_t c_real, int64_t k_real, int layout, int accumulate, void* ws, size_t ws_bytes,
+                           ssseg_stream_t stream);
+int ssseg_conv_wgrad_group_pays(const ssseg_conv_desc* desc_host, int64_t n2, int dt);
+int ssseg_conv_wgrad_group_max(const ssseg_conv_desc* desc_host, int64_t n2, int dt);
 
 int ssseg_conv_wgrad_vcat(const void* x, const ssseg_vcat* vc, const void* dy, float* dw,
                           const ssseg_conv_desc* desc_host, int dt, int64_t c_real, int64_t k_real, int layout,
diff --git a/semi-supervised_semantic_segmentation_amd/csrc/conv_kernels.h b/semi-supervised_semantic_segmentation_amd/csrc/conv_kernels.h
--- a/semi-supervised_semantic_segmentation_amd/csrc/conv_kernels.h
+++ b/semi-supervised_semantic_segmentation_amd/csrc/conv_kernels.h
@@ -1398,10 +1398,17 @@
   int ncb, nkb, nstrips, splits, s1;
   long long steps[2], sps[2];
 };
+struct WGroupTab {
+  ssseg_wgrad_member m[SSSEG_WGRAD_GROUP_MAX];
+  int n;
+  int per;
+  long long slab_stride;
+};
 bool halo3_eligible(const ConvGeom& g, int dt);
-HaloPlan halo3_plan(const ConvGeom& g, long long n1, long long n2);
-size_t halo3_ws_bytes(const ConvGeom& g, long long n1, long long n2);
+HaloPlan halo3_plan(const ConvGeom& g, long long n1, long long n2, int group = 1);
+size_t halo3_ws_bytes(const ConvGeom& g, long long n1, long long n2, int group = 1);
 void launch_wgrad_halo3(int dt, const HaloArgs& a, hipStream_t s);
+void launch_wgrad_halo3_group(int dt, const HaloArgs& a, const WGroupTab& tab, hipStream_t s);
 
 template <typename T, typename TO>
 int dispatch_regstaged(const void* x, const void* w, void* y, const ConvGeom& g, const Epi<TO>& ep, float* ws,
diff --git a/semi-supervised_semantic_segmentation_amd/csrc/conv_wgrad.hip b/semi-supervised_semantic_segmentation_amd/csrc/conv_wgrad.hip
--- a/semi-supervised_semantic_segmentation_amd/csrc/conv_wgrad.hip
+++ b/semi-supervised_semantic_segmentation_amd/csrc/conv_wgrad.hip
@@ -266,11 +266,11 @@
   unsigned xabytes, xbbytes;
 };
 
-template <typename T16, int BMW, int BNW, int NS, int WM = 2, int WN = 2, int BKP = 64, bool ST = false, bool GK = false>
-__global__ void __launch_bounds__(WM * WN * 64) wgrad_glds_kernel(const T16* __restrict__ x, const T16* __restrict__ dy,
-                                                                   float* __restrict__ slab, ConvGeom g,
-                                                                   long long pix_per_split, WDirect dd, unsigned xbytes,
-                                                                   unsigned dbytes, WSeg2 sg) {
+template <typename T16, int BMW, int BNW, int NS, int WM, int WN, int BKP, bool ST, bool GK>
+__device__ __forceinline__ void wgrad_glds_body(const T16* __restrict__ x, const T16* __restrict__ dy,
+                                                float* __restrict__ slab, const ConvGeom& g, long long pix_per_split,
+                                                const WDirect& dd, unsigned xbytes, unsigned dbytes, const WSeg2& sg,
+                                                int tile) {
   constexpr int NW = WM * WN, NT = NW * 64;
   constexpr int ROWX = BMW * 2, ROWD = BNW * 2;
   constexpr int XCPR = ROWX / 16, DCPR = ROWD / 16;
@@ -284,7 +284,6 @@
   const int t = threadIdx.x, lane = t & 63, wave = __builtin_amdgcn_readfirstlane(t >> 6);
   const int wm = wave / WN, wn = wave % WN;
   const int mt = (g.KK + BMW - 1) / BMW, nt = (g.K + BNW - 1) / BNW;
-  const int tile = xcd_tile(blockIdx.x, gridDim.x);
   const int split = tile / (mt * nt), rem = tile - split * (mt * nt);
   const int kk0 = (rem % mt) * BMW, co0 = (rem / mt) * BNW;
   const bool seg2 = sg.s1 > 0 && split >= sg.s1;
@@ -444,10 +443,35 @@
   wgrad_store<FM, FN>(acc, kk0 + wm * WTM, co0 + wn * WTN, lane, g, slab, dd, split);
 }
 
+template <typename T16, int BMW, int BNW, int NS, int WM = 2, int WN = 2, int BKP = 64, bool ST = false, bool GK = false>
+__global__ void __launch_bounds__(WM * WN * 64) wgrad_glds_kernel(const T16* __restrict__ x, const T16* __restrict__ dy,
+                                                                   float* __restrict__ slab, ConvGeom g,
+                                                                   long long pix_per_split, WDirect dd, unsigned xbytes,
+                                                                   unsigned dbytes, WSeg2 sg) {
+  wgrad_glds_body<T16, BMW, BNW, NS, WM, WN, BKP, ST, GK>(x, dy, slab, g, pix_per_split, dd, xbytes, dbytes, sg,
+                                                           xcd_tile(blockIdx.x, gridDim.x));
+}
+
+template <typename T16, int BMW, int BNW, int NS, int WM = 2, int WN = 2, int BKP = 64, bool GK = false>
+__global__ void __launch_bounds__(WM * WN * 64) wgrad_glds_group_kernel(WGroupTab tab, ConvGeom g,
+                                                                         long long pix_per_split, WDirect dd,
+                                                                         unsigned xbytes, unsigned dbytes, WSeg2 sg,
+                                                                         float* __restrict__ slab) {
+  const int id = xcd_tile(blockIdx.x, gridDim.x);
+  const int mi = id / tab.per;
+  const ssseg_wgrad_member& m = tab.m[mi];
+  sg.x = m.x2;
+  sg.dy = m.dy2;
+  if (dd.dw) dd.dw = m.dw;
+  wgrad_glds_body<T16, BMW, BNW, NS, WM, WN, BKP, false, GK>((const T16*)m.x1, (const T16*)m.dy1,
+                                                             slab + (long long)mi * tab.slab_stride, g, pix_per_split,
+                                                             dd, xbytes, dbytes, sg, id - mi * tab.per);
+}
+
 template <int V>
-__global__ void __launch_bounds__(1024) wgrad_reduce_wide_kernel(const float* __restrict__ slab, int splits, int K, int R,
-                                                            int S, int C, int c_real, int k_real,
-                                                            float* __restrict__ dst, int layout, int accumulate) {
+__device__ __forceinline__ void wgrad_reduce_wide_body(const float* __restrict__ slab, int splits, int K, int R, int S,
+                                                       int C, int c_real, int k_real, float* __restrict__ dst,
+                                                       int layout, int accumulate) {
   typedef float vec_t __attribute__((ext_vector_type(V)));
   __shared__ vec_t red[16][64];
   const long long KK = (long long)R * S * C;
@@ -484,8 +508,16 @@
   }
 }
 
-__global__ void wgrad_reduce_kernel(const float* __restrict__ slab, int splits, int K, int R, int S, int C, int c_real,
-                                    int k_real, float* __restrict__ dst, int layout, int accumulate) {
+template <int V>
+__global__ void __launch_bounds__(1024) wgrad_reduce_wide_kernel(const float* __restrict__ slab, int splits, int K, int R,
+                                                            int S, int C, int c_real, int k_real,
+                                                            float* __restrict__ dst, int layout, int accumulate) {
+  wgrad_reduce_wide_body<V>(slab, splits, K, R, S, C, c_real, k_real, dst, layout, accumulate);
+}
+
+__device__ __forceinline__ void wgrad_reduce_body(const float* __restrict__ slab, int splits, int K, int R, int S, int C,
+                                                  int c_real, int k_real, float* __restrict__ dst, int layout,
+                                                  int accumulate) {
   const long long KK = (long long)R * S * C;
   const long long total = (long long)K * KK;
   for (long long i = (long long)blockIdx.x * blockDim.x + threadIdx.x; i < total; i += (long long)gridDim.x * blockDim.x) {
@@ -507,6 +539,23 @@
     else o = (((long long)k * c_real + c) * R + r) * S + s;
     dst[o] = accumulate ? dst[o] + sum : sum;
   }
+}
+
+__global__ void wgrad_reduce_kernel(const float* __restrict__ slab, int splits, int K, int R, int S, int C, int c_real,
+                                    int k_real, float* __restrict__ dst, int layout, int accumulate) {
+  wgrad_reduce_body(slab, splits, K, R, S, C, c_real, k_real, dst, layout, accumulate);
+}
+
+template <int V>
+__global__ void __launch_bounds__(V ? 1024 : 256) wgrad_reduce_group_kernel(WGroupTab tab, const float* __restrict__ slab,
+                                                                          int splits, int K, int R, int S, int C,
+                                                                          int c_real, int k_real, int layout,
+                                                                          int accumulate) {
+  const int mi = blockIdx.y;
+  const float* sl = slab + (long long)mi * tab.slab_stride;
+  float* dst = tab.m[mi].dw;
+  if constexpr (V == 0) wgrad_reduce_body(sl, splits, K, R, S, C, c_real, k_real, dst, layout, accumulate);
+  else wgrad_reduce_wide_body<V>(sl, splits, K, R, S, C, c_real, k_real, dst, layout, accumulate);
 }
 
 namespace {
@@ -549,7 +598,8 @@
 constexpr int N_WGRAD_CFGS = (int)(sizeof(WGRAD_CFGS) / sizeof(WGRAD_CFGS[0]));
 
 template <typename T>
-WgradPlan plan_wgrad(const ConvGeom& g, int bmw = 0, long long slots = 0, int bnw = 0, int bkp_ = 0, int pct = 100) {
+WgradPlan plan_wgrad(const ConvGeom& g, int bmw = 0, long long slots = 0, int bnw = 0, int bkp_ = 0, int pct = 100,
+                     int group = 1) {
   WgradPlan p;
   p.glds = false;
   p.cfg = 0;
@@ -557,7 +607,7 @@
   p.bmw = bmw ? bmw : (g.KK <= 64 ? 64 : 128);
   p.mt = (g.KK + p.bmw - 1) / p.bmw;
   p.nt = (g.K + p.bnw - 1) / p.bnw;
-  const long long tiles = (long long)p.mt * p.nt;
+  const long long tiles = (long long)p.mt * p.nt * group;
   const int bkp = bkp_ ? bkp_ : WG<T>::BKP;
   const long long max_splits_by_work = std::max<long long>(1, g.M / (bkp * 8));
   long long want = std::max<long long>(1, (1024 + tiles - 1) / tiles);
@@ -566,12 +616,16 @@
     want = std::max<long long>(1, rounds * slots / tiles);
   }
   if (pct != 100) want = std::max<long long>(1, want * pct / 100);
+  if (group > 1) want = std::max<long long>(want, 4);
   if (g_knobs[10] != 100 && g_knobs[10] > 0) want = std::max<long long>(1, want * g_knobs[10] / 100);
-  const long long slab_cap = std::max<long long>(1, (64ll << 20) / (4ll * g.K * g.KK + 1));
+  const long long slab_cap = std::max<long long>(1, (64ll << 20) / (4ll * g.K * g.KK * group + 1));
   long long sp = std::min(std::min(want, max_splits_by_work), slab_cap);
   sp = std::max<long long>(1, std::min<long long>(sp, 65535));
+  const WgradPlan alone = group > 1 ? plan_wgrad<T>(g, bmw, slots, bnw, bkp_, pct, 1) : WgradPlan{};
+  if (group > 1) sp = std::max<long long>(sp, (alone.splits + 1) / 2);
   p.pps = (g.M + sp - 1) / sp;
   p.pps = (p.pps + bkp - 1) / bkp * bkp;
+  if (group > 1) p.pps = std::min(p.pps, 2 * alone.pps);
   p.splits = (int)((g.M + p.pps - 1) / p.pps);
   if (p.splits < 1) p.splits = 1;
   return p;
@@ -618,9 +672,9 @@
   return c;
 }
 
-static WgradPlan plan_for_cfg(const ConvGeom& g, int c) {
+static WgradPlan plan_for_cfg(const ConvGeom& g, int c, int group = 1) {
   const WgradCfg& wc = WGRAD_CFGS[c];
-  WgradPlan p = plan_wgrad<bf16_t>(g, wc.bmw, wgrad_slots(c), wc.bnw, wc.bkp, wc.pct);
+  WgradPlan p = plan_wgrad<bf16_t>(g, wc.bmw, wgrad_slots(c), wc.bnw, wc.bkp, wc.pct, group);
   p.glds = true;
   p.cfg = c;
   return p;
@@ -705,6 +759,37 @@
   launch_wgrad_glds_dispatch<T16, 1>(x, dy, slab, g, p, dd, s, sg);
 }
 
+template <typename T16, int C>
+void launch_wgrad_group_t(const WGroupTab& tab, float* slab, const ConvGeom& g, const WgradPlan& p, WDirect dd,
+                          hipStream_t s, const WSeg2& sg) {
+  constexpr WgradCfg wc = WGRAD_CFGS[C];
+  const unsigned xb = (unsigned)((long long)g.N * g.H * g.W * g.ldx * 2), db = (unsigned)(g.M * g.ldy * 2);
+  const dim3 grid((unsigned)(tab.per * tab.n)), block(wc.wm * wc.wn * 64);
+  if constexpr (wc.bmw == 64) {
+    if (g.C % 64) {
+      hipLaunchKernelGGL((wgrad_glds_group_kernel<T16, wc.bmw, wc.bnw, wc.ns, wc.wm, wc.wn, wc.bkp, true>), grid, block,
+                         0, s, tab, g, p.pps, dd, xb, db, sg, slab);
+      return;
+    }
+  }
+  hipLaunchKernelGGL((wgrad_glds_group_kernel<T16, wc.bmw, wc.bnw, wc.ns, wc.wm, wc.wn, wc.bkp, false>), grid, block, 0,
+                     s, tab, g, p.pps, dd, xb, db, sg, slab);
+}
+
+template <typename T16>
+bool launch_wgrad_group(const WGroupTab& tab, float* slab, const ConvGeom& g, const WgradPlan& p, WDirect dd,
+                        hipStream_t s, const WSeg2& sg) {
+  switch (p.cfg) {
+    case 1: launch_wgrad_group_t<T16, 1>(tab, slab, g, p, dd, s, sg); return true;
+    case 18: launch_wgrad_group_t<T16, 18>(tab, slab, g, p, dd, s, sg); return true;
+    case 19: launch_wgrad_group_t<T16, 19>(tab, slab, g, p, dd, s, sg); return true;
+    case 20: launch_wgrad_group_t<T16, 20>(tab, slab, g, p, dd, s, sg); return true;
+    default: return false;
+  }
+}
+
+bool wgrad_group_cfg_ok(int cfg) { return cfg == 1 || cfg == 18 || cfg == 19 || cfg == 20; }
+
 
 bool wg_geom_ok(const ConvGeom& g, int dt) {
   const int vec = dt == SSSEG_F32 ? 4 : 8;
@@ -736,10 +821,34 @@
 
 namespace {
 
+int reduce_width(const float* slab, const ConvGeom& g, int splits) {
+  if (splits < 64) return 0;
+  return ((long long)g.K * g.KK >= 32768 && g.C % 4 == 0 && ((uintptr_t)slab & 15) == 0) ? 4 : 1;
+}
+
+bool launch_reduce_group(const WGroupTab& tab, const float* slab, const ConvGeom& g, int splits, int64_t c_real,
+                         int64_t k_real, int layout, int accumulate, hipStream_t s) {
+  const long long total = (long long)g.K * g.KK;
+  const int v = reduce_width(slab, g, splits);
+  for (int i = 1; i < tab.n; ++i)
+    if (reduce_width(slab + i * tab.slab_stride, g, splits) != v) return false;
+  const unsigned ny = (unsigned)tab.n;
+  if (v == 4)
+    hipLaunchKernelGGL(wgrad_reduce_group_kernel<4>, dim3((unsigned)((total + 255) / 256), ny), dim3(1024), 0, s, tab,
+                       slab, splits, g.K, g.R, g.S, g.C, (int)c_real, (int)k_real, layout, accumulate);
+  else if (v == 1)
+    hipLaunchKernelGGL(wgrad_reduce_group_kernel<1>, dim3((unsigned)((total + 63) / 64), ny), dim3(1024), 0, s, tab, slab,
+                       splits, g.K, g.R, g.S, g.C, (int)c_real, (int)k_real, layout, accumulate);
+  else
+    hipLaunchKernelGGL(wgrad_reduce_group_kernel<0>, dim3(ssseg_grid(total, 256), ny), dim3(256), 0, s, tab, slab, splits,
+                       g.K, g.R, g.S, g.C, (int)c_real, (int)k_real, layout, accumulate);
+  return true;
+}
+
 void launch_reduce(const float* slab, const ConvGeom& g, int splits, int64_t c_real, int64_t k_real, float* dw,
                    int layout, int accumulate, hipStream_t s) {
   const long long total = (long long)g.K * g.KK;
-  if (splits >= 64 && total >= 32768 && g.C % 4 == 0 && ((uintptr_t)slab & 15) == 0)
+  if (reduce_width(slab, g, splits) == 4)
     hipLaunchKernelGGL(wgrad_reduce_wide_kernel<4>, dim3((unsigned)((total + 255) / 256)), dim3(1024), 0, s, slab,
                        splits, g.K, g.R, g.S, g.C, (int)c_real, (int)k_real, dw, layout, accumulate);
   else if (splits >= 64)
@@ -757,17 +866,15 @@
          (long long)g.N * g.H * g.W * vc->ldx2 * 2 < 0x7fffffffLL;
 }
 
-void run_halo3(const ConvGeom& g, int dt, const void* x, const ssseg_vcat* vc, const void* dy, const void* x2,
-               const ssseg_vcat* vc2, const void* dy2, long long n2, float* dw, int64_t c_real, int64_t k_real,
-               int layout, int accumulate, float* slab, hipStream_t s) {
-  const HaloPlan p = halo3_plan(g, g.N, n2);
+HaloArgs halo_args(const ConvGeom& g, const HaloPlan& p, const ssseg_vcat* vc, long long n2, int64_t c_real,
+                   int64_t k_real, int layout, int accumulate) {
   HaloArgs a{};
   const long long pix1 = (long long)g.N * g.H * g.W, pix2 = n2 * g.H * g.W;
-  a.seg[0] = HaloSeg{x, vc ? vc->x2 : nullptr, dy, (unsigned)(pix1 * g.ldx * 2),
+  a.seg[0] = HaloSeg{nullptr, nullptr, nullptr, (unsigned)(pix1 * g.ldx * 2),
                      vc ? (unsigned)(pix1 * vc->ldx2 * 2) : 0u, (unsigned)(pix1 * g.ldy * 2)};
   if (n2 > 0)
-    a.seg[1] = HaloSeg{x2, vc2 ? vc2->x2 : nullptr, dy2, (unsigned)(pix2 * g.ldx * 2),
-                       vc2 ? (unsigned)(pix2 * vc2->ldx2 * 2) : 0u, (unsigned)(pix2 * g.ldy * 2)};
+    a.seg[1] = HaloSeg{nullptr, nullptr, nullptr, (unsigned)(pix2 * g.ldx * 2),
+                       vc ? (unsigned)(pix2 * vc->ldx2 * 2) : 0u, (unsigned)(pix2 * g.ldy * 2)};
   a.H = g.H;
   a.W = g.W;
   a.C = g.C;
@@ -785,12 +892,28 @@
   a.sps[1] = p.sps[1];
   a.splits = p.splits;
   a.s1 = p.s1;
-  a.slab = slab;
-  a.dw = p.splits == 1 ? dw : nullptr;
   a.c_real = (int)c_real;
   a.k_real = (int)k_real;
   a.layout = layout;
   a.accumulate = accumulate;
+  return a;
+}
+
+void run_halo3(const ConvGeom& g, int dt, const void* x, const ssseg_vcat* vc, const void* dy, const void* x2,
+               const ssseg_vcat* vc2, const void* dy2, long long n2, float* dw, int64_t c_real, int64_t k_real,
+               int layout, int accumulate, float* slab, hipStream_t s) {
+  const HaloPlan p = halo3_plan(g, g.N, n2);
+  HaloArgs a = halo_args(g, p, vc, n2, c_real, k_real, layout, accumulate);
+  a.seg[0].x = x;
+  a.seg[0].x2 = vc ? vc->x2 : nullptr;
+  a.seg[0].dy = dy;
+  if (n2 > 0) {
+    a.seg[1].x = x2;
+    a.seg[1].x2 = vc2 ? vc2->x2 : nullptr;
+    a.seg[1].dy = dy2;
+  }
+  a.slab = slab;
+  a.dw = p.splits == 1 ? dw : nullptr;
   launch_wgrad_halo3(dt, a, s);
   if (p.splits > 1) launch_reduce(slab, g, p.splits, c_real, k_real, dw, layout, accumulate, s);
 }
@@ -851,7 +974,7 @@
 }
 
 bool merged_plan(const ConvGeom& g1, int64_t n2, int dt, WgradPlan& p, int& s1, ConvGeom& g2, int c1 = 0,
-                 bool allow_st = true) {
+                 bool allow_st = true, int group = 1) {
   if (n2 < 1 || n2 > 0x7fffffff || !wgrad_glds_ok(g1, dt)) return false;
   g2 = g1;
   g2.N = (int)n2;
@@ -860,13 +983,19 @@
   ConvGeom gm = g1;
   gm.M = g1.M + g2.M;
   bool st = false;
-  p = plan_for_cfg(gm, wgrad_cfg_for(g1, c1, allow_st ? &st : nullptr));
+  p = plan_for_cfg(gm, wgrad_cfg_for(g1, c1, allow_st ? &st : nullptr), group);
   p.st = st;
   const int bkp = WGRAD_CFGS[p.cfg].bkp;
   const long long sp = std::max(2, p.splits);
   long long a = std::min(sp - 1, std::max(1LL, (long long)((double)sp * g1.M / gm.M + 0.5)));
   long long pps = std::max((g1.M + a - 1) / a, (g2.M + (sp - a) - 1) / (sp - a));
   pps = (pps + bkp - 1) / bkp * bkp;
+  if (group > 1) {
+    WgradPlan p1;
+    ConvGeom t2;
+    int t1;
+    if (merged_plan(g1, n2, dt, p1, t1, t2, c1, allow_st, 1)) pps = std::min(pps, 2 * p1.pps);
+  }
   p.pps = pps;
   s1 = (int)((g1.M + pps - 1) / pps);
   p.splits = s1 + (int)((g2.M + pps - 1) / pps);
@@ -940,6 +1069,136 @@
   return 0;
 }
 
+bool group_plan(const ConvGeom& g, int64_t n2, int dt, int count, WgradPlan& p, int& s1, ConvGeom& g2) {
+  if (n2 > 0) {
+    if (!merged_plan(g, n2, dt, p, s1, g2, 0, false, count)) return false;
+  } else {
+    if (!wgrad_glds_ok(g, dt)) return false;
+    p = plan_for_cfg(g, wgrad_cfg_for(g), count);
+    s1 = 0;
+    g2 = g;
+  }
+  if (count > 1 && p.splits > 1 && 4ll * count * p.splits * g.K * g.KK > (64ll << 20)) return false;
+  return wgrad_group_cfg_ok(p.cfg);
+}
+
+size_t wgrad_group_ws_bytes(const ConvGeom& g, int64_t n2, int dt, int count) {
+  if (halo3_eligible(g, dt)) {
+    const HaloPlan hp = halo3_plan(g, g.N, n2, count);
+    if (count > 1 && hp.splits > 1 && 4ll * count * hp.splits * g.K * g.KK > (64ll << 20)) return 0;
+    return halo3_ws_bytes(g, g.N, n2, count) * count;
+  }
+  WgradPlan p;
+  ConvGeom g2;
+  int s1;
+  if (!group_plan(g, n2, dt, count, p, s1, g2)) return 0;
+  return (size_t)count * p.splits * g.K * g.KK * sizeof(float) + 256;
+}
+
+int wgrad_group_max(const ConvGeom& g, int64_t n2, int dt) {
+  for (int c = SSSEG_WGRAD_GROUP_MAX; c >= 1; --c)
+    if (wgrad_group_ws_bytes(g, n2, dt, c) > 0) return c;
+  return 0;
+}
+
+int wgrad_group(const ssseg_wgrad_member* mem, int count, int64_t n2, const ssseg_conv_desc* d, int dt, int64_t c_real,
+                int64_t k_real, int layout, int accumulate, void* ws, size_t ws_bytes, ssseg_stream_t stream) {
+  ConvGeom g, g2;
+  if (!make_geom(d, g) || !mem || count < 1 || count > SSSEG_WGRAD_GROUP_MAX || n2 < 0 || n2 > 0x7fffffff)
+    return SSSEG_EINVAL;
+  if (dt != SSSEG_BF16 && dt != SSSEG_F16) return SSSEG_EUNSUPPORTED;
+  if (!wg_geom_ok(g, dt) || g.ldy % 8 || g.K % 8) return SSSEG_EINVAL;
+  if (c_real < 1 || c_real > g.C || k_real < 1 || k_real > g.K || (layout != 0 && layout != 1)) return SSSEG_EINVAL;
+  WGroupTab tab{};
+  for (int i = 0; i < count; ++i) {
+    const ssseg_wgrad_member& m = mem[i];
+    if (!m.x1 || !m.dy1 || !m.dw || (n2 > 0 && (!m.x2 || !m.dy2))) return SSSEG_EINVAL;
+    for (int j = 0; j < i; ++j)
+      if (mem[j].dw == m.dw) return SSSEG_EINVAL;
+    tab.m[i] = m;
+  }
+  tab.n = count;
+  hipStream_t s = (hipStream_t)stream;
+  float* slab = (float*)ws;
+  if (halo3_eligible(g, dt)) {
+    if (!halo3_fits(g, g.N, nullptr) || (n2 > 0 && !halo3_fits(g, n2, nullptr))) return SSSEG_EUNSUPPORTED;
+    if (!wgrad_group_ws_bytes(g, n2, dt, count)) return SSSEG_EUNSUPPORTED;
+    if (!ws || ws_bytes < wgrad_group_ws_bytes(g, n2, dt, count)) return SSSEG_EWORKSPACE;
+    const HaloPlan hp = halo3_plan(g, g.N, n2, count);
+    HaloArgs a = halo_args(g, hp, nullptr, n2, c_real, k_real, layout, accumulate);
+    tab.per = hp.splits * hp.ncb * hp.nkb;
+    tab.slab_stride = (long long)hp.splits * g.K * g.KK;
+    a.slab = slab;
+    a.dw = hp.splits == 1 ? tab.m[0].dw : nullptr;
+    launch_wgrad_halo3_group(dt, a, tab, s);
+    if (hp.splits > 1 && !launch_reduce_group(tab, slab, g, hp.splits, c_real, k_real, layout, accumulate, s))
+      return SSSEG_EINVAL;
+    SSSEG_LAUNCH_CHECK();
+    return 0;
+  }
+  WgradPlan p;
+  int s1;
+  if (!group_plan(g, n2, dt, count, p, s1, g2)) return SSSEG_EUNSUPPORTED;
+  if (!ws || ws_bytes < wgrad_group_ws_bytes(g, n2, dt, count)) return SSSEG_EWORKSPACE;
+  tab.per = p.mt * p.nt * p.splits;
+  tab.slab_stride = (long long)p.splits * g.K * g.KK;
+  if ((long long)tab.per * count > 0x7fffffffLL) return SSSEG_EUNSUPPORTED;
+  WSeg2 sg{nullptr, nullptr, 0, 0, 0, 0, 0, 0, nullptr, nullptr, 0, 0};
+  if (n2 > 0)
+    sg = WSeg2{tab.m[0].x2, tab.m[0].dy2, g2.M, (unsigned)((long long)g2.N * g2.H * g2.W * g2.ldx * 2),
+               (unsigned)(g2.M * g2.ldy * 2), s1, 0, 0, nullptr, nullptr, 0, 0};
+  const WDirect dd{p.splits == 1 ? tab.m[0].dw : nullptr, (int)c_real, (int)k_real, layout, accumulate};
+  const bool ok = dt == SSSEG_F16 ? launch_wgrad_group<f16_t>(tab, slab, g, p, dd, s, sg)
+                                  : launch_wgrad_group<bf16_t>(tab, slab, g, p, dd, s, sg);
+  if (!ok) return SSSEG_EUNSUPPORTED;
+  if (p.splits > 1 && !launch_reduce_group(tab, slab, g, p.splits, c_real, k_real, layout, accumulate, s))
+    return SSSEG_EINVAL;
+  SSSEG_LAUNCH_CHECK();
+  return 0;
+}
+
+}
+
+extern "C" size_t ssseg_conv_wgrad_group_workspace_bytes(const ssseg_conv_desc* d, int64_t n2, int dt, int count) {
+  ConvGeom g;
+  if (!make_geom(d, g) || n2 < 0 || n2 > 0x7fffffff || count < 1 || count > SSSEG_WGRAD_GROUP_MAX) return 0;
+  return wgrad_group_ws_bytes(g, n2, dt, count);
+}
+
+extern "C" int ssseg_conv_wgrad_group(const ssseg_wgrad_member* members, int count, int64_t n2,
+                                      const ssseg_conv_desc* d, int dt, int64_t c_real, int64_t k_real, int layout,
+                                      int accumulate, void* ws, size_t ws_bytes, ssseg_stream_t stream) {
+  return wgrad_group(members, count, n2, d, dt, c_real, k_real, layout, accumulate, ws, ws_bytes, stream);
+}
+
+extern "C" int ssseg_conv_wgrad_group_pays(const ssseg_conv_desc* d, int64_t n2, int dt) {
+  ConvGeom g, g2;
+  if (!make_geom(d, g) || n2 < 0 || n2 > 0x7fffffff || (dt != SSSEG_BF16 && dt != SSSEG_F16)) return 0;
+  if (!wg_geom_ok(g, dt) || g.ldy % 8 || g.K % 8) return 0;
+  const long long M = g.M + n2 * (long long)g.OH * g.OW;
+  long long splits;
+  if (halo3_eligible(g, dt)) {
+    if (!halo3_fits(g, g.N, nullptr) || (n2 > 0 && !halo3_fits(g, n2, nullptr))) return 0;
+    splits = halo3_plan(g, g.N, n2).splits;
+  } else {
+    WgradPlan p;
+    int s1;
+    if (!group_plan(g, n2, dt, 1, p, s1, g2)) return 0;
+    splits = p.splits;
+    WgradPlan p2;
+    ConvGeom t2;
+    int t1;
+    if (p.pps >= 32ll * WGRAD_CFGS[p.cfg].bkp && group_plan(g, n2, dt, 2, p2, t1, t2) && p2.pps >= 2 * p.pps) return 0;
+  }
+  if (splits < 2 || wgrad_group_max(g, n2, dt) < 2) return 0;
+  return 6 * (splits * 4ll * g.K * g.KK) >= 2ll * M * (g.C + g.K) ? 1 : 0;
+}
+
+extern "C" int ssseg_conv_wgrad_group_max(const ssseg_conv_desc* d, int64_t n2, int dt) {
+  ConvGeom g;
+  if (!make_geom(d, g) || n2 < 0 || n2 > 0x7fffffff || (dt != SSSEG_BF16 && dt != SSSEG_F16)) return 0;
+  if (!wg_geom_ok(g, dt) || g.ldy % 8 || g.K % 8) return 0;
+  return wgrad_group_max(g, n2, dt);
 }
 
 extern "C" int ssseg_conv_wgrad(const void* x, const void* dy, float* dw, const ssseg_conv_desc* d, int dt,
diff --git a/semi-supervised_semantic_segmentation_amd/csrc/conv_wgrad_halo.hip b/semi-supervised_semantic_segmentation_amd/csrc/conv_wgrad_halo.hip
--- a/semi-supervised_semantic_segmentation_amd/csrc/conv_wgrad_halo.hip
+++ b/semi-supervised_semantic_segmentation_amd/csrc/conv_wgrad_halo.hip
@@ -15,11 +15,12 @@
 __device__ __forceinline__ int hkp(int g, int j) { return 16 * (g >> 1) + 8 * (g & 1) + 4 * (j >> 2) + (j & 3); }
 
 template <typename T16>
-__global__ void __launch_bounds__(256, 2) wgrad_halo3_kernel(HaloArgs a) {
+__device__ __forceinline__ void wgrad_halo3_body(const HaloArgs& a, const void* x0, const void* dy0, const void* x1,
+                                                 const void* dy1, float* __restrict__ slab, float* __restrict__ dw,
+                                                 int tile) {
   __shared__ __attribute__((aligned(1024))) char smem[H_SMEM];
   const int lane = threadIdx.x & 63, wave = __builtin_amdgcn_readfirstlane(threadIdx.x >> 6);
   const int tiles = a.ncb * a.nkb;
-  const int tile = xcd_tile(blockIdx.x, gridDim.x);
   const int split = tile / tiles, rem = tile - split * tiles;
   const int cb = rem % a.ncb, kb = rem / a.ncb;
   const int sg = split >= a.s1 ? 1 : 0;
@@ -27,11 +28,12 @@
   const long long t1 = min(t0 + a.sps[sg], a.steps[sg]);
   const HaloSeg& S = a.seg[sg];
   const bool part2 = a.c1 > 0 && cb * 64 >= a.c1;
-  const char* xsrc = (const char*)(part2 ? S.x2 : S.x);
+  const char* xsrc = (const char*)(part2 ? S.x2 : (sg ? x1 : x0));
   const unsigned xbytes = part2 ? S.x2bytes : S.xbytes;
   const int ldx = part2 ? a.ldx2 : a.ldx, c0 = part2 ? cb * 64 - a.c1 : cb * 64;
   const __amdgpu_buffer_rsrc_t xr = __builtin_amdgcn_make_buffer_rsrc((void*)xsrc, (short)0, (int)xbytes, 0x00020000);
-  const __amdgpu_buffer_rsrc_t dr = __builtin_amdgcn_make_buffer_rsrc((void*)S.dy, (short)0, (int)S.dbytes, 0x00020000);
+  const __amdgpu_buffer_rsrc_t dr =
+      __builtin_amdgcn_make_buffer_rsrc((void*)(sg ? dy1 : dy0), (short)0, (int)S.dbytes, 0x00020000);
   const int H = a.H, W = a.W;
 
   const int lrow = lane >> 3;
@@ -149,7 +151,7 @@
     for (int j = 0; j < 4; ++j) {
       const int k = kb * 64 + 16 * j + li;
       const int kk = tap * a.C + cbase;
-      if (a.dw) {
+      if (dw) {
         if (k >= a.k_real) continue;
 #pragma unroll
         for (int e = 0; e < 4; ++e) {
@@ -157,13 +159,28 @@
           if (c >= a.c_real) continue;
           const long long o = a.layout == 0 ? ((long long)k * 9 + tap) * a.C + c
                                             : (((long long)k * a.c_real + c) * 3 + tap / 3) * 3 + tap % 3;
-          a.dw[o] = a.accumulate ? a.dw[o] + acc[tap][j][e] : acc[tap][j][e];
+          dw[o] = a.accumulate ? dw[o] + acc[tap][j][e] : acc[tap][j][e];
         }
       } else {
-        float* p = a.slab + ((long long)split * a.K + k) * (9LL * a.C) + kk;
+        float* p = slab + ((long long)split * a.K + k) * (9LL * a.C) + kk;
         *(float4*)p = make_float4(acc[tap][j][0], acc[tap][j][1], acc[tap][j][2], acc[tap][j][3]);
       }
     }
+}
+
+template <typename T16>
+__global__ void __launch_bounds__(256, 2) wgrad_halo3_kernel(HaloArgs a) {
+  wgrad_halo3_body<T16>(a, a.seg[0].x, a.seg[0].dy, a.seg[1].x, a.seg[1].dy, a.slab, a.dw,
+                        xcd_tile(blockIdx.x, gridDim.x));
+}
+
+template <typename T16>
+__global__ void __launch_bounds__(256, 2) wgrad_halo3_group_kernel(HaloArgs a, WGroupTab tab) {
+  const int id = xcd_tile(blockIdx.x, gridDim.x);
+  const int mi = id / tab.per;
+  const ssseg_wgrad_member& m = tab.m[mi];
+  wgrad_halo3_body<T16>(a, m.x1, m.dy1, m.x2, m.dy2, a.slab + (long long)mi * tab.slab_stride, a.dw ? m.dw : nullptr,
+                        id - mi * tab.per);
 }
 
 }
@@ -175,18 +192,20 @@
          g.ldy % 8 == 0 && g.ldy >= g.K;
 }
 
-HaloPlan halo3_plan(const ConvGeom& g, long long n1, long long n2) {
+HaloPlan halo3_plan(const ConvGeom& g, long long n1, long long n2, int group) {
   HaloPlan p;
   p.ncb = g.C / 64;
   p.nkb = g.K / 64;
   p.nstrips = g.W / 64;
-  const long long tiles = (long long)p.ncb * p.nkb;
+  const long long tiles = (long long)p.ncb * p.nkb * group;
   const long long st1 = n1 * p.nstrips * g.H, st2 = n2 * p.nstrips * g.H;
-  const long long slab1 = 4LL * g.K * 9 * g.C;
+  const long long slab1 = 4LL * g.K * 9 * g.C * group;
   long long want = std::max<long long>(1, (512 + tiles - 1) / tiles);
   const long long cap = std::max<long long>((256 + tiles - 1) / tiles, (64LL << 20) / slab1);
   want = std::min(want, cap);
   if (g_knobs[10] != 100 && g_knobs[10] > 0) want = std::max<long long>(1, want * g_knobs[10] / 100);
+  const HaloPlan alone = group > 1 ? halo3_plan(g, n1, n2, 1) : HaloPlan{};
+  if (group > 1) want = std::max<long long>(want, (alone.splits + 1) / 2);
   want = std::min<long long>(want, st1 + st2);
   long long a1 = n2 > 0 ? std::max<long long>(1, std::min(want - 1, (long long)((double)want * st1 / (st1 + st2) + 0.5)))
                         : want;
@@ -196,13 +215,17 @@
   p.steps[1] = st2;
   p.sps[0] = (st1 + a1 - 1) / a1;
   p.sps[1] = a2 ? (st2 + a2 - 1) / a2 : 1;
+  if (group > 1) {
+    p.sps[0] = std::min(p.sps[0], 2 * alone.sps[0]);
+    if (a2) p.sps[1] = std::min(p.sps[1], 2 * alone.sps[1]);
+  }
   p.s1 = (int)((st1 + p.sps[0] - 1) / p.sps[0]);
   p.splits = p.s1 + (a2 ? (int)((st2 + p.sps[1] - 1) / p.sps[1]) : 0);
   return p;
 }
 
-size_t halo3_ws_bytes(const ConvGeom& g, long long n1, long long n2) {
-  const HaloPlan p = halo3_plan(g, n1, n2);
+size_t halo3_ws_bytes(const ConvGeom& g, long long n1, long long n2, int group) {
+  const HaloPlan p = halo3_plan(g, n1, n2, group);
   return (size_t)p.splits * g.K * 9 * g.C * sizeof(float) + 256;
 }
 
@@ -213,3 +236,11 @@
   else
     hipLaunchKernelGGL(wgrad_halo3_kernel<bf16_t>, dim3(blocks), dim3(256), 0, s, a);
 }
+
+void launch_wgrad_halo3_group(int dt, const HaloArgs& a, const WGroupTab& tab, hipStream_t s) {
+  const unsigned blocks = (unsigned)(tab.per * tab.n);
+  if (dt == SSSEG_F16)
+    hipLaunchKernelGGL(wgrad_halo3_group_kernel<f16_t>, dim3(blocks), dim3(256), 0, s, a, tab);
+  else
+    hipLaunchKernelGGL(wgrad_halo3_group_kernel<bf16_t>, dim3(blocks), dim3(256), 0, s, a, tab);
+}
diff --git a/semi-supervised_semantic_segmentation_amd/ssseg/native.py b/semi-supervised_semantic_segmentation_amd/ssseg/native.py
--- a/semi-supervised_semantic_segmentation_amd/ssseg/native.py
+++ b/semi-supervised_semantic_segmentation_amd/ssseg/native.py
@@ -151,6 +151,10 @@
     'ssseg_conv_wgrad': (i32, [vp, vp, vp, vp, i32, i64, i64, i32, i32, vp, sz, vp]),
     'ssseg_conv_wgrad2_workspace_bytes': (sz, [vp, i64, i32]),
     'ssseg_conv_wgrad2': (i32, [vp, vp, vp, vp, i64, vp, vp, i32, i64, i64, i32, i32, vp, sz, vp]),
+    'ssseg_conv_wgrad_group_workspace_bytes': (sz, [vp, i64, i32, i32]),
+    'ssseg_conv_wgrad_group': (i32, [vp, i32, i64, vp, i32, i64, i64, i32, i32, vp, sz, vp]),
+    'ssseg_conv_wgrad_group_pays': (i32, [vp, i64, i32]),
+    'ssseg_conv_wgrad_group_max': (i32, [vp, i64, i32]),
     'ssseg_conv_igemm_epi_vcat': (i32, [vp, vp, vp, vp, vp, i32, i32, vp, vp, sz, vp]),
     'ssseg_conv_igemm_epi_vsplit': (i32, [vp, vp, vp, vp, vp, i32, i32, vp, vp, sz, vp]),
     'ssseg_conv_wgrad_vcat': (i32, [vp, vp, vp, vp, vp, i32, i64, i64, i32, i32, vp, sz, vp]),
@@ -255,6 +259,17 @@
     _fields_ = [('x2', ctypes.c_void_p), ('c1', ctypes.c_int64), ('ldx2', ctypes.c_int64)]
 
 
+WGRAD_GROUP_MAX = 8
+
+
+class WgradMember(ctypes.Structure):
+    _fields_ = [(n, ctypes.c_void_p) for n in ('x1', 'dy1', 'x2', 'dy2', 'dw')]
+
+
+def wgrad_members(rows):
+    return (WgradMember * len(rows))(*[WgradMember(*r) for r in rows])
+
+
 _lib = None
 
 
diff --git a/semi-supervised_semantic_segmentation_amd/ssseg/nn.py b/semi-supervised_semantic_segmentation_amd/ssseg/nn.py
--- a/semi-supervised_semantic_segmentation_amd/ssseg/nn.py
+++ b/semi-supervised_semantic_segmentation_amd/ssseg/nn.py
@@ -91,6 +91,83 @@
         pair = mod.__dict__.pop('_ssseg_wg_pending', None)
         if pair is not None:
             mod._ssseg_wgrad(*pair, bias_grad=False, want=(True, False))
+    for key in list(_WGROUP['queues']):
+        _wg_group_launch(key)
+
+
+_WGROUP = {'on': os.environ.get('SSSEG_WGRAD_GROUP', '1') != '0', 'live': False, 'queues': {}, 'pays': {}}
+
+
+def set_wgrad_group(on):
+    _WGROUP['on'] = bool(on)
+
+
+@contextlib.contextmanager
+def group_wgrad():
+    prev = _WGROUP['live']
+    _WGROUP['live'] = _WGROUP['on']
+    try:
+        yield
+    finally:
+        _WGROUP['live'] = prev
+
+
+def wgrad_group_pending():
+    return sum(len(q) for q in _WGROUP['queues'].values())
+
+
+def _wg_group_add(mod, d, x1, gy1, x, gy, n):
+    if not _WGROUP['live'] or not x.is_cuda:
+        return False
+    if any(getattr(p, '_ssseg_reducer', None) is not None for p in (mod.weight, mod.bias) if p is not None):
+        return False
+    dt = N.dt_code(x)
+    if dt not in (N.BF16, N.F16):
+        return False
+    key = (tuple(getattr(d, f) for f, _ in d._fields_), n, dt, mod.in_channels, mod.out_channels, x.device)
+    cap = _WGROUP['pays'].get(key)
+    if cap is None:
+        pays = N.lib().ssseg_conv_wgrad_group_pays(ctypes_ref(d), n, dt)
+        cap = _WGROUP['pays'][key] = N.lib().ssseg_conv_wgrad_group_max(ctypes_ref(d), n, dt) if pays else 0
+    if cap < 2:
+        return False
+    q = _WGROUP['queues'].get(key)
+    if q and any(e[0] is mod for e in q):
+        _wg_group_launch(key)
+        q = None
+    if q is None:
+        q = _WGROUP['queues'][key] = []
+    q.append((mod, d, x1, gy1, x, gy, n))
+    if len(q) >= cap:
+        _wg_group_launch(key)
+    return True
+
+
+def _wg_group_launch(key):
+    q = _WGROUP['queues'].pop(key, None)
+    if not q:
+        return
+    mod0, d, _, _, x0, _, n = q[0]
+    nb = N.lib().ssseg_conv_wgrad_group_workspace_bytes(ctypes_ref(d), n, key[2], len(q)) if len(q) > 1 else 0
+    done = False
+    if nb:
+        cur = torch.cuda.current_stream()
+        for e in q:
+            for t in e[2:6]:
+                t.record_stream(cur)
+        ws = N.workspace(nb, x0.device)
+        tab = N.wgrad_members([(N.dev_ptr(x1), N.dev_ptr(gy1), N.dev_ptr(x), N.dev_ptr(gy),
+                                N.dev_ptr(_grad_of(m.weight))) for m, _, x1, gy1, x, gy, _ in q])
+        R, S = mod0.kernel_size
+        with _Timed(len(q) * _conv_flops(d.N + n, d.OH, d.OW, mod0.out_channels, mod0.in_channels, R, S), 'wgrad',
+                    f'{len(q)} x {_tag(mod0, d.N + n, d.H, d.W)}'):
+            done = N.call_or_unsupported('ssseg_conv_wgrad_group', tab, len(q), n, ctypes_ref(d), key[2],
+                                         mod0.in_channels, mod0.out_channels, 1, 1, N.dev_ptr(ws), nb, N.stream())
+    for m, _, x1, gy1, x, gy, _ in q:
+        if done:
+            _ready(*[p for p in (m.weight, m.bias) if p is not None])
+        else:
+            m._wgrad_launch(x, gy, (x1, gy1), group=False)
 
 
 _HOLD = {'on': False, 'tag': None, 'calls': [], 'params': False, 'adds': []}
@@ -149,9 +226,10 @@
         for tag, mod, args, kw in calls:
             if tag == order[0]:
                 mod._ssseg_wgrad(*args, **kw)
-    for tag, mod, args, kw in calls:
-        if tag == order[1]:
-            mod._ssseg_wgrad(*args, **kw)
+    with group_wgrad():
+        for tag, mod, args, kw in calls:
+            if tag == order[1]:
+                mod._ssseg_wgrad(*args, **kw)
     flush_wgrad()
 
 
@@ -907,7 +985,7 @@
             return
         self._wgrad_launch(x, gy, self._wg_take(x, gy))
 
-    def _wgrad_launch(self, x, gy, pend):
+    def _wgrad_launch(self, x, gy, pend, group=True):
         n, _, H, W = x.shape
         R, S = self.kernel_size
         if pend is None:
@@ -930,9 +1008,11 @@
             x1, gy1 = pend
             n1 = x1.shape[0]
             d = self._fwd_desc(n1, H, W)
+            v1, v2 = _vcat_of(x1), _vcat_of(x)
+            if group and v1 is None and v2 is None and _wg_group_add(self, d, x1, gy1, x, gy, n):
+                return
             nb = N.lib().ssseg_conv_wgrad2_workspace_bytes(ctypes_ref(d), n, N.dt_code(x))
             ws = N.workspace(nb, x.device)
-            v1, v2 = _vcat_of(x1), _vcat_of(x)
             with _Timed(_conv_flops(n1 + n, d.OH, d.OW, self.out_channels, self.in_channels, R, S), 'wgrad',
                         _tag(self, n1 + n, H, W)):
                 both = v1 is not None and v2 is not None and v1.same_split(v2) and v1.ready(d)
diff --git a/semi-supervised_semantic_segmentation_amd/train.py b/semi-supervised_semantic_segmentation_amd/train.py
--- a/semi-supervised_semantic_segmentation_amd/train.py
+++ b/semi-supervised_semantic_segmentation_amd/train.py
@@ -296,7 +296,7 @@
         del targets, cons
         if ddp is not None:
             ddp.arm()
-        with snn.defer_param_grads():
+        with snn.defer_param_grads(), snn.group_wgrad():
             if side_fwd:
                 side = _side_stream(image.device)
                 side.wait_stream(torch.cuda.current_stream())
```
